# mmorise/World

Hardware: AMD Instinct MI355X
Metric: analysis frames/sec (Harvest+CheapTrick+D4C, 48 kHz, 5 ms hop) (higher is better)
Workload: dtype f64; 1 GPU; configs[1]: 1 x (48 kHz, 10 s) utterance(s) per step, Harvest+CheapTrick+D4C, fft_size=2048, frame_period=5 ms, inputs/outputs in HBM, 12 independent jobs in flight (one HIP stream + context each, a different utterance per job); utterances_per_gpu=1, jobs_in_flight=12, parallelism=single GPU, no collective

## Files before the change

### include/world_hip.h

```cpp
#ifndef WORLD_HIP_H_
#define WORLD_HIP_H_

#ifdef __cplusplus
extern "C" {
#endif

#if defined(__GNUC__)
#define WORLD_HIP_API __attribute__((visibility("default")))
#else
#define WORLD_HIP_API
#endif


typedef struct {
  double f0_floor;
  double f0_ceil;
  double channels_in_octave;
  double frame_period;
  int speed;
  double allowed_range;
} DioOption;

typedef struct {
  double f0_floor;
// ... 58 lines not shown
  fft_complex *c_in;
  double *in;
  fft_complex *c_out;
  double *out;
  double *input;
  int *ip;
  double *w;
} fft_plan;
typedef struct {
  int fft_size;
  double *waveform;
  fft_complex *spectrum;
  fft_plan forward_fft;
} ForwardRealFFT;
typedef struct {
  int fft_size;
  double *waveform;
  fft_complex *spectrum;
  fft_plan inverse_fft;
} InverseRealFFT;
typedef struct {
  int fft_size;
  double *log_spectrum;
  fft_complex *minimum_phase_spectrum;
  fft_complex *cepstrum;
  fft_plan inverse_fft;
  fft_plan forward_fft;
} MinimumPhaseAnalysis;
typedef struct {
  unsigned int g_randn_x;
  unsigned int g_randn_y;
  unsigned int g_randn_z;
  unsigned int g_randn_w;
} RandnState;
typedef struct {
  int fs;
  double frame_period;
  int buffer_size;
  int number_of_pointers;
  int fft_size;
  double *buffer;
  int current_pointer;
  int i;
  double *dc_remover;
  int *f0_length;
  int *f0_origin;
  double ***spectrogram;
  double ***aperiodicity;
  int current_pointer2;
  int head_pointer;
  int synthesized_sample;
  int handoff;
  double handoff_phase;
  double handoff_f0;
  int last_location;
  int cumulative_frame;
  int current_frame;
  double **interpolated_vuv;
  double **pulse_locations;
  int **pulse_locations_index;
  int *number_of_pulses;
  double *impulse_response;
  RandnState randn_state;
  MinimumPhaseAnalysis minimum_phase;
  InverseRealFFT inverse_real_fft;
  ForwardRealFFT forward_real_fft;
} WorldSynthesizer;
WORLD_HIP_API void InitializeSynthesizer(int fs, double frame_period, int fft_size, int buffer_size,
                                         int number_of_pointers, WorldSynthesizer *synth);
WORLD_HIP_API int AddParameters(double *f0, int f0_length, double **spectrogram, double **aperiodicity,
                                WorldSynthesizer *synth);
WORLD_HIP_API void RefreshSynthesizer(WorldSynthesizer *synth);
WORLD_HIP_API void DestroySynthesizer(WorldSynthesizer *synth);
WORLD_HIP_API int IsLocked(WorldSynthesizer *synth);
WORLD_HIP_API int Synthesis2(WorldSynthesizer *synth);

WORLD_HIP_API void wavwrite(const double *x, int x_length, int fs, int nbit, const char *filename);
WORLD_HIP_API int GetAudioLength(const char *filename);
WORLD_HIP_API void wavread(const char *filename, int *fs, int *nbit, double *x);
WORLD_HIP_API void WriteF0(const char *filename, int f0_length, double frame_period,
                           const double *temporal_positions, const double *f0, int text_flag);
WORLD_HIP_API int ReadF0(const char *filename, double *temporal_positions, double *f0);
WORLD_HIP_API double GetHeaderInformation(const char *filename, const char *parameter);
WORLD_HIP_API void WriteSpectralEnvelope(const char *filename, int fs, int f0_length, double frame_period,
                                         int fft_size, int number_of_dimensions, const double *const *spectrogram);
WORLD_HIP_API int ReadSpectralEnvelope(const char *filename, double **spectrogram);
WORLD_HIP_API void WriteAperiodicity(const char *filename, int fs, int f0_length, double frame_period,
                                     int fft_size, int number_of_dimensions, const double *const *aperiodicity);
WORLD_HIP_API int ReadAperiodicity(const char *filename, double **aperiodicity);


typedef void (*WorldHipErrorHandler)(const char *function, const char *message, void *user);
WORLD_HIP_API void world_hip_set_error_handler(WorldHipErrorHandler handler, void *user);
WORLD_HIP_API int world_hip_shutdown(void);
WORLD_HIP_API void world_hip_dropin_stats(unsigned long long *slots, unsigned long long *x_hits,
                                          unsigned long long *x_misses);

typedef struct WorldHipContext WorldHipContext;

WORLD_HIP_API WorldHipContext *world_hip_create(int device, void *stream);
WORLD_HIP_API void world_hip_destroy(WorldHipContext *ctx);
WORLD_HIP_API const char *world_hip_last_error(void);
#define WORLD_HIP_ABI_VERSION 6
#define WORLD_HIP_HINT_SHARED_DEVICE 1
WORLD_HIP_API int world_hip_set_hint(WorldHipContext *ctx, int hint);
WORLD_HIP_API int world_hip_abi_version(void);
WORLD_HIP_API int world_hip_sync(WorldHipContext *ctx);
WORLD_HIP_API unsigned long long world_hip_workspace_bytes(WorldHipContext *ctx);
WORLD_HIP_API unsigned long long world_hip_noise_table_bytes(WorldHipContext *ctx);
WORLD_HIP_API int world_hip_verify_tables(WorldHipContext *ctx);
WORLD_HIP_API double world_hip_noise_table_build_ms(WorldHipContext *ctx, int *builds);

WORLD_HIP_API void world_hip_profile_enable(int on);
WORLD_HIP_API int world_hip_profile_collect(char *buf, int cap);

WORLD_HIP_API int world_hip_harvest_batch(WorldHipContext *ctx, int n_utt, int fs, const double *d_x,
                                          int x_stride, const int *x_length, const HarvestOption *option,
                                          int f_stride, double *d_tpos, double *d_f0);
WORLD_HIP_API int world_hip_dio_batch(WorldHipContext *ctx, int n_utt, int fs, const double *d_x,
                                      int x_stride, const int *x_length, const DioOption *option,
                                      int f_stride, double *d_tpos, double *d_f0);
WORLD_HIP_API int world_hip_stonemask_batch(WorldHipContext *ctx, int n_utt, int fs, const double *d_x,
                                            int x_stride, const int *x_length, const int *n_frames,
                                            int f_stride, const double *d_tpos, const double *d_f0,
                                            double *d_refined_f0);
WORLD_HIP_API int world_hip_cheaptrick_batch(WorldHipContext *ctx, int n_utt, int fs, const double *d_x,
                                             int x_stride, const int *x_length, const int *n_frames,
                                             int f_stride, const double *d_tpos, const double *d_f0,
                                             const CheapTrickOption *option, double *d_spectrogram);
WORLD_HIP_API int world_hip_d4c_batch(WorldHipContext *ctx, int n_utt, int fs, const double *d_x,
                                      int x_stride, const int *x_length, const int *n_frames,
                                      int f_stride, const double *d_tpos, const double *d_f0,
                                      int fft_size, const D4COption *option, double *d_aperiodicity);

WORLD_HIP_API int world_hip_synthesis_batch(WorldHipContext *ctx, int n_utt, int fs, double frame_period,
                                            int fft_size, const int *n_frames, int f_stride, const double *d_f0,
                                            const double *d_spectrogram, const double *d_aperiodicity,
                                            const int *y_length, int y_stride, double *d_y);

WORLD_HIP_API int world_hip_synthesis_records(WorldHipContext *ctx, int n_utt, int fs, double frame_period, int fft_size,
                                              const int *n_frames, long long first_row, const double *d_block, int cols,
                                              int wire, int number_of_dimensions, const int *y_length, int y_stride,
                                              double *d_y);

WORLD_HIP_API int world_hip_probe_machine(WorldHipContext *ctx, double *values, int n_values);
WORLD_HIP_API int world_hip_probe_rfft(WorldHipContext *ctx, int lg_n, int max_lr, int threads, int static_plan,
                                       long long batch, const double *d_in, double *d_spectrum);
WORLD_HIP_API int world_hip_probe_irfft(WorldHipContext *ctx, int lg_n, int max_lr, int threads, int static_plan,
                                        long long batch, const double *d_spectrum, double *d_out);
WORLD_HIP_API int world_hip_probe_fft(WorldHipContext *ctx, int mode, int lg_n, int max_lr, int threads, int swizzle,
                                      long long batch, const void *d_in, void *d_out);
WORLD_HIP_API int world_hip_probe_select(WorldHipContext *ctx, int mode, int threads, int K, long long rows,
                                         const double *d_keys, double *d_out);
WORLD_HIP_API int world_hip_probe_harvest_contour(WorldHipContext *ctx, int n_utt, const int *nfb, const int *nc, int maxc,
                                                  int fb_stride, const double *d_cand, const double *d_score, double frame_period,
                                                  int f_stride, double *d_pruned_cand, double *d_pruned_score, double *d_step2,
                                                  double *d_step3, double *d_step4, int sec_cap, int *d_sec_n, int *d_sec,
                                                  double *d_basic_f0, double *d_tpos, double *d_f0);
WORLD_HIP_API int world_hip_probe_harvest_candidates(WorldHipContext *ctx, int n_utt, const int *nfb, double afs, double f0_floor,
                                                     double f0_ceil, int nch, const double *band_f0, int maxc, int fb_stride,
                                                     int nseg, int seg_cap, int ev_cap, int ev_group, int stages,
                                                     const double *d_seg_events, const int *d_seg_count, double *d_events,
                                                     int *d_ev_count, double *d_raw, double *d_cand, int *d_nc);

WORLD_HIP_API int world_hip_analyze_batch(WorldHipContext *ctx, int n_utt, int fs, const double *d_x, int x_stride,
                                          const int *x_length, const HarvestOption *harvest_option,
                                          const CheapTrickOption *cheaptrick_option, const D4COption *d4c_option,
                                          int f_stride, double *d_tpos, double *d_f0, double *d_spectrogram,
                                          double *d_aperiodicity);
WORLD_HIP_API int world_hip_record_columns(int fft_size, int wire);
WORLD_HIP_API int world_hip_analyze_packed(WorldHipContext *ctx, int n_utt, int fs, const double *d_x, int x_stride,
                                           const int *x_length, const HarvestOption *harvest_option,
                                           const CheapTrickOption *cheaptrick_option, const D4COption *d4c_option,
                                           long long first_row, double *d_block, int cols);
WORLD_HIP_API int world_hip_coded_columns(int fs, int number_of_dimensions);
WORLD_HIP_API int world_hip_analyze_coded(WorldHipContext *ctx, int n_utt, int fs, const double *d_x, int x_stride,
                                          const int *x_length, const HarvestOption *harvest_option,
                                          const CheapTrickOption *cheaptrick_option, const D4COption *d4c_option,
                                          int number_of_dimensions, long long first_row, double *d_block, int cols);
WORLD_HIP_API int world_hip_spectral_packed_range(WorldHipContext *ctx, int n_utt, int fs, const double *d_x, int x_stride,
                                                  const int *x_length, const int *n_frames, int f_stride,
                                                  const double *d_tpos, const double *d_f0,
                                                  const CheapTrickOption *cheaptrick_option, const D4COption *d4c_option,
                                                  int frame_lo, int frame_hi, int reuse_offsets, long long first_row,
                                                  double *d_block, int cols);
WORLD_HIP_API int world_hip_cheaptrick_batch_range(WorldHipContext *ctx, int n_utt, int fs, const double *d_x, int x_stride,
                                                   const int *x_length, const int *n_frames, int f_stride,
                                                   const double *d_tpos, const double *d_f0, const CheapTrickOption *option,
                                                   int frame_lo, int frame_hi, int reuse_offsets, double *d_spectrogram);
WORLD_HIP_API int world_hip_d4c_batch_range(WorldHipContext *ctx, int n_utt, int fs, const double *d_x, int x_stride,
                                            const int *x_length, const int *n_frames, int f_stride, const double *d_tpos,
                                            const double *d_f0, int fft_size, const D4COption *option, int frame_lo,
                                            int frame_hi, int reuse_offsets, double *d_aperiodicity);
WORLD_HIP_API int world_hip_pack_results(WorldHipContext *ctx, int n_utt, const int *n_frames, int f_stride,
                                         int bins, const double *d_tpos, const double *d_f0,
                                         const double *d_spectrogram, const double *d_aperiodicity,
                                         long long first_row, double *d_block);
WORLD_HIP_API int world_hip_unpack_results(WorldHipContext *ctx, int n_utt, const int *n_frames, int f_stride,
                                           int bins, const double *d_block, long long first_row, double *d_tpos,
                                           double *d_f0, double *d_spectrogram, double *d_aperiodicity);
WORLD_HIP_API int world_hip_allgather_blocks(int n_dev, WorldHipContext *const *ctxs, const double *const *d_src,
                                             const long long *rows, int cols, double *const *d_dst);

WORLD_HIP_API int world_hip_analyze_sharded(int n_dev, WorldHipContext *const *ctxs, int n_utt, int fs,
                                            const double *const *x, const int *x_length,
                                            const HarvestOption *harvest_option, const CheapTrickOption *cheaptrick_option,
                                            const D4COption *d4c_option, int sub_batch, double *const *d_blocks,
                                            long long rows_capacity, int cols, long long *where);

WORLD_HIP_API int world_hip_check_shape(int fs, int cheaptrick_fft_size, char *why, int why_capacity);

WORLD_HIP_API int world_hip_graph_begin(WorldHipContext *ctx);
WORLD_HIP_API int world_hip_graph_end(WorldHipContext *ctx, void **graph);
WORLD_HIP_API int world_hip_graph_launch(WorldHipContext *ctx, void *graph);
WORLD_HIP_API int world_hip_graph_destroy(void *graph);

WORLD_HIP_API int world_hip_set_synthesis_pulse_capacity(WorldHipContext *ctx, int pulses_per_utterance);
WORLD_HIP_API int world_hip_synthesis_pulses_dropped(WorldHipContext *ctx, int *needed);

WORLD_HIP_API int world_hip_pcm16_to_double(WorldHipContext *ctx, long long n, const short *d_pcm, double *d_x);

WORLD_HIP_API int world_hip_pcm_to_double(WorldHipContext *ctx, long long n, int nbit, const void *d_pcm, double *d_x);
WORLD_HIP_API int world_hip_double_to_pcm16(WorldHipContext *ctx, long long n, const double *d_x, short *d_pcm);
WORLD_HIP_API int world_hip_wav_layout(const char *filename, int *fs, int *nbit, int *x_length,
                                       long long *data_offset);
WORLD_HIP_API int world_hip_wav_write_pcm16(const char *filename, int fs, long long n, const short *pcm);

#define WORLD_HIP_RESAMPLE_BEST 0
#define WORLD_HIP_RESAMPLE_FAST 1
typedef struct { int zeros; double rolloff; double kaiser_beta; } WorldHipResampleOption;
WORLD_HIP_API void world_hip_resample_option(int quality, WorldHipResampleOption *opt);
WORLD_HIP_API int world_hip_resample_length(int n_in, int fs_in, int fs_out);
WORLD_HIP_API int world_hip_resample_shape(int fs_in, int fs_out, const WorldHipResampleOption *opt, int *L, int *M, int *W);
WORLD_HIP_API int world_hip_resample_taps(int fs_in, int fs_out, const WorldHipResampleOption *opt, double *table );
WORLD_HIP_API int world_hip_resample_batch(WorldHipContext *ctx, int n_utt, int fs_in, int fs_out,
                                           const WorldHipResampleOption *opt, const double *d_x, int x_stride,
                                           const int *x_length , double *d_y, int y_stride);

WORLD_HIP_API double world_hip_mcep_alpha(int fs);
WORLD_HIP_API int world_hip_mcep_tables(int fft_size, int order, double alpha, double *M ,
                                        double *D );
WORLD_HIP_API int world_hip_sp2mc(WorldHipContext *ctx, int rows, int fft_size, int order, double alpha, const double *d_sp,
                                  long long sp_row_stride, double *d_mc, long long mc_row_stride);
WORLD_HIP_API int world_hip_mc2sp(WorldHipContext *ctx, int rows, int fft_size, int order, double alpha, const double *d_mc,
                                  long long mc_row_stride, double *d_sp, long long sp_row_stride);

WORLD_HIP_API int world_hip_delta_batch(WorldHipContext *ctx, int n_utt, int dim, int n_win, int half_width,
                                        const double *win , const int *n_frames ,
                                        const unsigned char *d_mask, long long mask_utt_stride, const double *d_c,
                                        long long c_utt_stride, long long c_row_stride, double fill, double *d_out,
                                        long long out_utt_stride, long long out_row_stride);
WORLD_HIP_API int world_hip_mlpg_batch(WorldHipContext *ctx, int n_utt, int dim, int n_win, int half_width,
                                       const double *win , const int *n_frames ,
                                       const unsigned char *d_mask, long long mask_utt_stride, const double *d_mean,
                                       long long mean_utt_stride, long long mean_row_stride, const double *d_var,
                                       long long var_utt_stride, long long var_row_stride, int precision, double fill,
                                       double *d_out, long long out_utt_stride, long long out_row_stride);

WORLD_HIP_API long long world_hip_gmm_model_doubles(int M, int Dx, int Dy);
WORLD_HIP_API int world_hip_gmm_prepare(int M, int Dx, int Dy, const double *w, const double *mu, const double *cov,
                                        double *model );
WORLD_HIP_API int world_hip_gmm_model_parts(int M, int Dx, int Dy, const double *model , double *c, double *mux,
                                            double *muy, double *U, double *A, double *v);
WORLD_HIP_API int world_hip_gmm_convert(WorldHipContext *ctx, int M, int Dx, int Dy, const double *d_model, int rows,
                                        const double *d_x, long long x_row_stride, int mode, double *d_mean,
                                        long long mean_row_stride, double *d_var, long long var_row_stride, double *d_post,
                                        long long post_row_stride, double *d_loglik);
WORLD_HIP_API int world_hip_gmm_accumulate(WorldHipContext *ctx, int M, int P, int rows, const double *d_z,
                                           long long z_row_stride, const double *d_post, long long post_row_stride,
                                           const double *d_shift , double *d_N , double *d_S1 ,
                                           double *d_G );
WORLD_HIP_API int world_hip_gmm_update(int M, int P, const double *N, const double *S1, const double *G, const double *shift,
                                       double total_rows, double reg, double *w, double *mu, double *cov);
WORLD_HIP_API int world_hip_gmm_fit(WorldHipContext *ctx, int M, int P, int rows, const double *d_z, long long z_row_stride,
                                    int n_iter, double reg, double *w, double *mu, double *cov ,
                                    double *loglik );
WORLD_HIP_API int world_hip_gmm_init(WorldHipContext *ctx, int M, int P, int rows, const double *d_z, long long z_row_stride,
                                     double *w, double *mu, double *cov );

WORLD_HIP_API int world_hip_frame_power_batch(WorldHipContext *ctx, int n_utt, int fft_size, const int *n_frames ,
                                              const double *d_sp, long long sp_utt_stride, long long sp_row_stride,
                                              double *d_power, long long power_utt_stride, double *d_mean);
WORLD_HIP_API int world_hip_select_frames_batch(WorldHipContext *ctx, int n_utt, const int *n_frames ,
                                                const double *d_value, long long value_utt_stride, long long value_stride,
                                                double threshold, const double *d_scale, const unsigned char *d_mask,
                                                long long mask_utt_stride, int *d_index, long long index_utt_stride,
                                                int *d_count, unsigned char *d_keep, long long keep_utt_stride);
WORLD_HIP_API int world_hip_gather_rows_batch(WorldHipContext *ctx, int n_utt, int dim, const int *n_src ,
                                              const double *d_in, long long in_utt_stride, long long in_row_stride,
                                              const int *n_out , const int *d_index, long long index_utt_stride,
                                              double fill, double *d_out, long long out_utt_stride, long long out_row_stride);
WORLD_HIP_API int world_hip_joint_rows_batch(WorldHipContext *ctx, int n_pairs, int dim_a, int dim_b, const double *d_a,
                                             const long long *a_row , const int *n_a , long long a_row_stride,
                                             const double *d_b, const long long *b_row , const int *n_b ,
                                             long long b_row_stride, const int *path_len , const int *d_path,
                                             int p_stride, const int *d_sel_a, const int *n_sel_a ,
                                             long long sel_a_stride, const int *d_sel_b, const int *n_sel_b ,
                                             long long sel_b_stride, double fill, double *d_z, const long long *z_row ,
                                             long long z_row_stride);

WORLD_HIP_API int world_hip_code_spectral_envelope(WorldHipContext *ctx, int rows, int fs, int fft_size,
                                                   int number_of_dimensions, const double *d_spectrogram,
                                                   double *d_coded);
WORLD_HIP_API int world_hip_decode_spectral_envelope(WorldHipContext *ctx, int rows, int fs, int fft_size,
                                                     int number_of_dimensions, const double *d_coded,
                                                     double *d_spectrogram);
// ... 76 lines not shown
```

### world_amd/api.py

```python
import ctypes as C
import os
import weakref

import numpy as np

HERE = os.path.dirname(os.path.abspath(__file__))
LIB_PATH = os.environ.get("WORLD_HIP_LIB") or os.path.join(HERE, "libworld_hip.so")

_dp = C.POINTER(C.c_double)
_ip = C.POINTER(C.c_int)


class DioOption(C.Structure):
    _fields_ = [("f0_floor", C.c_double), ("f0_ceil", C.c_double), ("channels_in_octave", C.c_double),
                ("frame_period", C.c_double), ("speed", C.c_int), ("allowed_range", C.c_double)]


class HarvestOption(C.Structure):
    _fields_ = [("f0_floor", C.c_double), ("f0_ceil", C.c_double), ("frame_period", C.c_double)]


class CheapTrickOption(C.Structure):
    _fields_ = [("q1", C.c_double), ("f0_floor", C.c_double), ("fft_size", C.c_int)]

# ... 90 lines not shown
                ("cepstrum", C.c_void_p), ("inverse_fft", FftPlan), ("forward_fft", FftPlan)]


class WorldSynthesizer(C.Structure):
    _fields_ = [("fs", C.c_int), ("frame_period", C.c_double), ("buffer_size", C.c_int), ("number_of_pointers", C.c_int),
                ("fft_size", C.c_int), ("buffer", _dp), ("current_pointer", C.c_int), ("i", C.c_int),
                ("dc_remover", _dp), ("f0_length", _ip), ("f0_origin", _ip), ("spectrogram", C.c_void_p),
                ("aperiodicity", C.c_void_p), ("current_pointer2", C.c_int), ("head_pointer", C.c_int),
                ("synthesized_sample", C.c_int), ("handoff", C.c_int), ("handoff_phase", C.c_double),
                ("handoff_f0", C.c_double), ("last_location", C.c_int), ("cumulative_frame", C.c_int),
                ("current_frame", C.c_int), ("interpolated_vuv", C.c_void_p), ("pulse_locations", C.c_void_p),
                ("pulse_locations_index", C.POINTER(_ip)), ("number_of_pulses", _ip), ("impulse_response", _dp),
                ("randn_state", RandnState), ("minimum_phase", MinimumPhaseAnalysis),
                ("inverse_real_fft", InverseRealFFT), ("forward_real_fft", ForwardRealFFT)]


REALTIME_SCALARS = ("current_pointer", "i", "current_pointer2", "head_pointer", "synthesized_sample", "handoff",
                    "handoff_phase", "handoff_f0", "last_location", "cumulative_frame", "current_frame")
RT_ADD, RT_SYNTH, RT_LOCKED, RT_REFRESH = 0, 1, 2, 3


def bind_realtime(L):
    sp = C.POINTER(WorldSynthesizer)
    L.InitializeSynthesizer.argtypes = [C.c_int, C.c_double, C.c_int, C.c_int, C.c_int, sp]
    L.InitializeSynthesizer.restype = None
    L.AddParameters.argtypes = [_dp, C.c_int, C.POINTER(_dp), C.POINTER(_dp), sp]
    L.RefreshSynthesizer.argtypes = [sp]
    L.RefreshSynthesizer.restype = None
    L.DestroySynthesizer.argtypes = [sp]
    L.DestroySynthesizer.restype = None
    L.IsLocked.argtypes = [sp]
    L.Synthesis2.argtypes = [sp]
    return L


def run_realtime_plan(L, plan):
    fs, fp, fft, bs, P = (int(plan["fs"]), float(plan["frame_period"]), int(plan["fft_size"]), int(plan["buffer_size"]),
                          int(plan["number_of_pointers"]))
    f0, sp, ap = _f64(plan["f0"]), _f64(plan["sp"]), _f64(plan["ap"])
    chunks = [int(c) for c in plan["chunks"]]
    drain_every = int(plan.get("drain_every", 1))
    refresh_before = int(plan.get("refresh_before", -1))
    stop_on_lock = bool(plan.get("stop_on_lock", False))
    rows_sp, rows_ap = _rows(sp), _rows(ap)

    def at(rows, i):
        return C.cast(C.c_void_p(C.cast(rows, C.c_void_p).value + i * C.sizeof(_dp)), C.POINTER(_dp))

    s = WorldSynthesizer()
    L.InitializeSynthesizer(fs, fp, fft, bs, P, C.byref(s))
    calls, out, pulses, counts, rings = [], [], [], [], []

    def record(op, ret):
        r = s.randn_state
        calls.append([op, ret] + [getattr(s, k) for k in REALTIME_SCALARS] +
                     [r.g_randn_x, r.g_randn_y, r.g_randn_z, r.g_randn_w])

    def drain():
        while True:
            r = L.Synthesis2(C.byref(s))
            record(RT_SYNTH, r)
            if r == 0:
                break
            out.append(np.ctypeslib.as_array(s.buffer, shape=(bs,)).copy())
        locked = L.IsLocked(C.byref(s))
        record(RT_LOCKED, locked)
        return locked

    i = k = adds = 0
    refused = 0
    try:
        while k < len(chunks):
            if k == refresh_before and refused == 0:
                L.RefreshSynthesizer(C.byref(s))
                record(RT_REFRESH, 0)
                refresh_before = -1
            n = chunks[k]
            r = L.AddParameters(f0[i:].ctypes.data_as(_dp), n, at(rows_sp, i), at(rows_ap, i), C.byref(s))
            record(RT_ADD, r)
            if r == 1:
                slot = (s.head_pointer - 1) % P
                npu = s.number_of_pulses[slot]
                counts.append(npu)
                if npu:
                    pulses.extend(s.pulse_locations_index[slot][:npu])
                i += n; k += 1; adds += 1; refused = 0
                w = min(adds, P)
                rings.append([[s.f0_length[j] if j < w else 0 for j in range(P)],
                              [s.f0_origin[j] if j < w else 0 for j in range(P)],
                              [s.number_of_pulses[j] for j in range(P)]])
                if adds % drain_every != 0 and k < len(chunks):
                    continue
            else:
                refused += 1
                if refused > 1:
                    break
            if drain() and stop_on_lock:
                break
    finally:
        L.DestroySynthesizer(C.byref(s))
    return {"calls": np.array(calls, dtype=np.float64).reshape(-1, 2 + len(REALTIME_SCALARS) + 4),
            "out": np.concatenate(out) if out else np.zeros(0), "pulses": np.array(pulses, dtype=np.int64),
            "pulse_counts": np.array(counts, dtype=np.int64), "rings": np.array(rings, dtype=np.int64).reshape(-1, 3, P)}


def _hip_runtime_first():
    try:
        import torch
    except ImportError:
        pass


def load_library(path=LIB_PATH):
    if not os.path.exists(path):
        raise ImportError(f"{path} is missing: build it with `python -m world_amd.build` "
                          "(hipcc, gfx950). There is no non-GPU fallback.")
    _hip_runtime_first()
    lib = C.CDLL(path)
    abi = lib.world_hip_abi_version() if hasattr(lib, "world_hip_abi_version") else 5
    if abi not in (5, 6):
        raise ImportError(f"{path}: batched ABI version {abi}, this binding speaks 5-6")
    lib.abi_version = abi
    vp = C.c_void_p
    lib.world_hip_create.restype = vp
    lib.world_hip_create.argtypes = [C.c_int, vp]
    lib.world_hip_destroy.argtypes = [vp]
    lib.world_hip_last_error.restype = C.c_char_p
    lib.world_hip_sync.argtypes = [vp]
    lib.world_hip_workspace_bytes.restype = C.c_ulonglong
    lib.world_hip_workspace_bytes.argtypes = [vp]
    lib.world_hip_noise_table_bytes.restype = C.c_ulonglong
    lib.world_hip_noise_table_bytes.argtypes = [vp]
    lib.world_hip_verify_tables.argtypes = [vp]
    lib.world_hip_harvest_batch.argtypes = [vp, C.c_int, C.c_int, vp, C.c_int, _ip, C.POINTER(HarvestOption),
                                            C.c_int, vp, vp]
    lib.world_hip_dio_batch.argtypes = [vp, C.c_int, C.c_int, vp, C.c_int, _ip, C.POINTER(DioOption),
                                        C.c_int, vp, vp]
    lib.world_hip_stonemask_batch.argtypes = [vp, C.c_int, C.c_int, vp, C.c_int, _ip, _ip, C.c_int, vp, vp, vp]
    lib.world_hip_cheaptrick_batch.argtypes = [vp, C.c_int, C.c_int, vp, C.c_int, _ip, _ip, C.c_int, vp, vp,
                                               C.POINTER(CheapTrickOption), vp]
    lib.world_hip_d4c_batch.argtypes = [vp, C.c_int, C.c_int, vp, C.c_int, _ip, _ip, C.c_int, vp, vp, C.c_int,
                                        C.POINTER(D4COption), vp]
    lib.world_hip_synthesis_batch.argtypes = [vp, C.c_int, C.c_int, C.c_double, C.c_int, _ip, C.c_int, vp, vp, vp,
                                              _ip, C.c_int, vp]
    lib.world_hip_pcm16_to_double.argtypes = [vp, C.c_longlong, vp, vp]
    lib.world_hip_set_synthesis_pulse_capacity.argtypes = [vp, C.c_int]
    lib.world_hip_synthesis_pulses_dropped.argtypes = [vp, _ip]
    lib.world_hip_probe_rfft.argtypes = [vp, C.c_int, C.c_int, C.c_int, C.c_int, C.c_longlong, vp, vp]
    lib.world_hip_probe_irfft.argtypes = [vp, C.c_int, C.c_int, C.c_int, C.c_int, C.c_longlong, vp, vp]
    if hasattr(lib, "world_hip_probe_fft"):
        lib.world_hip_probe_fft.argtypes = [vp, C.c_int, C.c_int, C.c_int, C.c_int, C.c_int, C.c_longlong, vp, vp]
    if hasattr(lib, "world_hip_probe_select"):
        lib.world_hip_probe_select.argtypes = [vp, C.c_int, C.c_int, C.c_int, C.c_longlong, vp, vp]
    if hasattr(lib, "world_hip_probe_harvest_contour"):
        lib.world_hip_probe_harvest_contour.argtypes = [vp, C.c_int, _ip, _ip, C.c_int, C.c_int, vp, vp, C.c_double, C.c_int,
                                                        vp, vp, vp, vp, vp, C.c_int, vp, vp, vp, vp, vp]
    if hasattr(lib, "world_hip_probe_harvest_candidates"):
        lib.world_hip_probe_harvest_candidates.argtypes = [vp, C.c_int, _ip, C.c_double, C.c_double, C.c_double, C.c_int,
                                                           C.POINTER(C.c_double)] + [C.c_int] * 7 + [vp] * 7
    lib.world_hip_analyze_packed.argtypes = [vp, C.c_int, C.c_int, vp, C.c_int, _ip, C.POINTER(HarvestOption),
                                             C.POINTER(CheapTrickOption), C.POINTER(D4COption), C.c_longlong, vp, C.c_int]
    lib.world_hip_analyze_sharded.argtypes = [C.c_int, C.POINTER(vp), C.c_int, C.c_int, C.POINTER(vp), _ip,
                                              C.POINTER(HarvestOption), C.POINTER(CheapTrickOption), C.POINTER(D4COption),
                                              C.c_int, C.POINTER(vp), C.c_longlong, C.c_int, C.POINTER(C.c_longlong)]
    lib.world_hip_check_shape.argtypes = [C.c_int, C.c_int, C.c_char_p, C.c_int]
    if hasattr(lib, "world_hip_set_hint"):
        lib.world_hip_set_hint.argtypes = [vp, C.c_int]
    if hasattr(lib, "world_hip_probe_machine"):
        lib.world_hip_probe_machine.argtypes = [vp, C.POINTER(C.c_double), C.c_int]
    lib.world_hip_record_columns.argtypes = [C.c_int, C.c_int]
    if hasattr(lib, "world_hip_analyze_coded"):
        lib.world_hip_coded_columns.argtypes = [C.c_int, C.c_int]
        lib.world_hip_analyze_coded.argtypes = [vp, C.c_int, C.c_int, vp, C.c_int, _ip, C.POINTER(HarvestOption),
                                                C.POINTER(CheapTrickOption), C.POINTER(D4COption), C.c_int, C.c_longlong, vp, C.c_int]
    lib.world_hip_spectral_packed_range.argtypes = [vp, C.c_int, C.c_int, vp, C.c_int, _ip, _ip, C.c_int, vp, vp,
                                                    C.POINTER(CheapTrickOption), C.POINTER(D4COption), C.c_int, C.c_int,
                                                    C.c_int, C.c_longlong, vp, C.c_int]
    lib.world_hip_cheaptrick_batch_range.argtypes = [vp, C.c_int, C.c_int, vp, C.c_int, _ip, _ip, C.c_int, vp, vp,
                                                     C.POINTER(CheapTrickOption), C.c_int, C.c_int, C.c_int, vp]
    lib.world_hip_d4c_batch_range.argtypes = [vp, C.c_int, C.c_int, vp, C.c_int, _ip, _ip, C.c_int, vp, vp, C.c_int,
                                              C.POINTER(D4COption), C.c_int, C.c_int, C.c_int, vp]
    lib.world_hip_analyze_batch.argtypes = [vp, C.c_int, C.c_int, vp, C.c_int, _ip, C.POINTER(HarvestOption),
                                            C.POINTER(CheapTrickOption), C.POINTER(D4COption), C.c_int, vp, vp, vp, vp]
    lib.world_hip_graph_begin.argtypes = [vp]
    lib.world_hip_graph_end.argtypes = [vp, C.POINTER(vp)]
    lib.world_hip_graph_launch.argtypes = [vp, vp]
    lib.world_hip_graph_destroy.argtypes = [vp]
    lib.world_hip_pack_results.argtypes = [vp, C.c_int, _ip, C.c_int, C.c_int, vp, vp, vp, vp, C.c_longlong, vp]
    lib.world_hip_unpack_results.argtypes = [vp, C.c_int, _ip, C.c_int, C.c_int, vp, C.c_longlong, vp, vp, vp, vp]
    lib.world_hip_allgather_blocks.argtypes = [C.c_int, C.POINTER(vp), C.POINTER(vp), C.POINTER(C.c_longlong), C.c_int,
                                               C.POINTER(vp)]
    lib.world_hip_pcm_to_double.argtypes = [vp, C.c_longlong, C.c_int, vp, vp]
    lib.world_hip_double_to_pcm16.argtypes = [vp, C.c_longlong, vp, vp]
    lib.world_hip_wav_layout.argtypes = [C.c_char_p, _ip, _ip, _ip, C.POINTER(C.c_longlong)]
    lib.world_hip_wav_write_pcm16.argtypes = [C.c_char_p, C.c_int, C.c_longlong, vp]
    lib.world_hip_code_spectral_envelope.argtypes = [vp, C.c_int, C.c_int, C.c_int, C.c_int, vp, vp]
    lib.world_hip_decode_spectral_envelope.argtypes = [vp, C.c_int, C.c_int, C.c_int, C.c_int, vp, vp]
    lib.world_hip_code_aperiodicity.argtypes = [vp, C.c_int, C.c_int, C.c_int, vp, vp]
    lib.world_hip_decode_aperiodicity.argtypes = [vp, C.c_int, C.c_int, C.c_int, vp, vp]
    lib.GetNumberOfAperiodicities.argtypes = [C.c_int]
    lib.GetFFTSizeForCheapTrick.argtypes = [C.c_int, C.POINTER(CheapTrickOption)]
    if hasattr(lib, "world_hip_realtime_create"):
        lib.world_hip_realtime_create.argtypes = [vp, C.c_int, C.c_int, C.c_double, C.c_int, C.c_int, C.c_int,
                                                  C.POINTER(vp)]
        lib.world_hip_realtime_destroy.argtypes = [vp]
        lib.world_hip_realtime_destroy.restype = None
        lib.world_hip_realtime_add.argtypes = [vp, C.c_int, _dp, C.c_int, vp, vp, C.c_int]
        lib.world_hip_realtime_synthesize.argtypes = [vp, vp, _ip]
        lib.world_hip_realtime_is_locked.argtypes = [vp, C.c_int]
        lib.world_hip_realtime_refresh.argtypes = [vp, C.c_int]
        lib.world_hip_realtime_rng_jump.argtypes = [C.POINTER(C.c_uint32), C.c_ulonglong, C.POINTER(C.c_uint32)]
        lib.world_hip_realtime_rng_jump.restype = None
    if hasattr(lib, "world_hip_modify_batch"):
        mp = C.POINTER(WorldHipModification)
        lib.world_hip_f0_statistics.argtypes = [vp, C.c_int, _ip, C.c_int, vp, vp]
        lib.world_hip_modify_batch.argtypes = [vp, C.c_int, C.c_int, C.c_int, _ip, C.c_int, mp, vp, vp, vp, vp]
        lib.world_hip_resynthesis_length.argtypes = [C.c_int, C.c_int, C.c_double, C.c_double]
        lib.world_hip_resynthesize_batch.argtypes = [vp, C.c_int, C.c_int, vp, C.c_int, _ip, C.POINTER(HarvestOption),
                                                     C.POINTER(CheapTrickOption), C.POINTER(D4COption), mp, C.c_double,
                                                     _ip, C.c_int, vp]
    if hasattr(lib, "world_hip_modify_frames_batch"):
        mp, cp = C.POINTER(WorldHipModification), C.POINTER(WorldHipFrameCurves)
        lib.world_hip_modify_frames_batch.argtypes = [vp, C.c_int, C.c_int, C.c_int, _ip, C.c_int, _ip, C.c_int, mp, cp,
                                                      vp, vp, vp, vp, vp, vp]
        lib.world_hip_resynthesize_frames_batch.argtypes = [vp, C.c_int, C.c_int, vp, C.c_int, _ip, C.POINTER(HarvestOption),
                                                            C.POINTER(CheapTrickOption), C.POINTER(D4COption), mp, cp, _ip,
                                                            C.c_int, _ip, C.c_int, vp]
    if hasattr(lib, "world_hip_synthesis_records"):
        lib.world_hip_synthesis_records.argtypes = [vp, C.c_int, C.c_int, C.c_double, C.c_int, _ip, C.c_longlong, vp,
                                                    C.c_int, C.c_int, C.c_int, _ip, C.c_int, vp]
        lib.world_hip_realtime_add_coded.argtypes = [vp, C.c_int, _dp, C.c_int, vp, C.c_int, vp, C.c_int]
    if hasattr(lib, "world_hip_align_batch"):
        lp = C.POINTER(C.c_longlong)
        lib.world_hip_align_batch.argtypes = [vp, C.c_int, C.c_int, vp, lp, _ip, C.c_int, vp, lp, _ip, C.c_int, C.c_int,
                                              vp, vp, vp, C.c_int, vp, vp]
        lib.world_hip_align_workspace_cells.argtypes = []
    if hasattr(lib, "world_hip_morph_batch"):
        lib.world_hip_morph_length.argtypes = [C.c_int, C.c_int, C.c_double]
        lib.world_hip_morph_batch.argtypes = [vp, C.c_int, C.c_int, C.c_int, _ip, C.c_int, vp, vp, vp, _ip, C.c_int, vp, vp, vp,
                                              C.c_int, vp, vp, C.POINTER(WorldHipMorph), C.POINTER(WorldHipMorphCurves),
                                              C.c_int, vp, vp, vp, vp, vp]
    if hasattr(lib, "world_hip_resample_batch"):
        op = C.POINTER(WorldHipResampleOption)
        lib.world_hip_resample_option.argtypes = [C.c_int, op]
        lib.world_hip_resample_option.restype = None
        lib.world_hip_resample_length.argtypes = [C.c_int, C.c_int, C.c_int]
        lib.world_hip_resample_shape.argtypes = [C.c_int, C.c_int, op, _ip, _ip, _ip]
        lib.world_hip_resample_taps.argtypes = [C.c_int, C.c_int, op, vp]
        lib.world_hip_resample_batch.argtypes = [vp, C.c_int, C.c_int, C.c_int, op, vp, C.c_int, _ip, vp, C.c_int]
    if hasattr(lib, "world_hip_sp2mc"):
        lib.world_hip_mcep_alpha.argtypes = [C.c_int]
        lib.world_hip_mcep_alpha.restype = C.c_double
        lib.world_hip_mcep_tables.argtypes = [C.c_int, C.c_int, C.c_double, vp, vp]
        for fn in (lib.world_hip_sp2mc, lib.world_hip_mc2sp):
            fn.argtypes = [vp, C.c_int, C.c_int, C.c_int, C.c_double, vp, C.c_longlong, vp, C.c_longlong]
    if hasattr(lib, "world_hip_mlpg_batch"):
        ll = C.c_longlong
        lib.world_hip_delta_batch.argtypes = [vp, C.c_int, C.c_int, C.c_int, C.c_int, vp, _ip, vp, ll, vp, ll, ll, C.c_double,
                                              vp, ll, ll]
        lib.world_hip_mlpg_batch.argtypes = [vp, C.c_int, C.c_int, C.c_int, C.c_int, vp, _ip, vp, ll, vp, ll, ll, vp, ll, ll,
                                             C.c_int, C.c_double, vp, ll, ll]
    if hasattr(lib, "world_hip_gmm_convert"):
        ll, i, d = C.c_longlong, C.c_int, C.c_double
        lib.world_hip_gmm_model_doubles.argtypes = [i, i, i]
        lib.world_hip_gmm_model_doubles.restype = ll
        lib.world_hip_gmm_prepare.argtypes = [i, i, i, vp, vp, vp, vp]
        lib.world_hip_gmm_model_parts.argtypes = [i, i, i, vp, vp, vp, vp, vp, vp, vp]
        lib.world_hip_gmm_convert.argtypes = [vp, i, i, i, vp, i, vp, ll, i, vp, ll, vp, ll, vp, ll, vp]
        lib.world_hip_gmm_accumulate.argtypes = [vp, i, i, i, vp, ll, vp, ll, vp, vp, vp, vp]
        lib.world_hip_gmm_update.argtypes = [i, i, vp, vp, vp, vp, d, d, vp, vp, vp]
        lib.world_hip_gmm_fit.argtypes = [vp, i, i, i, vp, ll, i, d, vp, vp, vp, vp]
        lib.world_hip_gmm_init.argtypes = [vp, i, i, i, vp, ll, vp, vp, vp]
    if hasattr(lib, "world_hip_joint_rows_batch"):
        ll, i, d, lp = C.c_longlong, C.c_int, C.c_double, C.POINTER(C.c_longlong)
        lib.world_hip_frame_power_batch.argtypes = [vp, i, i, _ip, vp, ll, ll, vp, ll, vp]
        lib.world_hip_select_frames_batch.argtypes = [vp, i, _ip, vp, ll, ll, d, vp, vp, ll, vp, ll, vp, vp, ll]
        lib.world_hip_gather_rows_batch.argtypes = [vp, i, i, _ip, vp, ll, ll, _ip, vp, ll, d, vp, ll, ll]
        lib.world_hip_joint_rows_batch.argtypes = [vp, i, i, i, vp, lp, _ip, ll, vp, lp, _ip, ll, _ip, vp, i, vp, _ip, ll, vp, _ip, ll,
                                                   d, vp, lp, ll]
    lib.world_hip_profile_enable.argtypes = [C.c_int]
    lib.world_hip_profile_collect.argtypes = [C.c_char_p, C.c_int]
    return lib


def frame_count(fs, x_length, frame_period):
    return int(1000.0 * x_length / fs / frame_period) + 1


def resample_length(n_in, fs_in, fs_out):
    import math
    n_in, fs_in, fs_out = int(n_in), int(fs_in), int(fs_out)
    if n_in < 1 or fs_in < 1 or fs_out < 1:
        raise ValueError(f"resample_length: {n_in} samples, {fs_in} -> {fs_out} Hz")
    g = math.gcd(fs_in, fs_out)
    n = -((-n_in * (fs_out // g)) // (fs_in // g))
    if n > 2 ** 31 - 1:
        raise ValueError(f"resample_length: {n_in} samples at {fs_in} Hz are more than INT_MAX at {fs_out} Hz")
    return n


def resample_option(quality="best"):
    if isinstance(quality, WorldHipResampleOption):
        return quality
    if isinstance(quality, str):
        if quality not in RESAMPLE_QUALITIES:
            raise ValueError(f"resample: quality {quality!r} is neither 'best' nor 'fast' nor a (zeros, rolloff, beta) triple")
# ... 1624 lines not shown
```

### world_amd/csrc/api.hip

```cpp
#include "../../include/world_hip.h"

#include <algorithm>
#include <climits>
#include <cmath>
#include <cstdint>
#include <cstring>
#include <cstdarg>
#include <deque>
#include <mutex>
#include <thread>
#include <unordered_map>
#include <stdexcept>
#include <string>
#include <vector>

#include "common.h"
#include "bandfilter.h"
#include "codec.h"
#include "decimate.h"
#include "dio.h"
#include "exchange.h"
#include "fft_probe.h"
#include "d4c_select_probe.h"
#include "gmm_host.h"
// ... 271 lines not shown
}
template <class T> static T *upload(WorldHipContext *c, const std::vector<T> &v) { return upload(c, v.data(), v.size()); }

struct Span { const void *p; size_t bytes; const char *name; };
static void refuse_overlap(const char *call, std::initializer_list<Span> outs, std::initializer_list<Span> ins) {
  auto meet = [](const Span &a, const Span &b) {
    const char *a_lo = static_cast<const char *>(a.p), *b_lo = static_cast<const char *>(b.p);
    return a.p && b.p && a_lo < b_lo + b.bytes && b_lo < a_lo + a.bytes;
  };
  for (const Span *o = outs.begin(); o != outs.end(); ++o) {
    for (const Span &i : ins)
      if (meet(*o, i)) fail("%s: %s overlaps %s; no output may alias an input", call, o->name, i.name);
    for (const Span *o2 = o + 1; o2 != outs.end(); ++o2)
      if (meet(*o, *o2)) fail("%s: %s overlaps %s", call, o->name, o2->name);
  }
}

static int ilog2_exact(int n) {
  int l = 0;
  while ((1 << l) < n) ++l;
  if ((1 << l) != n) fail("fft size %d is not a power of two", n);
  return l;
}
constexpr int kGridY = 65535;

static int frame_count(int fs, int x_length, double frame_period) {
  return static_cast<int>(1000.0 * x_length / fs / frame_period) + 1;
}

static void check_batch(int n_utt, int fs, const void *d_x, int x_stride, const int *x_length) {
  if (n_utt <= 0) fail("n_utt must be positive");
  if (fs <= 0) fail("fs must be positive");
  if (!d_x || !x_length) fail("null input");
  for (int u = 0; u < n_utt; ++u)
    if (x_length[u] <= 0 || x_length[u] > x_stride) fail("x_length[%d]=%d outside (0, x_stride=%d]", u, x_length[u], x_stride);
}
static int max_frame_count(const int *n_frames, int n_utt, int f_stride) {
  int max_frames = 0;
  for (int u = 0; u < n_utt; ++u) {
    if (n_frames[u] < 0 || n_frames[u] > f_stride) fail("n_frames[%d] outside [0, f_stride]", u);
    max_frames = std::max(max_frames, n_frames[u]);
  }
  return max_frames;
}
static std::vector<int> record_rows(const int *n_frames, int n_utt, long long first_row) {
  std::vector<int> rows(n_utt);
  long long row = first_row;
  for (int u = 0; u < n_utt; ++u) {
    if (row + n_frames[u] > 0x7FFFFFFFll) fail("block exceeds 2^31 records");
    rows[u] = static_cast<int>(row);
    row += n_frames[u];
  }
  return rows;
}
static BatchView batch_view(WorldHipContext *c, int n_utt, int fs, const double *d_x, int x_stride, const int *x_length,
                            const int *n_frames, int f_stride) {
  BatchView b;
  b.n_utt = n_utt; b.fs = fs; b.x_stride = x_stride; b.f_stride = f_stride; b.x = d_x;
  b.x_len = upload(c, std::vector<int>(x_length, x_length + n_utt));
  b.n_frames = upload(c, std::vector<int>(n_frames, n_frames + n_utt));
  return b;
}

struct RowLayout {
  const int *rows = nullptr;
  size_t stride = 0;
  size_t col_bytes = 0;
  int f32 = 0;
  double *rec = nullptr;
  int code_dims = 0;
  const int *code_knot = nullptr;
  const double *code_frac = nullptr, *code_w_re = nullptr, *code_w_im = nullptr;
  int frame_lo = 0, frame_hi = 0x7FFFFFFF;
  bool skip_prepare = false;
};
static int record_cols(int fft_size, int wire) {
  const int nb = fft_size / 2 + 1;
  return wire == 1 ? 2 + nb : 2 + 2 * nb;
}

static int d4c_internal_fft(int fs) { return static_cast<int>(pow(2.0, 1.0 + static_cast<int>(log(4.0 * fs / kFloorF0D4C + 1) / kLog2))); }
static int d4c_park_slots(int n_utt, int f_stride) {
  return static_cast<int>(std::min<size_t>((size_t)n_utt * f_stride, (size_t)std::max(n_utt, 2048)));
}

static void arena_reset(WorldHipContext *c) {
  c->arena.reset();
  c->prep_ct.valid = c->prep_d4c.valid = false;
}
template <class Carve> static void begin_stage(WorldHipContext *c, Carve carve) {
  ensure_arena(c, measure(carve));
  arena_reset(c);
  devrt::dpoison(c->arena.base + c->arena.floor, c->arena.cap - c->arena.floor, c->stream);
  carve(c->arena);
  open_uploads(c);
}
template <class Carve, class Body> static void hold_at_floor(WorldHipContext *c, const char *what, Carve carve, Body body) {
  struct Release {
    WorldHipContext *c;
    ~Release() { c->arena.floor = 0; c->prep_ct.valid = c->prep_d4c.valid = false; }
  } release{c};
  size_t want = 0;
  for (int attempt = 0;; ++attempt) {
    c->arena.floor = 0;
    ensure_arena(c, std::max(measure(carve), want));
    arena_reset(c);
    devrt::dpoison(c->arena.base, c->arena.cap, c->stream);
    carve(c->arena);
    c->arena.floor = c->arena.used;
    try {
      body();
      return;
    } catch (const ArenaRegrow &r) {
      if (devrt::is_capturing(c->stream)) fail("a call shape that was never run before cannot be captured: run it once first");
      if (attempt >= 4) fail("%s: the workspace did not settle", what);
      want = std::max(want, r.bytes);
    }
  }
}

static uint64_t lengths_hash(const int *x_length, const int *n_frames, int n_utt) {
  const uint64_t a = SmallArrays::hash(x_length, sizeof(int) * n_utt), b = SmallArrays::hash(n_frames, sizeof(int) * n_utt);
  return a * 0x9E3779B97F4A7C15ull ^ b;
}
static void claim_prepared(WorldHipContext *c, WorldHipContext::PrepToken &mine, WorldHipContext::PrepToken &other,
                           WorldHipContext::PrepToken want, bool reuse, const char *stage) {
  want.arena_base = c->arena.base; want.generation = c->generation;
  if (reuse) {
    if (!mine.valid)
      fail("%s: reuse_offsets, but this context holds no prepared offsets (another stage, another shape or a regrown "
           "workspace since the call that prepared them)", stage);
    if (!mine.same_inputs(want))
      fail("%s: reuse_offsets, but the prepared offsets belong to other inputs (shape, buffers or options differ from the "
           "call that prepared them)", stage);
    return;
  }
  if (other.valid && want.lo < other.hi && other.lo < want.hi) other.valid = false;
  mine = want;
  mine.valid = true;
}
static void carve_cheaptrick(Arena &a, CtParams &p) {
  p.offsets = a.take<unsigned>((size_t)p.b.n_utt * p.b.f_stride);
  p.frec = a.take<CtFrameRec>((size_t)p.b.n_utt * p.b.f_stride);
}
static void carve_d4c(Arena &a, D4cParams &p) {
  CtParams below;
  below.b = p.b;
  carve_cheaptrick(a, below);
  const size_t fr = (size_t)p.b.n_utt * p.b.f_stride;
  p.ap0 = a.take<double>(fr);
  p.offsets1 = a.take<unsigned>(fr);
  p.draws2 = a.take<unsigned>(fr);
  p.draws1 = a.take<unsigned>(p.b.n_utt);
  p.frec = a.take<D4cFrameRec>(fr);
  p.coarse = a.take<double>(fr * 16);
  const size_t slot = d4c_park_slot_doubles(p.lg_d4c);
  p.park_ws = slot ? a.take<double>(slot * p.park_slots) : nullptr;
}
static void spectral_workspace(WorldHipContext *c, CtParams *ct, D4cParams *d4c, const int *x_length, const int *n_frames) {
  ensure_arena(c, d4c ? measure([&](Arena &a) { carve_d4c(a, *d4c); }) : measure([&](Arena &a) { carve_cheaptrick(a, *ct); }));
  const BatchView &b = ct ? ct->b : d4c->b;
  WorldHipContext::PrepToken t;
  t.n_utt = b.n_utt; t.fs = b.fs; t.f_stride = b.f_stride; t.x_stride = b.x_stride; t.x = b.x;
  t.lengths_hash = lengths_hash(x_length, n_frames, b.n_utt);
  if (ct) {
    c->arena.reset();
    carve_cheaptrick(c->arena, *ct);
    t.fft = 1 << ct->lg_fft; t.f0 = ct->f0; t.tpos = ct->tpos; t.opt = ct->f0_floor;
    t.lo = 0; t.hi = c->arena.used;
    claim_prepared(c, c->prep_ct, c->prep_d4c, t, ct->skip_prepare != 0, "CheapTrick");
    if (!ct->skip_prepare) devrt::dpoison(c->arena.base + c->arena.floor, c->arena.used - c->arena.floor, c->stream);
  }
  if (d4c) {
    c->arena.reset();
    carve_d4c(c->arena, *d4c);
    t.fft = d4c->fft_out; t.f0 = d4c->f0; t.tpos = d4c->tpos; t.opt = d4c->threshold;
    t.lo = reinterpret_cast<char *>(d4c->ap0) - c->arena.base; t.hi = c->arena.used;
    claim_prepared(c, c->prep_d4c, c->prep_ct, t, d4c->skip_prepare != 0, "D4C");
    char *lo = reinterpret_cast<char *>(d4c->skip_prepare ? d4c->coarse : d4c->ap0);
    devrt::dpoison(lo, c->arena.base + c->arena.used - lo, c->stream);
  }
}

static std::string shape_limit(int what, int fs, int fft_size);
static void refuse_shape_limit(int what, int fs, int fft_size) {
  const std::string lim = shape_limit(what, fs, fft_size);
  if (!lim.empty()) fail("%s", lim.c_str());
}
static bool inkernel_consts() { return getenv("WORLD_HIP_INKERNEL_CONSTS") != nullptr; }
static CtParams setup_cheaptrick(WorldHipContext *c, int n_utt, int fs, const double *d_x, int x_stride,
                                 const int *x_length, const int *n_frames, int f_stride, const double *d_tpos,
                                 const double *d_f0, const CheapTrickOption *opt, double *d_sp, const RowLayout &lay,
                                 int *max_frames_out) {
  check_batch(n_utt, fs, d_x, x_stride, x_length);
  const int lg = ilog2_exact(opt->fft_size);
  const std::string lim = shape_limit(2, fs, opt->fft_size);
  if (!lim.empty()) fail("%s", lim.c_str());
  const int max_frames = *max_frames_out = max_frame_count(n_frames, n_utt, f_stride);
  CtParams p;
  p.b = batch_view(c, n_utt, fs, d_x, x_stride, x_length, n_frames, f_stride);
  p.tpos = d_tpos; p.f0 = d_f0; p.spectrogram = d_sp;
  p.out_row = lay.rows ? upload(c, std::vector<int>(lay.rows, lay.rows + n_utt)) : nullptr;
  p.out_stride = lay.stride ? lay.stride : (size_t)(opt->fft_size / 2 + 1);
  p.out_col_bytes = lay.col_bytes; p.out_f32 = lay.f32;
  p.code_ndim = lay.code_dims; p.code_knot = lay.code_knot; p.code_frac = lay.code_frac;
  p.code_w_re = lay.code_w_re; p.code_w_im = lay.code_w_im;
  if (p.code_ndim > 0 && (lay.f32 || !lay.code_knot || p.code_ndim > opt->fft_size / 4 + 1)) fail("CheapTrick: bad coded-row layout");
  p.f0_floor = 3.0 * fs / (opt->fft_size - 3.0);
  p.noise = ensure_noise(c, (size_t)max_frames * ct_max_draws_per_frame(opt->fft_size));
  p.tab = c->tab;
  p.q1 = opt->q1;
  p.lg_fft = lg;
  p.frec = nullptr;
  p.frame_consts = inkernel_consts() ? 0 : 1;
  p.frame_threads = ct_frame_threads(lg);
  p.lift0 = (1.0 - 2.0 * opt->q1) + 2.0 * opt->q1;
  if (lay.frame_lo < 0 || lay.frame_hi < lay.frame_lo) fail("bad frame range [%d, %d)", lay.frame_lo, lay.frame_hi);
  p.frame_lo = lay.frame_lo; p.frame_hi = lay.frame_hi; p.skip_prepare = lay.skip_prepare ? 1 : 0;
  return p;
}
static void run_cheaptrick(WorldHipContext *c, int n_utt, int fs, const double *d_x, int x_stride,
                           const int *x_length, const int *n_frames, int f_stride, const double *d_tpos,
                           const double *d_f0, const CheapTrickOption *opt, double *d_sp,
                           const RowLayout &lay = RowLayout()) {
  open_uploads(c);
  int max_frames = 0;
  CtParams p = setup_cheaptrick(c, n_utt, fs, d_x, x_stride, x_length, n_frames, f_stride, d_tpos, d_f0, opt, d_sp, lay,
                                &max_frames);
  spectral_workspace(c, &p, nullptr, x_length, n_frames);
  launch_cheaptrick(p, max_frames, c->stream);
}

static D4cParams setup_d4c(WorldHipContext *c, int n_utt, int fs, const double *d_x, int x_stride, const int *x_length,
                           const int *n_frames, int f_stride, const double *d_tpos, const double *d_f0, int fft_size,
                           const D4COption *opt, double *d_ap, const RowLayout &lay, int *max_frames_out) {
  check_batch(n_utt, fs, d_x, x_stride, x_length);
  ilog2_exact(fft_size);
  const int max_frames = *max_frames_out = max_frame_count(n_frames, n_utt, f_stride);
  const int fft_d4c = d4c_internal_fft(fs);
  const int fft_love = static_cast<int>(pow(2.0, 1.0 + static_cast<int>(log(3.0 * fs / 40.0 + 1) / kLog2)));
  if (fft_d4c > 16384 || fft_love > 16384)
    fail("D4C: fs=%d needs an internal FFT of %d > 16384 points (LDS budget); fs <= 192 kHz supported", fs, std::max(fft_d4c, fft_love));
  if (fs < 15800) fail("D4C: fs=%d is below the 15.8 kHz the reference's LoveTrain band edges require", fs);
  const int nap = static_cast<int>(std::min(15000.0, fs / 2.0 - 3000.0) / 3000.0);
  const int wl = static_cast<int>(3000.0 * fft_d4c / fs) * 2 + 1;
  if (nap < 1 || nap > 6) fail("D4C: unsupported number of aperiodicity bands %d", nap);
  if (c->nuttall_len != wl) {
    std::vector<double> w(wl);
    for (int i = 0; i < wl; ++i) {
      double t = i / (wl - 1.0);
      w[i] = 0.355768 - 0.487396 * cos(2.0 * kPi * t) + 0.144232 * cos(4.0 * kPi * t) - 0.012604 * cos(6.0 * kPi * t);
    }
    devrt::sync(c->stream);
    put_table(c, c->d_nuttall, w);
    devrt::sync(c->stream);
    c->nuttall_len = wl;
  }
  if (c->ap_grid_fs != fs || c->ap_grid_fft != fft_size) {
    const int nb_out = fft_size / 2 + 1, nk = nap + 2;
    std::vector<double> frac(nb_out);
    std::vector<int> knot(nb_out);
    for (int i = 0; i < nb_out; ++i) {
      const double xi = static_cast<double>(i) * fs / fft_size;
      int cnt = 0;
      for (int k = 0; k < nk; ++k) {
        const double kn = k <= nap ? k * 3000.0 : fs / 2.0;
        if (kn <= xi) cnt++;
      }
      const int k = cnt < 1 ? 1 : (cnt > nk - 1 ? nk - 1 : cnt);
      const double x0 = (k - 1) <= nap ? (k - 1) * 3000.0 : fs / 2.0;
      const double x1 = k <= nap ? k * 3000.0 : fs / 2.0;
      knot[i] = k;
      frac[i] = (xi - x0) / (x1 - x0);
    }
    devrt::sync(c->stream);
    put_table(c, c->d_ap_frac, frac);
    put_table(c, c->d_ap_knot, knot);
    devrt::sync(c->stream);
    c->ap_grid_fs = fs; c->ap_grid_fft = fft_size;
  }
  D4cParams p;
  p.b = batch_view(c, n_utt, fs, d_x, x_stride, x_length, n_frames, f_stride);
  p.tpos = d_tpos; p.f0 = d_f0; p.aperiodicity = d_ap;
  p.out_row = lay.rows ? upload(c, std::vector<int>(lay.rows, lay.rows + n_utt)) : nullptr;
  p.out_stride = lay.stride ? lay.stride : (size_t)(fft_size / 2 + 1);
  p.out_col_bytes = lay.col_bytes; p.out_f32 = lay.f32;
  p.code_nap = lay.code_dims;
  if (p.code_nap > 0 && lay.f32) fail("D4C: bad coded-row layout");
  p.rec = lay.rec;
  p.park_slots = d4c_park_slots(n_utt, f_stride);
  p.noise = ensure_noise(c, (size_t)max_frames * d4c_max_draws_per_frame(fs));
  p.nuttall = c->d_nuttall;
  p.ap_frac = c->d_ap_frac; p.ap_knot = c->d_ap_knot;
  p.tab = c->tab;
  p.threshold = opt->threshold;
  p.fft_out = fft_size;
  p.lg_love = ilog2_exact(fft_love);
  p.lg_d4c = ilog2_exact(fft_d4c);
  p.nap = nap;
  p.wl = wl;
  if (wl / 2 + 1 > 512) fail("D4C: band window of %d samples at fs=%d exceeds the 1023 the frame kernel is built for", wl, fs);
  for (int b = 0; b < 8; ++b) p.band_center[b] = static_cast<int>(3000.0 * (b + 1) * fft_d4c / fs);
  p.frec = nullptr;
  p.frame_consts = inkernel_consts() ? 0 : 1;
  p.love_threads = d4c_love_threads(p.lg_love);
  p.frame_threads = d4c_frame_threads(p.lg_d4c);
  p.love_b[0] = static_cast<int>(ceil(100.0 * fft_love / fs));
  p.love_b[1] = static_cast<int>(ceil(4000.0 * fft_love / fs));
  p.love_b[2] = static_cast<int>(ceil(7900.0 * fft_love / fs));
  p.band_bnd = mround(fft_d4c * 8.0 / wl);
  if (lay.frame_lo < 0 || lay.frame_hi < lay.frame_lo) fail("bad frame range [%d, %d)", lay.frame_lo, lay.frame_hi);
  p.frame_lo = lay.frame_lo; p.frame_hi = lay.frame_hi;
  p.skip_prepare = lay.skip_prepare ? kD4cSkipScan | kD4cSkipLoveTrain : 0;
  return p;
}
static void run_d4c(WorldHipContext *c, int n_utt, int fs, const double *d_x, int x_stride, const int *x_length,
                    const int *n_frames, int f_stride, const double *d_tpos, const double *d_f0, int fft_size,
                    const D4COption *opt, double *d_ap, const RowLayout &lay = RowLayout()) {
  open_uploads(c);
  int max_frames = 0;
  D4cParams p = setup_d4c(c, n_utt, fs, d_x, x_stride, x_length, n_frames, f_stride, d_tpos, d_f0, fft_size, opt, d_ap,
                          lay, &max_frames);
  spectral_workspace(c, nullptr, &p, x_length, n_frames);
  launch_d4c(p, max_frames, c->stream);
}

static void prepare_bands(WorldHipContext *c, int fs, double f0_floor, double f0_ceil, int ratio) {
  HarvestBands &hb = c->bands;
  if (hb.fs == fs && hb.f0_floor == f0_floor && hb.f0_ceil == f0_ceil && hb.nch > 0) return;
  const double lo = f0_floor * 0.9, hi = f0_ceil * 1.1, cpo = 40;
  const int nch = 1 + static_cast<int>(log(hi / lo) / kLog2 * cpo);
  const double afs = static_cast<double>(fs) / ratio;
  std::vector<double> fb(nch), taps;
  std::vector<int> half(nch), off(nch);
  int max_half = 0;
  for (int i = 0; i < nch; ++i) {
    fb[i] = lo * pow(2.0, (i + 1) / cpo);
    const int L = mround(afs / fb[i] * 2.0);
    half[i] = L;
    off[i] = (int)taps.size();
    max_half = std::max(max_half, L);
    const int len = 2 * L + 1;
    for (int k = -L; k <= L; ++k) {
      double t = (k + L) / (len - 1.0);
      double w = 0.355768 - 0.487396 * cos(2.0 * kPi * t) + 0.144232 * cos(4.0 * kPi * t) - 0.012604 * cos(6.0 * kPi * t);
      taps.push_back(w * cos(2 * kPi * fb[i] * k / afs));
    }
  }
  devrt::sync(c->stream);
  put_table(c, hb.d_band_f0, fb);
  put_table(c, hb.d_taps, taps);
  put_table(c, hb.d_half, half);
  put_table(c, hb.d_off, off);
  devrt::sync(c->stream);
  hb.fs = fs; hb.f0_floor = f0_floor; hb.f0_ceil = f0_ceil; hb.nch = nch; hb.max_half = max_half;
  hb.band_f0 = fb;
  hb.fft_seg = getenv("WORLD_HIP_HARVEST_FIR") ? 0 : hv_fft_segment(max_half);
  if (hb.fft_seg > 0) {
    put_table(c, hb.d_spec, (size_t)nch * kBandFftBins);
    launch_band_spectra(hb.d_taps, hb.d_off, hb.d_half, nch, hb.d_spec, c->tab, c->stream);
    devrt::sync(c->stream);
  } else {
    drop_table(c, hb.d_spec);
  }
  const int hw_max = static_cast<int>(1.5 * afs / f0_floor + 1.0) + 2;
  const size_t head = (size_t)(hw_max + 1) * 6;
  std::vector<double> wt(head + (size_t)(hw_max + 1) * WAVE * 2);
  const long double pi_l = 3.14159265358979323846264338327950288L;
  for (int hw = 0; hw <= hw_max; ++hw) {
    const double wlen_t = (2.0 * hw + 1.0) / afs;
    const double d = (1.0 / afs) * (2.0 / wlen_t);
    wt[6 * hw + 0] = sin(kPi * d); wt[6 * hw + 1] = cos(kPi * d);
    wt[6 * hw + 2] = sin(kPi * (WAVE * d)); wt[6 * hw + 3] = cos(kPi * (WAVE * d));
    wt[6 * hw + 4] = 2.0 / ((2.0 * hw + 1.0) * (1.0 / afs));
    wt[6 * hw + 5] = kPi * d;
    const long double dl = 2.0L / (2.0L * hw + 1.0L);
    for (int lane = 0; lane < WAVE; ++lane) {
      const long double a = pi_l * (lane - hw - 1) * dl;
      wt[head + ((size_t)hw * WAVE + lane) * 2 + 0] = (double)sinl(a);
      wt[head + ((size_t)hw * WAVE + lane) * 2 + 1] = (double)cosl(a);
    }
  }
  hb.win_full_entries = 0;
  if (fmod(afs, 1000.0) == 0.0) {
    hb.win_full_entries = (size_t)(hw_max + 1) * (hw_max + 1);
    const size_t base = wt.size();
    wt.resize(base + 2 * hb.win_full_entries);
    std::vector<long double> w;
    for (int hw = 0; hw <= hw_max; ++hw) {
      const int blen = 2 * hw + 1;
      w.assign(blen, 0.0L);
      const long double dl = 2.0L / (2.0L * hw + 1.0L);
      for (int i = 0; i < blen; ++i) {
        const long double a = pi_l * (i - hw - 1) * dl;
        w[i] = 0.42L + 0.5L * cosl(a) + 0.08L * cosl(2.0L * a);
      }
      double *o = wt.data() + base + 2 * (size_t)hw * hw;
      for (int i = 0; i < blen; ++i) {
        long double dw;
        if (blen == 1) dw = 0.0L;
        else if (i == 0) dw = -w[1] / 2.0L;
        else if (i == blen - 1) dw = w[blen - 2] / 2.0L;
        else dw = -(w[i + 1] - w[i - 1]) / 2.0L;
        o[2 * i] = (double)w[i]; o[2 * i + 1] = (double)dw;
      }
    }
  }
  put_table(c, hb.d_win_tab, wt);
  devrt::sync(c->stream);
  hb.win_tab_len = hw_max + 1;
}

static void plan_harvest_tail(const WorldHipContext *c, HarvestParams &p, int n_utt, int max_fb) {
  p.fb_stride = (max_fb + 7) & ~7;
  p.sec_cap = hv_section_rows(max_fb);
  p.lone_job = n_utt == 1 && !(c->hint & WORLD_HIP_HINT_SHARED_DEVICE);
  p.ext_cap = max_fb + 304 * hv_sliced_sections(max_fb) + 8;
}
static void carve_harvest_tail(Arena &a, HarvestParams &p, size_t B) {
  const size_t cand_elems = B * p.fb_stride * p.maxc;
  p.cand_a = a.take<double>(cand_elems); p.score_a = a.take<double>(cand_elems);
  p.cand_b = a.take<double>(cand_elems); p.score_b = a.take<double>(cand_elems);
  p.nc = a.take<int>(B);
  p.c0 = a.take<double>(B * p.fb_stride);
  p.c2 = a.take<double>(B * p.fb_stride); p.c3 = a.take<double>(B * p.fb_stride);
  p.basic_f0 = a.take<double>(B * p.fb_stride);
  p.sec = a.take<int>(B * 6 * p.sec_cap);
  p.sec_n = a.take<int>(B * 2);
  p.sec_sum = a.take<double>(B * p.sec_cap);
  p.ext = a.take<double>(B * p.ext_cap);
}

static void run_harvest(WorldHipContext *c, int n_utt, int fs, const double *d_x, int x_stride,
                        const int *x_length, const HarvestOption *opt, int f_stride, double *d_tpos,
                        double *d_f0) {
  check_batch(n_utt, fs, d_x, x_stride, x_length);
  if (!(opt->f0_floor > 0) || !(opt->f0_ceil > opt->f0_floor) || !(opt->frame_period > 0)) fail("bad HarvestOption");
  HarvestParams p;
  p.ratio = std::max(std::min(mround(fs / 8000.0), 12), 1);
  p.afs = static_cast<double>(fs) / p.ratio;
  prepare_bands(c, fs, opt->f0_floor, opt->f0_ceil, p.ratio);
  const HarvestBands &hb = c->bands;
  p.f0_floor = opt->f0_floor; p.f0_ceil = opt->f0_ceil; p.frame_period = opt->frame_period;
  p.nch = hb.nch;
  p.maxc = mround(hb.nch / 10.0) * 7;
  if (p.maxc > 256) fail("Harvest: %d candidate slots per frame exceed the 256 the tracking kernel handles", p.maxc);
  p.lag = static_cast<int>(ceil(140.0 / p.ratio) * p.ratio);
  std::vector<int> xl(x_length, x_length + n_utt), yl(n_utt), nfb(n_utt), nfr(n_utt), rfft(n_utt);
  int max_x = 0, max_y = 0, max_fb = 0, max_fr = 0;
  for (int u = 0; u < n_utt; ++u) {
    yl[u] = static_cast<int>(ceil(static_cast<double>(xl[u]) / p.ratio));
    const int span = yl[u] + 5 + 2 * static_cast<int>(2.0 * p.afs / hb.band_f0[0]);
    rfft[u] = static_cast<int>(pow(2.0, static_cast<int>(log(static_cast<double>(span)) / kLog2) + 1.0));
    nfb[u] = frame_count(fs, xl[u], 1);
    nfr[u] = frame_count(fs, xl[u], opt->frame_period);
    if (nfr[u] > f_stride) fail("f_stride %d too small for %d frames", f_stride, nfr[u]);
    max_x = std::max(max_x, xl[u]); max_y = std::max(max_y, yl[u]);
    max_fb = std::max(max_fb, nfb[u]); max_fr = std::max(max_fr, nfr[u]);
  }
  p.y_stride = (max_y + 7) & ~7;
  plan_harvest_tail(c, p, n_utt, max_fb);
  p.m_stride = (max_x + 2 * p.lag + 2 * kDecPad + 7) & ~7;
  p.ev_cap = max_y / 2 + 2;
// ... 1804 lines not shown
    run_analyze_coded(c, n_utt, fs, d_x, x_stride, x_length, harvest_option, cheaptrick_option, d4c_option,
                      number_of_dimensions, first_row, d_block, cols);
  });
}

int world_hip_spectral_packed_range(WorldHipContext *c, int n_utt, int fs, const double *d_x, int x_stride, const int *x_length,
                                     const int *n_frames, int f_stride, const double *d_tpos, const double *d_f0,
                                     const CheapTrickOption *cheaptrick_option, const D4COption *d4c_option, int frame_lo,
                                     int frame_hi, int reuse_offsets, long long first_row, double *d_block, int cols) {
  return guarded(c, [&] {
    run_spectral_packed_range(c, n_utt, fs, d_x, x_stride, x_length, n_frames, f_stride, d_tpos, d_f0, cheaptrick_option,
                              d4c_option, frame_lo, frame_hi, first_row, d_block, cols, reuse_offsets != 0);
  });
}

int world_hip_cheaptrick_batch_range(WorldHipContext *c, int n_utt, int fs, const double *d_x, int x_stride,
                                     const int *x_length, const int *n_frames, int f_stride, const double *d_tpos,
                                     const double *d_f0, const CheapTrickOption *option, int frame_lo, int frame_hi,
                                     int reuse_offsets, double *d_sp) {
  return guarded(c, [&] {
    RowLayout lay;
    lay.frame_lo = frame_lo; lay.frame_hi = frame_hi; lay.skip_prepare = reuse_offsets != 0;
    run_cheaptrick(c, n_utt, fs, d_x, x_stride, x_length, n_frames, f_stride, d_tpos, d_f0, option, d_sp, lay);
  });
}
int world_hip_d4c_batch_range(WorldHipContext *c, int n_utt, int fs, const double *d_x, int x_stride, const int *x_length,
                              const int *n_frames, int f_stride, const double *d_tpos, const double *d_f0, int fft_size,
                              const D4COption *option, int frame_lo, int frame_hi, int reuse_offsets, double *d_ap) {
  return guarded(c, [&] {
    RowLayout lay;
    lay.frame_lo = frame_lo; lay.frame_hi = frame_hi; lay.skip_prepare = reuse_offsets != 0;
    run_d4c(c, n_utt, fs, d_x, x_stride, x_length, n_frames, f_stride, d_tpos, d_f0, fft_size, option, d_ap, lay);
  });
}

struct GraphHandle {
  void *exec;
  WorldHipContext *ctx;
  unsigned long long generation;
};
int world_hip_graph_begin(WorldHipContext *c) {
  return guarded(c, [&] { devrt::graph_begin(c->stream); });
}
int world_hip_graph_end(WorldHipContext *c, void **graph) {
  return guarded(c, [&] {
    if (!graph) fail("null graph handle");
    *graph = nullptr;
    void *exec = devrt::graph_end(c->stream);
    *graph = new GraphHandle{exec, c, c->generation};
  });
}
int world_hip_graph_launch(WorldHipContext *c, void *graph) {
  return guarded(c, [&] {
    if (!graph) fail("null graph");
    const GraphHandle *g = static_cast<const GraphHandle *>(graph);
    if (g->ctx != c) fail("graph_launch: the graph was captured on another context");
    if (g->generation != c->generation)
      fail("graph_launch: stale graph -- the context reallocated memory the graph points into since it was captured "
           "(a larger batch, a new option set or shape ran eagerly); capture it again");
    devrt::graph_launch(g->exec, c->stream);
  });
}
int world_hip_graph_destroy(void *graph) {
  if (!graph) return 0;
  GraphHandle *g = static_cast<GraphHandle *>(graph);
  try { devrt::graph_destroy(g->exec); delete g; return 0; } catch (const std::exception &e) { delete g; g_last_error = e.what(); return 1; }
}

int world_hip_check_shape(int fs, int cheaptrick_fft_size, char *why, int cap) {
  const std::string r = shape_limit(15, fs, cheaptrick_fft_size);
  if (why && cap > 0) { snprintf(why, (size_t)cap, "%s", r.c_str()); }
  return r.empty() ? 0 : 1;
}

int world_hip_synthesis_batch(WorldHipContext *c, int n_utt, int fs, double frame_period, int fft_size,
                              const int *n_frames, int f_stride, const double *d_f0, const double *d_spectrogram,
                              const double *d_aperiodicity, const int *y_length, int y_stride, double *d_y) {
  return guarded(c, [&] {
    run_synthesis(c, n_utt, fs, frame_period, fft_size, n_frames, f_stride, d_f0, d_spectrogram, d_aperiodicity,
                  y_length, y_stride, d_y);
  });
}

int world_hip_synthesis_records(WorldHipContext *c, int n_utt, int fs, double frame_period, int fft_size,
                                const int *n_frames, long long first_row, const double *d_block, int cols, int wire,
                                int number_of_dimensions, const int *y_length, int y_stride, double *d_y) {
  return guarded(c, [&] {
    run_synthesis_records(c, n_utt, fs, frame_period, fft_size, n_frames, first_row, d_block, cols, wire,
                          number_of_dimensions, y_length, y_stride, d_y);
  });
}

int world_hip_probe_machine(WorldHipContext *c, double *values, int n_values) {
  return guarded(c, [&] {
    if (!values || n_values < world_hip::kMachineProbeValues) fail("probe_machine: room for %d values needed", world_hip::kMachineProbeValues);
    devrt::sync(c->stream);
    world_hip::run_machine_probe(values, c->stream);
  });
}

static void run_fft_probe(WorldHipContext *c, bool inverse, int lg_n, int max_lr, int threads, int static_plan,
                          long long batch, const void *d_in, void *d_out) {
  if (lg_n < 6 || lg_n > kTwLog2) fail("probe: 2^%d points unsupported (64 .. %d)", lg_n, kTwN);
  if (max_lr != 3 && max_lr != 4) fail("probe: max_lr must be 3 (radix-8 plan) or 4 (radix-16 plan)");
  if (threads == 0) threads = std::max(64, (1 << lg_n) >> (max_lr + 1));
  if (threads < 64 || threads > 1024 || threads % 64) fail("probe: bad workgroup size %d", threads);
  if (batch < 0 || batch > 0x7FFFFFFFll) fail("probe: bad batch");
  if (batch == 0) return;
  if (!d_in || !d_out) fail("null buffer");
  if (static_plan && !fft_probe_has_static(lg_n, max_lr)) fail("probe: no compile-time plan for 2^%d points, max_lr %d", lg_n, max_lr);
  launch_fft_probe(inverse, lg_n, max_lr, threads, static_plan != 0, (long)batch, d_in, d_out, c->tab, c->stream);
}
int world_hip_probe_rfft(WorldHipContext *c, int lg_n, int max_lr, int threads, int static_plan, long long batch,
                         const double *d_in, double *d_spectrum) {
  return guarded(c, [&] { run_fft_probe(c, false, lg_n, max_lr, threads, static_plan, batch, d_in, d_spectrum); });
}
int world_hip_probe_irfft(WorldHipContext *c, int lg_n, int max_lr, int threads, int static_plan, long long batch,
                          const double *d_spectrum, double *d_out) {
  return guarded(c, [&] { run_fft_probe(c, true, lg_n, max_lr, threads, static_plan, batch, d_spectrum, d_out); });
}

int world_hip_probe_fft(WorldHipContext *c, int mode, int lg_n, int max_lr, int threads, int swizzle, long long batch,
                        const void *d_in, void *d_out) {
  return guarded(c, [&] {
    if (swizzle != 0 && swizzle != 1) fail("probe_fft: swizzle map %d unsupported (0: the shipped map, 1: d4c.hip's)", swizzle);
    if (batch < 0 || batch > 0x7FFFFFFFll) fail("probe_fft: bad batch");
    if (batch == 0) return;
    if (!d_in || !d_out) fail("null buffer");
#ifdef WORLD_EMU
    if (swizzle == 1 && !launch_fft_routes_swz1) fail("probe_fft: this host emulation was built without fft_probe_swz1.hip");
#endif
    const bool ok = swizzle == 0 ? launch_fft_routes_swz0(mode, lg_n, max_lr, threads, (long)batch, d_in, d_out, c->tab, c->stream)
                                 : launch_fft_routes_swz1(mode, lg_n, max_lr, threads, (long)batch, d_in, d_out, c->tab, c->stream);
    if (!ok)
      fail("probe_fft: mode %d at 2^%d points, max_lr %d, %d threads, swizzle %d is not a composition the stage kernels run.  Supported "
           "(threads = 64 .. 1024 in steps of 64 unless fixed; include/world_hip.h): modes 1, 2 at 2^6 .. 2^14, max_lr 3 or 4; 3 at "
           "2^6 .. 2^14, max_lr 3; 4, 5 at 2^6 .. 2^13, max_lr 4; 6 at 2^6 .. 2^13, max_lr 3; 7, 8, 9 at 2^10 .. 2^12, max_lr 3; 10 .. 13 "
           "at 2^12, max_lr 3, 256 threads; 14 .. 17 at 2^11 .. 2^14, max_lr 3, N / 16 threads; 18, 19 at lg_n 3 (rows of 8).  Swizzle 0 has modes "
           "1 .. 12, 18 and 19; swizzle 1 modes 1 (max_lr 3), 7 (2^11) and 13 .. 19.  Modes 7 .. 17 do not exist in the one-lane host emulation", mode, lg_n, max_lr, threads, swizzle);
  });
}

int world_hip_probe_select(WorldHipContext *c, int mode, int threads, int K, long long rows, const double *d_keys, double *d_out) {
  return guarded(c, [&] {
    if (mode != 0 && mode != 1) fail("probe_select: mode %d unsupported (0: block_excluding_largest, 1: block_smallest_sum)", mode);
    if (threads != 128 && threads != 256 && threads != 512 && threads != 1024)
      fail("probe_select: threads = %d is not one of d4c_frame's workgroup sizes (128, 256, 512, 1024)", threads);
    if (K < 1 || K > 10 * threads) fail("probe_select: K = %d outside 1 .. %d (the keys of a row)", K, 10 * threads);
    if (rows < 0 || rows > 0x7FFFFFFFll) fail("probe_select: bad rows");
    if (!d_keys || !d_out) fail("probe_select: null buffer (%s)", !d_keys ? "keys" : "out");
    if (rows == 0) return;
    if (!launch_d4c_select_probe(mode, threads, K, (long)rows, d_keys, d_out, c->stream)) fail("probe_select: threads = %d has no kernel", threads);
  });
}

int world_hip_probe_harvest_contour(WorldHipContext *c, int n_utt, const int *nfb, const int *nc, int maxc, int fb_stride,
                                    const double *d_cand, const double *d_score, double frame_period, int f_stride,
                                    double *d_pruned_cand, double *d_pruned_score, double *d_step2, double *d_step3,
                                    double *d_step4, int sec_cap, int *d_sec_n, int *d_sec, double *d_basic_f0,
                                    double *d_tpos, double *d_f0) {
  return guarded(c, [&] {
    const char *const me = "probe_harvest_contour";
    if (n_utt <= 0 || n_utt > kGridY) fail("%s: n_utt = %d outside 1 .. %d", me, n_utt, kGridY);
    if (!nfb || !nc) fail("%s: null buffer (%s)", me, !nfb ? "nfb" : "nc");
    if (maxc < 7 || maxc > 256 || maxc % 7) fail("%s: maxc = %d is not a multiple of 7 in 7 .. 252 (256 slots is what the tracking kernel handles)", me, maxc);
    if (!(frame_period > 0)) fail("%s: frame_period must be positive", me);
    const struct { const void *p; const char *name; } bufs[] = {
        {d_cand, "cand"}, {d_score, "score"}, {d_pruned_cand, "pruned_cand"}, {d_pruned_score, "pruned_score"}, {d_step2, "step2"},
        {d_step3, "step3"}, {d_step4, "step4"}, {d_sec_n, "sec_n"}, {d_sec, "sec"}, {d_basic_f0, "basic_f0"}, {d_tpos, "tpos"}, {d_f0, "f0"}};
    for (const auto &b : bufs)
      if (!b.p) fail("%s: null buffer (%s)", me, b.name);
    HarvestParams p{};
    p.maxc = maxc; p.frame_period = frame_period;
    std::vector<int> fb(nfb, nfb + n_utt), cn(nc, nc + n_utt), nfr(n_utt);
    int max_fb = 0, max_fr = 0;
    for (int u = 0; u < n_utt; ++u) {
      if (fb[u] < 1) fail("%s: nfb[%d] = %d: an utterance has at least one frame", me, u, fb[u]);
      if (cn[u] < 0 || cn[u] * 7 > maxc) fail("%s: nc[%d] = %d: 7 nc slots do not fit maxc = %d", me, u, cn[u], maxc);
      nfr[u] = static_cast<int>((fb[u] - 1) / frame_period) + 1;
      if (nfr[u] > f_stride) fail("%s: f_stride %d too small for %d frames", me, f_stride, nfr[u]);
      max_fb = std::max(max_fb, fb[u]); max_fr = std::max(max_fr, nfr[u]);
    }
    plan_harvest_tail(c, p, n_utt, max_fb);
    if (fb_stride != p.fb_stride) fail("%s: fb_stride = %d, the batch's is %d (max nfb rounded up to 8)", me, fb_stride, p.fb_stride);
    if (sec_cap != p.sec_cap) fail("%s: sec_cap = %d, the batch's is %d (max nfb / 2 + 4)", me, sec_cap, p.sec_cap);
    const size_t B = n_utt, row = p.fb_stride, cand_bytes = sizeof(double) * B * row * maxc;
    refuse_overlap(me,
                   {{d_pruned_cand, cand_bytes, "pruned_cand"}, {d_pruned_score, cand_bytes, "pruned_score"},
                    {d_step2, sizeof(double) * B * row, "step2"}, {d_step3, sizeof(double) * B * row, "step3"},
                    {d_step4, sizeof(double) * B * row, "step4"}, {d_basic_f0, sizeof(double) * B * row, "basic_f0"},
                    {d_sec_n, sizeof(int) * B * 2, "sec_n"}, {d_sec, sizeof(int) * B * 6 * p.sec_cap, "sec"},
                    {d_tpos, sizeof(double) * B * f_stride, "tpos"}, {d_f0, sizeof(double) * B * f_stride, "f0"}},
                   {{d_cand, cand_bytes, "cand"}, {d_score, cand_bytes, "score"}});
    begin_stage(c, [&](Arena &a) { carve_harvest_tail(a, p, B); });
    p.b.n_utt = n_utt; p.b.f_stride = f_stride;
    p.b.n_frames = upload(c, nfr);
    p.nfb = upload(c, fb);
    devrt::d2d(p.nc, upload(c, cn), sizeof(int) * B, c->stream);
    for (size_t u = 0; u < B; ++u) {
      const size_t at = u * row * maxc, n = sizeof(double) * fb[u] * maxc;
      devrt::d2d(p.cand_b + at, d_cand + at, n, c->stream);
      devrt::d2d(p.score_b + at, d_score + at, n, c->stream);
    }
    p.tpos = d_tpos; p.f0 = d_f0;
    launch_harvest_tail(p, max_fb, max_fr, c->stream);
    for (size_t u = 0; u < B; ++u) {
      const size_t at = u * row * maxc, n = sizeof(double) * fb[u] * maxc, f = u * row, nf = sizeof(double) * fb[u];
      if (cn[u]) {
        devrt::d2d(d_pruned_cand + at, p.cand_a + at, n, c->stream);
        devrt::d2d(d_pruned_score + at, p.score_a + at, n, c->stream);
      }
      devrt::d2d(d_step2 + f, p.c2 + f, nf, c->stream);
      devrt::d2d(d_step3 + f, p.c3 + f, nf, c->stream);
      devrt::d2d(d_step4 + f, p.c0 + f, nf, c->stream);
      devrt::d2d(d_basic_f0 + f, p.basic_f0 + f, nf, c->stream);
    }
    devrt::d2d(d_sec_n, p.sec_n, sizeof(int) * B * 2, c->stream);
    devrt::d2d(d_sec, p.sec, sizeof(int) * B * 6 * p.sec_cap, c->stream);
  });
}

int world_hip_probe_harvest_candidates(WorldHipContext *c, int n_utt, const int *nfb, double afs, double f0_floor, double f0_ceil,
                                       int nch, const double *band_f0, int maxc, int fb_stride, int nseg, int seg_cap, int ev_cap,
                                       int ev_group, int stages, const double *d_seg_events, const int *d_seg_count,
                                       double *d_events, int *d_ev_count, double *d_raw, double *d_cand, int *d_nc) {
  return guarded(c, [&] {
    const char *const me = "probe_harvest_candidates";
    if (n_utt <= 0 || n_utt > kGridY) fail("%s: n_utt = %d outside 1 .. %d", me, n_utt, kGridY);
    if (stages <= 0 || (stages & ~7)) fail("%s: stages = %d: 1 compaction, 2 raw candidates, 4 detection", me, stages);
    if (nch < 12 || nch > 365) fail("%s: nch = %d outside 12 .. 365", me, nch);
    if (!nfb || !band_f0) fail("%s: null buffer (%s)", me, !nfb ? "nfb" : "band_f0");
    for (int j = 0; j < nch; ++j)
      if (!(band_f0[j] > 0)) fail("%s: band_f0[%d] is not positive", me, j);
    if (maxc != mround(nch / 10.0) * 7) fail("%s: maxc = %d, Harvest's is %d (round(nch / 10) * 7)", me, maxc, mround(nch / 10.0) * 7);
    if (!(afs > 0) || !(f0_floor > 0) || !(f0_ceil > f0_floor)) fail("%s: afs, f0_floor, f0_ceil must be positive and ascending", me);
    if (nseg < 1) fail("%s: nseg = %d: at least one segment list", me, nseg);
    if (seg_cap < 1) fail("%s: seg_cap = %d: a segment list holds at least one event", me, seg_cap);
    if (ev_cap < 1) fail("%s: ev_cap = %d: an event list holds at least one event", me, ev_cap);
    if (ev_group < 1) fail("%s: ev_group = %d: a group has at least one utterance", me, ev_group);
    const bool direct_lists = nseg == 1;
    if (direct_lists && seg_cap != ev_cap) fail("%s: seg_cap = %d, but with nseg = 1 the segment lists are the final lists of ev_cap = %d", me, seg_cap, ev_cap);
    if ((stages & 3) == 2 && !direct_lists) fail("%s: stages = %d: %d segment lists need the compaction (1) in front of the raw candidates (2)", me, stages, nseg);
    const bool reports_lists = (stages & 1) && !direct_lists;
    const struct { const void *p; bool needed; const char *name; } bufs[] = {
        {d_seg_events, (stages & 3) != 0, "seg_events"}, {d_seg_count, (stages & 3) != 0, "seg_count"}, {d_events, reports_lists, "events"},
        {d_ev_count, reports_lists, "ev_count"}, {d_raw, (stages & 6) != 0, "raw"}, {d_cand, (stages & 4) != 0, "cand"}, {d_nc, (stages & 4) != 0, "nc"}};
    for (const auto &b : bufs)
      if (b.needed && !b.p) fail("%s: null buffer (%s)", me, b.name);
    HarvestParams p{};
    p.afs = afs; p.f0_floor = f0_floor; p.f0_ceil = f0_ceil; p.nch = nch; p.maxc = maxc;
    p.nseg = nseg; p.seg_cap = seg_cap; p.ev_cap = ev_cap;
    p.fft_seg = direct_lists ? 1 : 0;
    std::vector<int> fb(nfb, nfb + n_utt);
    int max_fb = 0;
    for (int u = 0; u < n_utt; ++u) {
      if (fb[u] < 1) fail("%s: nfb[%d] = %d: an utterance has at least one frame", me, u, fb[u]);
      max_fb = std::max(max_fb, fb[u]);
    }
    plan_harvest_tail(c, p, n_utt, max_fb);
    if (fb_stride != p.fb_stride) fail("%s: fb_stride = %d, the batch's is %d (max nfb rounded up to 8)", me, fb_stride, p.fb_stride);
    const size_t B = n_utt, L = static_cast<size_t>(nch) * 4, row = p.fb_stride;
    p.ev_group = std::min(n_utt, ev_group);
    const size_t E = p.ev_group;
    refuse_overlap(me,
                   {{reports_lists ? d_events : nullptr, sizeof(double) * B * L * ev_cap, "events"},
                    {reports_lists ? d_ev_count : nullptr, sizeof(int) * B * L, "ev_count"},
                    {(stages & 2) ? d_raw : nullptr, sizeof(double) * B * nch * row, "raw"},
                    {(stages & 4) ? d_cand : nullptr, sizeof(double) * B * row * maxc, "cand"}, {(stages & 4) ? d_nc : nullptr, sizeof(int) * B, "nc"}},
                   {{(stages & 3) ? d_seg_events : nullptr, sizeof(double) * B * L * nseg * seg_cap, "seg_events"},
                    {(stages & 3) ? d_seg_count : nullptr, sizeof(int) * B * L * nseg, "seg_count"},
                    {(stages & 6) == 4 ? d_raw : nullptr, sizeof(double) * B * nch * row, "raw"}});
    if (stages & 3) {
      std::vector<int> cnt(B * L * nseg);
      devrt::d2h(cnt.data(), d_seg_count, sizeof(int) * cnt.size(), c->stream);
      devrt::sync(c->stream);
      for (size_t i = 0; i < cnt.size(); ++i)
        if (cnt[i] < 0 || cnt[i] > seg_cap) fail("%s: seg_count[%zu] = %d outside 0 .. seg_cap = %d", me, i, cnt[i], seg_cap);
    }
    begin_stage(c, [&](Arena &a) {
      p.events = a.take<double>(E * L * ev_cap);
      p.ev_count = a.take<int>(E * L);
      if (direct_lists) {
        p.seg_events = p.events; p.seg_count = p.ev_count;
      } else {
        p.seg_events = a.take<double>(E * L * nseg * seg_cap);
        p.seg_count = a.take<int>(E * L * nseg);
      }
    });
    p.b.n_utt = n_utt;
    p.nfb = upload(c, fb);
    p.band_f0 = upload(c, band_f0, static_cast<size_t>(nch));
    p.raw = d_raw; p.cand_a = d_cand; p.nc = d_nc;
    std::vector<int> got;
    if (stages & 3)
      for (int u0 = 0; u0 < n_utt; u0 += p.ev_group) {
        HarvestParams g = p;
        g.ev_u0 = u0;
        const int G = std::min(p.ev_group, n_utt - u0);
        devrt::d2d(p.seg_events, d_seg_events + u0 * L * nseg * seg_cap, sizeof(double) * G * L * nseg * seg_cap, c->stream);
        devrt::d2d(p.seg_count, d_seg_count + u0 * L * nseg, sizeof(int) * G * L * nseg, c->stream);
        launch_harvest_raw(g, G, max_fb, stages & 3, c->stream);
        if (reports_lists) {
          got.resize(G * L);
          devrt::d2h(got.data(), p.ev_count, sizeof(int) * got.size(), c->stream);
          devrt::sync(c->stream);
          for (size_t l = 0; l < got.size(); ++l)
// ... 502 lines not shown
```

### world_amd/csrc/d4c.hip

```cpp
#ifdef D4C_FP_CONTRACT
#pragma clang fp contract(fast)
#endif
#ifndef WH_SWZ
#define WH_SWZ 1
#endif
#include <type_traits>
#include "stage_params.h"
#include "prepare.h"
#include "trace.h"
#include "d4c_select_probe.h"
WH_TRACE_DEFINE(d4c)
WH_BARTRACE_DEFINE(d4c)

namespace world_hip {

constexpr int kHanning = 1, kBlackman = 2;

__global__ void d4c_prepare1(D4cParams p) {
  DYN_LDS(lds);
  if (blockIdx.y == 0) d4c_offsets1_utt(p, blockIdx.x, reinterpret_cast<double *>(lds));
  else d4c_records_utt(p, blockIdx.x, blockIdx.y - 1);
}
__global__ void spectral_prepare(CtParams cp, D4cParams dp) {
  DYN_LDS(lds);
// ... 146 lines not shown
  int j;
  if (a + c3 >= K1) { j = 3; *bucket = c3; }
  else if ((a += c3) + c2 >= K1) { j = 2; *bucket = c2; }
  else if ((a += c2) + c1 >= K1) { j = 1; *bucket = c1; }
  else { j = 0; *bucket = c0; }
  *bin = 4 * l1 + j;
}
__device__ __forceinline__ void sel_zero_bins(int *hist, int tid, int nt) {
  for (int i = tid; i < 336; i += nt) reinterpret_cast<int4 *>(hist)[i] = make_int4(0, 0, 0, 0);
}

template <int NT, int kKeys>
__device__ __forceinline__ bool block_excluding_largest(const unsigned long long (&key)[kKeys], int K, int *hist, double *scratch,
                                                        double *partial, double *total, bool trace_me = false, int threads = NT,
                                                        int *route = nullptr) {
  (void)trace_me;
  constexpr int kFull = kKeys - 2;
  static_assert(NT % WAVE == 0 && NT / WAVE <= 16, "whole wavefronts");
  const int hx = (int)(key[kFull] >> 32);
  const int tid = wg_thread<NT>();
  int hk[kFull];
#pragma unroll
  for (int q = 0; q < kFull; ++q) hk[q] = (int)(key[q] >> 32);
  sel_zero_bins(hist, tid, NT);
  int fl, tp;
  {
    int hm = hx;
#pragma unroll
    for (int q = 0; q < kFull; ++q) hm = hk[q] > hm ? hk[q] : hm;
    sel_floor_top<NT>(hm, reinterpret_cast<int *>(scratch + 48), &fl, &tp);
  }
  WH_STAMP(0, 3);
  bool fast = threads >= K && tp > fl;
  bool t_low_two = false; (void)t_low_two;
  int t_low = 0;
  if (fast) {
    const unsigned range = (unsigned)(tp - fl);
    const int bits = 32 - __builtin_clz(range), s0 = bits > 10 ? bits - 10 : 0;
    auto count0 = [&](int h) __attribute__((always_inline)) {
      const unsigned b = (unsigned)(h - fl) >> s0;
      if (b < 1024u) { atomicAdd(&hist[b], 1); atomicAdd(&hist[1024 + (b >> 4)], 1); }
    };
#pragma unroll
    for (int q = 0; q < kFull; ++q) count0(hk[q]);
    if (tid == 0 && kFull < kKeys) count0(hx);
    __syncthreads();
    int bin0, above0, bucket;
    sel_locate_two_level(hist, K, &bin0, &above0, &bucket);
    t_low = fl + (bin0 << s0);
    WH_STAMP(0, 4);
    if (bucket != 1) {
      if (s0 == 0) {
        fast = false;
      } else {
        const int K1 = K - above0, s1 = s0 > 8 ? s0 - 8 : 0;
        int *h1 = hist + 1088;
        auto count1 = [&](int h) __attribute__((always_inline)) {
          const unsigned d = (unsigned)(h - t_low);
          if (d < (1u << s0)) atomicAdd(&h1[d >> s1], 1);
        };
#pragma unroll
        for (int q = 0; q < kFull; ++q) count1(hk[q]);
        if (tid == 0 && kFull < kKeys) count1(hx);
        __syncthreads();
        int bin1;
        sel_locate_256(h1, K1, &bin1, &bucket);
        t_low += bin1 << s1;
        t_low_two = true;
        if (bucket != 1) fast = false;
        WH_STAMP(0, 5);
      }
    }
  }
#ifdef WH_TRACE
  if (tid == 0) atomicAdd(reinterpret_cast<unsigned long long *>(&wh_trace[!fast ? 102 : (t_low_two ? 101 : 100)]), 1ull);
#endif
  if (route) *route = !fast ? 2 : (t_low_two ? 1 : 0);
  if (!fast) {
    __syncthreads();
    block_smallest_sum<NT>(key, kKeys, NT * kKeys, NT * kKeys - K, hist, scratch, partial, total, trace_me);
    return true;
  }
  double s_lt = 0.0, s_all = 0.0;
#pragma unroll
  for (int q = 0; q < kFull; ++q) {
    const double x = __longlong_as_double((long long)key[q]);
    s_all += x;
    s_lt += hk[q] < t_low ? x : 0.0;
  }
  if (tid == 0 && kFull < kKeys) {
    const double x = __longlong_as_double((long long)key[kFull]);
    s_all += x;
    s_lt += hx < t_low ? x : 0.0;
  }
  WH_STAMP(0, 8);
  *partial = wave_sum(s_lt);
  *total = wave_sum(s_all);
  return false;
}

template <int NMAX, int T> struct D4cShape {
  static constexpr int kItems = (NMAX / 4 + 1 + T - 1) / T;
  static constexpr int kBins = 2 * kItems;
  static constexpr int kLo = NMAX / 2 / T;
};

struct D4cWin {
  const double *x;
  const uint32_t *noise;
  int x_len, hw, wlen, origin, kind;
  double scale;
};
__device__ __forceinline__ D4cWin d4c_win(const double *x, int x_len, int hw, int origin, double scale, int kind,
                                          const uint32_t *noise) {
  D4cWin w;
  w.x = x; w.x_len = x_len; w.noise = noise; w.kind = kind;
  w.hw = hw;
  w.wlen = 2 * w.hw + 1;
  w.origin = origin;
  w.scale = scale;
  return w;
}
struct D4cWinRot { double c, s, dc, ds; };
__device__ __forceinline__ D4cWinRot d4c_win_rot(const D4cWin &w, int i0, double step_s, double step_c) {
  D4cWinRot r;
  sincospi(w.scale * (i0 - w.hw), &r.s, &r.c);
  r.ds = step_s; r.dc = step_c;
  return r;
}
__device__ __forceinline__ double d4c_win_next(const D4cWin &w, D4cWinRot &r) {
  const double c1 = r.c;
  const double v = w.kind == kHanning ? 0.5 * c1 + 0.5 : 0.42 + 0.5 * c1 + 0.08 * (2.0 * c1 * c1 - 1.0);
  r.c = c1 * r.dc - r.s * r.ds;
  r.s = r.s * r.dc + c1 * r.ds;
  return v;
}
struct D4cSample { double v, w; };
__device__ __forceinline__ D4cSample d4c_sample(const D4cWin &w, int i, D4cWinRot &rot) {
  D4cSample s;
  s.w = d4c_win_next(w, rot);
  s.v = w.x[imin(w.x_len - 1, imax(0, w.origin + i - w.hw))] * s.w + randn_value(w.noise[i]) * kSafeGuardD4C;
  return s;
}
template <int NT = 0>
__device__ __forceinline__ double d4c_window_to_lds(const D4cWin &w, const D4cWinRot &rot0, cplx *Z, double *scratch) {
  double s1 = 0.0, s2 = 0.0;
  D4cWinRot rot = rot0;
  block_map<4, D4cSample, NT>(w.wlen, [&](int i) { return d4c_sample(w, i, rot); },
                              [&](int i, D4cSample s) { rfft_in(Z, i) = s.v; s1 += s.v; s2 += s.w; });
  block_sum2<NT>(s1, s2, scratch);
  return s1 / s2;
}

template <int LGN, bool REC>
__device__ __forceinline__ void d4c_love_frame(const D4cParams &p, char *lds) {
  const int u = blockIdx.y, f = blockIdx.x;
  if (f >= p.b.n_frames[u]) return;
  const size_t fi = (size_t)u * p.b.f_stride + f;
  const double f0 = d4c_sane_f0(p.f0[fi], p.b.fs);
  if (f0 == 0.0) { if (threadIdx.x == 0) { p.ap0[fi] = 0.0; p.draws2[fi] = 0u; } return; }
  const int lgn = LGN > 0 ? LGN : p.lg_love, M = 1 << lgn, fs = p.b.fs;
  cplx *Z = reinterpret_cast<cplx *>(lds);
  double *Zr = reinterpret_cast<double *>(lds);
  double *scratch = Zr + M;
  const TwLds tw = stage_twiddles(scratch + 64, lgn - 1, p.tab.tw);
  D4cFrameRec own;
  const D4cFrameRec *rec = &own;
  if constexpr (REC) rec = p.frec + fi;
  else d4c_love_consts(own, f0, p.tpos[fi], fs, blockDim.x);
  auto fld = [](auto *field) __attribute__((always_inline)) {
    if constexpr (REC) return uniform_const_load(field); else return *field;
  };
  const D4cWin w = d4c_win(p.b.x + (size_t)u * p.b.x_stride, p.b.x_len[u], fld(&rec->love_hw), fld(&rec->love_origin), fld(&rec->love_scale),
                           kBlackman, p.noise + p.offsets1[fi]);
  const D4cWinRot rot0 = d4c_win_rot(w, threadIdx.x, fld(&rec->love_step_s), fld(&rec->love_step_c));
  const int b0 = REC ? p.love_b[0] : static_cast<int>(ceil(100.0 * M / fs));
  const int b1 = REC ? p.love_b[1] : static_cast<int>(ceil(4000.0 * M / fs));
  const int b2 = REC ? p.love_b[2] : static_cast<int>(ceil(7900.0 * M / fs));
  double lo = 0.0, hi = 0.0;
  auto band_power = [&](int k, double re, double im) __attribute__((always_inline)) {
    if (k > b0 && k <= b2) {
      const double pw = re * re + im * im;
      hi += pw;
      if (k <= b1) lo += pw;
    }
  };
  if constexpr (LGN > 0 && (1 << LGN) == 16 * 256) {
    constexpr int T = 256, kPer = (1 << LGN) / T, kItems = ((1 << LGN) / 4 + 1 + T - 1) / T;
    const int tid = wg_thread<T>();
    double v[kPer], ww[kPer];
    double s1 = 0.0, s2 = 0.0;
    {
      D4cWinRot rot = rot0;
#pragma unroll
      for (int j = 0; j < kPer; ++j) {
        const int i = tid + j * T;
        v[j] = 0.0; ww[j] = 0.0;
        if (i < w.wlen) { const D4cSample sm = d4c_sample(w, i, rot); v[j] = sm.v; ww[j] = sm.w; s1 += sm.v; s2 += sm.w; }
      }
    }
    block_sum2<T>(s1, s2, scratch);
    const double coef = s1 / s2;
#pragma unroll
    for (int j = 0; j < kPer; ++j) rfft_in(Z, tid + j * T) = v[j] - ww[j] * coef;
    constexpr FftPlan plan = make_plan_max(LGN - 1, 3);
    block_cfft_dif_static<LGN - 1, 3, T>(Z, tw);
    const cplx wb = twiddle(tw, tid, LGN, -1);
    const int h = 1 << (LGN - 1);
    rfft_merge_items_w<kItems, T, true>(Z, LGN, plan, [&](int m, int) { return mul_w16_fwd(wb, m); },
                                  [&](int, int k, double ar, double ai, bool paired, double br, double bi) {
      band_power(k, ar, ai);
      if (paired) band_power(h - k, br, bi);
    });
  } else {
    const double coef = d4c_window_to_lds(w, rot0, Z, scratch);
    {
      D4cWinRot rot = rot0;
      for (int i = threadIdx.x; i < M; i += blockDim.x)
        rfft_in(Z, i) = i < w.wlen ? rfft_in(Z, i) - d4c_win_next(w, rot) * coef : 0.0;
    }
    block_rfft<3, LGN>(Z, lgn, tw, band_power);
  }
  block_sum2<LGN == 11 ? 128 : LGN == 12 ? 256 : 0>(lo, hi, scratch);
  if (threadIdx.x == 0) {
    const double ap0 = lo / hi;
    p.ap0[fi] = ap0;
    const double bf0 = kFloorF0D4C > f0 ? kFloorF0D4C : f0;
    const int body_hw = REC ? fld(&rec->hw) : d4c_win_half(4.0, fs, bf0);
    p.draws2[fi] = ap0 <= p.threshold ? 0u : 3u * (unsigned)(2 * body_hw + 1);
  }
}
template <int LGN, bool REC = true>
__global__ void __launch_bounds__(256) d4c_lovetrain(D4cParams p) {
  DYN_LDS(lds);
  d4c_love_frame<LGN, REC>(p, lds);
}

#ifndef D4C_MIN_WAVES
#define D4C_MIN_WAVES 3
#endif
#if defined(D4C_FENCES)
#define D4C_SCHED_FENCE() __builtin_amdgcn_sched_barrier(0)
#else
#define D4C_SCHED_FENCE() do { } while (0)
#endif
#define D4C_KEY_PAD 0ull
#ifndef D4C_TW_LEVEL
#define D4C_TW_LEVEL 2
#endif
#if !defined(WORLD_SIMT)
#define D4C_FRESH_TID() do { asm volatile("" : "+v"(tid)); __builtin_assume(tid >= 0 && tid < T); } while (0)
#else
#define D4C_FRESH_TID() do { } while (0)
#endif
__host__ __device__ constexpr size_t d4c_frame_direct_tw_offset(int lg) {
  const size_t N = (size_t)1 << lg;
  const size_t park = lg > 13 ? 0 : N / 2 + 2;
  return sizeof(double) * (N + 64 + ((size_t)1 << (lg - D4C_TW_LEVEL - 2)) + 2 + park + 16 * (N / 1024 > 1 ? N / 1024 : 1));
}
template <int NMAX, int T, bool REC = true>
__global__ void __launch_bounds__(T, D4C_MIN_WAVES) d4c_frame(D4cParams p) {
  constexpr int kItems = D4cShape<NMAX, T>::kItems, kBins = D4cShape<NMAX, T>::kBins, kLo = D4cShape<NMAX, T>::kLo;
  constexpr bool kRot = T * 16 == NMAX;
  DYN_LDS(lds);
  const int u = blockIdx.y, f = p.frame_lo + blockIdx.x;
  const size_t fi = (size_t)u * p.b.f_stride + f;
  int tid = wg_thread<T>();
  constexpr int nt = T;
  const int nf_u = p.b.n_frames[u];
  const double f0_in = p.f0[fi], ap0_in = p.ap0[fi];
  const int x_len = p.b.x_len[u];
  const unsigned draws1_u = p.draws1[u];
  constexpr int kCntAhead = 8;
  unsigned cnt_v[kCntAhead];
  {
    const unsigned *cnt = p.draws2 + (size_t)u * p.b.f_stride;
#pragma unroll
    for (int k = 0; k < kCntAhead; ++k) cnt_v[k] = cnt[imin(tid + k * nt, f)];
  }
  if (f >= nf_u || f >= p.frame_hi) return;
  constexpr int kPwAt = T > 8 * WAVE ? 48 : 40;
  const double f0 = d4c_sane_f0(f0_in, p.b.fs);
  if (f0 == 0 || ap0_in <= p.threshold) return;
  const bool trace_me = f == WH_TRACE_FRAME && u == WH_TRACE_UTT; (void)trace_me;
  wh_bartrace_arm(trace_me);
  WH_STAMP(32, 0);
  constexpr int lgn = const_log2(NMAX);
  const int N = 1 << lgn, H = N / 2, q = H / 2, fs = p.b.fs;
  cplx *Z = reinterpret_cast<cplx *>(lds);
  double *Zr = reinterpret_cast<double *>(lds);
  double *scratch = Zr + N;
  const TwLds tw = stage_direct_twiddles<T>(stage_twiddles<T>(scratch + 64, lgn - D4C_TW_LEVEL, p.tab.tw),
                                            reinterpret_cast<cplx *>(lds + d4c_frame_direct_tw_offset(lgn)),
                                            lgn - 1 - 3, 1 << (lgn - 1 - 6), lgn - 1 - 6, 1 << (lgn - 1 - 9));
  constexpr FftPlan plan = make_plan_max(lgn - 1, 3);
  auto cfft = [&]() __attribute__((always_inline)) { block_cfft_dif_static<lgn - 1, 3, T>(Z, tw); };
  const cplx wb = twiddle(tw, tid, lgn, -1);
  auto for_nat = [&](auto body) __attribute__((always_inline)) {
#pragma unroll
    for (int m = 0; m < kItems; ++m) {
      const int it = tid + m * nt;
      if (it <= q) { body(2 * m, it); if (it < q) body(2 * m + 1, H - it); }
      D4C_SCHED_FENCE();
    }
  };
  auto for_pair = [&](auto body) __attribute__((always_inline)) {
#pragma unroll
    for (int m = 0; m < kItems; ++m) {
      const int it = tid + m * nt;
      if (it <= q) { body(2 * m, 2 * it); if (it < q) body(2 * m + 1, 2 * it + 1); }
      D4C_SCHED_FENCE();
    }
  };

  const double *x = p.b.x + (size_t)u * p.b.x_stride;
  D4cFrameRec own;
  const D4cFrameRec *rec = &own;
  if constexpr (REC) rec = p.frec + fi;
  else d4c_body_consts(own, f0, p.tpos[fi], fs, N, nt);
  auto fld = [](auto *field) __attribute__((always_inline)) {
    if constexpr (REC) return uniform_const_load(field); else return *field;
  };
  unsigned stream_at;
  {
    const unsigned *cnt = p.draws2 + (size_t)u * p.b.f_stride;
    unsigned su = 0;
#pragma unroll
    for (int k = 0; k < kCntAhead; ++k) su += tid + k * nt < f ? cnt_v[k] : 0u;
    for (int g = tid + kCntAhead * nt; g < f; g += nt) su += cnt[g];
    int s_ = wave_sum_int((int)su);
    int *part = reinterpret_cast<int *>(Zr);
    if (lane_id() == 0) part[wave_in_block()] = s_;
    __syncthreads();
    int tot_ = 0;
    for (int wv = 0; wv < wg_waves<T>(); ++wv) tot_ += part[wv];
    tot_ = __builtin_amdgcn_readfirstlane(tot_);
    stream_at = draws1_u + (unsigned)tot_;
  }
  const uint32_t *noise = p.noise + stream_at;
  const int wdraws = 2 * fld(&rec->hw) + 1;
  const bool park_global = lgn > 13;
  double *const after_tw = scratch + 64 + twiddle_lds_doubles(lgn - D4C_TW_LEVEL);
  double *park = park_global ? p.park_ws + ((size_t)blockIdx.y * gridDim.x + blockIdx.x) * (size_t)(H + 2) : after_tw;
  const double inv_n = 1.0 / N;

  auto dc_correct = [&](double (&S)[kBins], auto for_own) __attribute__((always_inline)) {
    const int upper = fld(&rec->upper), nrep = upper - 1;
    __syncthreads();
    for_own([&](int slot, int k) { if (k <= upper) Zr[k] = S[slot]; });
    __syncthreads();
    const int b0 = fld(&rec->b0);
    const double fr0 = fld(&rec->fr0);
    for_own([&](int slot, int k) {
      if (k < nrep) {
        const int b = b0 - k;
        const double y0 = Zr[b], y1 = Zr[b + 1 <= upper ? b + 1 : upper];
        S[slot] = keep(S[slot] + (y0 + (y1 - y0) * fr0));
      }
    });
    __syncthreads();
  };
  auto smooth = [&](const double (&in)[kBins], auto for_in, const D4cSmoothConsts *sc, double (&out)[kBins], auto for_out, const bool pre = true) __attribute__((always_inline)) {
    const int bnd = fld(&sc->bnd);
    const int seg_len = H + 2 * bnd + 1;
    if (pre) __syncthreads();
    for_in([&](int slot, int k) {
      const double v = in[slot] * fs * inv_n;
      Zr[k + bnd] = v;
      if (k >= 1 && k <= bnd) Zr[bnd - k] = v;
      if (k < H && k >= H - bnd) Zr[2 * H + bnd - k] = v;
    });
    block_scan_incl_double<T>(Zr, seg_len, scratch);
    const double inv_width = fld(&sc->inv_width);
    const int i_lo = fld(&sc->i_lo), i_hi = fld(&sc->i_hi);
    const double f_lo = fld(&sc->f_lo), f_hi = fld(&sc->f_hi);
    const double *z_lo = Zr + i_lo, *z_hi = Zr + i_hi;
    for_out([&](int slot, int k) {
      const double l0 = z_lo[k], l1 = z_lo[k + 1], h0 = z_hi[k], h1 = z_hi[k + 1];
      const double lo = l0 + (l1 - l0) * f_lo, hi = h0 + (h1 - h0) * f_hi;
      out[slot] = keep((hi - lo) * inv_width);
    });
    (void)seg_len;
  };

  const D4cWinRot rot0 = d4c_win_rot(d4c_win(x, x_len, fld(&rec->hw), fld(&rec->origin[2]), fld(&rec->scale), kHanning, noise), tid,
                                     fld(&rec->step_s), fld(&rec->step_c));

  auto for_hi = [&](const D4cWin &w, double coef, auto body) __attribute__((always_inline)) {
    if (w.wlen > H) {
      D4cWinRot rot = rot0;
#pragma unroll 1
      for (int i = tid; i < H; i += nt) d4c_win_next(w, rot);
      for (int i = H + tid; i < w.wlen; i += nt) {
        const D4cSample s = d4c_sample(w, i, rot);
        body(i, s.v - s.w * coef);
      }
    }
  };
  auto hi_samples = [&](const D4cWin &w, double coef, auto body) __attribute__((always_inline)) {
    if (w.wlen > H) {
      D4cWinRot rot = rot0;
#pragma unroll 1
      for (int i = tid; i < H; i += nt) d4c_win_next(w, rot);
#pragma unroll
      for (int k = 0; k < kLo; ++k) {
        const int i = H + tid + k * nt;
        if (i < w.wlen) {
          const D4cSample sm = d4c_sample(w, i, rot);
          body(k, i, sm.v - sm.w * coef);
        }
      }
    }
  };
  auto balanced = [&](const D4cWin &w, double (&ulo)[kLo]) __attribute__((always_inline)) {
    double wlo[kLo];
    double s1 = 0.0, s2 = 0.0;
    D4cWinRot rot = rot0;
    double xv[kLo];
    uint32_t nz[kLo];
#pragma unroll
    for (int j = 0; j < kLo; ++j) {
      const int i = imin(tid + j * nt, w.wlen - 1);
      xv[j] = w.x[imin(w.x_len - 1, imax(0, w.origin + i - w.hw))];
      nz[j] = w.noise[i];
    }
#pragma unroll
    for (int j = 0; j < kLo; ++j) { xv[j] = keep(xv[j]); nz[j] = keep_word(nz[j]); }
#pragma unroll
    for (int j = 0; j < kLo; ++j) {
      const int i = tid + j * nt;
      ulo[j] = 0.0; wlo[j] = 0.0;
      if (i < w.wlen && i < H) {
        const double ww = d4c_win_next(w, rot);
        const double v = xv[j] * ww + randn_value(nz[j]) * kSafeGuardD4C;
        ulo[j] = v; wlo[j] = ww; s1 += v; s2 += ww;
      }
    }
    for (int i = H + tid; i < w.wlen; i += nt) { const D4cSample s = d4c_sample(w, i, rot); s1 += s.v; s2 += s.w; }
    block_sum2<T, false>(s1, s2, scratch);
    const double coef = s1 / s2;
#pragma unroll
    for (int j = 0; j < kLo; ++j) ulo[j] = ulo[j] - wlo[j] * coef;
    return coef;
  };

  static_assert(kLo == 8 && T * 8 * 2 == NMAX, "one radix-8 butterfly per thread");
  auto cfft_from_registers = [&](cplx (&a)[8], const cplx &w1) __attribute__((always_inline)) {
    constexpr int sh = lgn - 1 - 3;
    dft_reg<true, 3>(a);
    mul_powers<3>(a, w1);
    const int s0 = swz(tid);
#pragma unroll
    for (int k = 0; k < 8; ++k) Z[s0 ^ swz(k << sh)] = a[k];
    DifStages<lgn - 1, 3, lgn - 1 - 3, T>::run(Z, tw);
    __syncthreads();
  };

#pragma unroll 1
  for (int c = 0; c < 2; ++c) {
    const D4cWin w = d4c_win(x, x_len, fld(&rec->hw), fld(&rec->origin[c]), fld(&rec->scale), kBlackman, noise + (size_t)c * wdraws);
    D4C_FRESH_TID();
    double ulo[kLo];
    const double coef = balanced(w, ulo);
    WH_STAMP(32, 1 + 4 * c);
    double pw = 0.0;
    {
      cplx a[8];
#pragma unroll
      for (int j = 0; j < 8; ++j) {
        a[j].re = ulo[j]; a[j].im = ulo[j] * (tid + j * nt + 1.0);
        pw += ulo[j] * ulo[j];
      }
      hi_samples(w, coef, [&](int k, int i, double uh) { a[k].re += uh; a[k].im += uh * (i + 1.0); pw += uh * uh; });
      pw = wave_sum(pw);
      if (lane_id() == 0) scratch[kPwAt + wave_in_block()] = pw;
      cfft_from_registers(a, twiddle(tw, tid, lgn - 1, -1));
    }
    pw = 0.0;
    for (int wv = 0; wv < wg_waves<T>(); ++wv) pw += scratch[kPwAt + wv];
    const double half_inv_pw = 0.5 / pw;
#pragma unroll
    for (int m = 0; m < kItems; ++m) {
      const int it = tid + m * nt;
      if (it <= q) {
        const cplx P = Z[fft_slot(plan, it)], Q = Z[fft_slot(plan, (H - it) & (H - 1))];
        const double v = (P.im * Q.re + Q.im * P.re) * half_inv_pw;
        park[2 * it] = c == 0 ? v : park[2 * it] + v;
      }
    }
    WH_STAMP(32, 2 + 4 * c);
    __syncthreads();
    D4C_FRESH_TID();
    {
      cplx a[8];
#pragma unroll
      for (int j = 0; j < 8; ++j) { a[j].re = ulo[j]; a[j].im = ulo[j] * (tid + j * nt + 1.0); }
      hi_samples(w, coef, [&](int k, int i, double uh) { a[k].re -= uh; a[k].im -= uh * (i + 1.0); });
#pragma unroll
      for (int j = 0; j < 8; ++j) a[j] = cmul(a[j], kRot ? mul_w16_fwd(wb, j) : twiddle(tw, tid + j * nt, lgn, -1));
      WH_STAMP(32, 3 + 4 * c);
      cfft_from_registers(a, twiddle(tw, tid, lgn - 1, -1));
    }
#pragma unroll
    for (int m = 0; m < kItems; ++m) {
      const int it = tid + m * nt;
      if (it < q) {
        const cplx P = Z[fft_slot(plan, it)], Q = Z[fft_slot(plan, H - 1 - it)];
        const double v = (P.im * Q.re + Q.im * P.re) * half_inv_pw;
        park[2 * it + 1] = c == 0 ? v : park[2 * it + 1] + v;
      }
    }
    WH_STAMP(32, 4 + 4 * c);
    __syncthreads();
  }
  WH_STAMP(32, 9);
  D4C_FRESH_TID();
  lds_dead(Zr, N);

  double B[kBins];
  {
    const D4cWin w = d4c_win(x, x_len, fld(&rec->hw), fld(&rec->origin[2]), fld(&rec->scale), kHanning, noise + (size_t)2 * wdraws);
    double ulo[kLo];
    const double coef = balanced(w, ulo);
#pragma unroll
    for (int j = 0; j < kLo; ++j) {
      const int n = tid + j * nt;
      if (n < H) rfft_in(Z, n) = ulo[j];
    }
    for (int i = H + tid; i < N; i += nt) rfft_in(Z, i) = 0.0;
    for_hi(w, coef, [&](int i, double uh) { rfft_in(Z, i) = uh; });
    WH_STAMP(32, 10);
    cfft();
    double Bn[kBins];
    rfft_merge_items_rot<kItems, T>(Z, lgn, plan, tw, wb, [&](int m, int, double ar, double ai, bool, double br, double bi) {
      Bn[2 * m] = keep(ar * ar + ai * ai); Bn[2 * m + 1] = keep(br * br + bi * bi);
    });
    WH_STAMP(32, 11);
    D4C_FRESH_TID();
    if (fld(&rec->upper) < WAVE) {
      const int upper = fld(&rec->upper), nrep = upper - 1;
      const int b0 = fld(&rec->b0);
      const double fr0 = fld(&rec->fr0);
      if (wave_in_block() == 0) {
        const int b = b0 - lane_id();
        const double y0 = __shfl(Bn[0], b & (WAVE - 1), WAVE), y1 = __shfl(Bn[0], (b + 1 <= upper ? b + 1 : upper) & (WAVE - 1), WAVE);
        if (lane_id() < nrep) Bn[0] = keep(Bn[0] + (y0 + (y1 - y0) * fr0));
      }
    } else
    dc_correct(Bn, for_nat);
    smooth(Bn, for_nat, &rec->sm[0], B, for_pair, false);
  }
  WH_STAMP(32, 12);
  lds_dead(Zr, N);

  double A[kBins];
  {
    const int upper = fld(&rec->upper), nrep = upper - 1;
    const int b0 = fld(&rec->b0);
    const double fr0 = fld(&rec->fr0);
    for_pair([&](int slot, int k) {
      double v = park[k];
      if (k < nrep) {
        const int b = b0 - k;
        const double y0 = park[b], y1 = park[b + 1 <= upper ? b + 1 : upper];
        v = v + (y0 + (y1 - y0) * fr0);
      }
      A[slot] = keep(v);
    });
  }
  WH_STAMP(32, 13);
  D4C_FRESH_TID();
#pragma unroll
  for (int e = 0; e < kBins; ++e) A[e] = fast_div(A[e], B[e]);
  D4C_FRESH_TID();
  smooth(A, for_pair, &rec->sm[1], A, for_pair);
  WH_STAMP(32, 14);
  D4C_FRESH_TID();
  smooth(A, for_pair, &rec->sm[0], B, for_pair);
  for_pair([&](int slot, int k) { park[k] = A[slot] - B[slot]; });
  WH_STAMP(32, 15);

  const int bnd = REC ? p.band_bnd : mround(N * 8.0 / p.wl);
  const int hwl = p.wl / 2, wl = 2 * hwl + 1;
  const int nz = hwl + 1;
  int mine = 0;
  for_nat([&](int, int) { ++mine; });
  int *hist = reinterpret_cast<int *>(Zr);
  constexpr int kWaves = (T + WAVE - 1) / WAVE;
  double *band_sums = park_global ? after_tw : park + (H + 2);
  const double nut0 = 2 * tid < wl ? p.nuttall[2 * tid] : 0.0, nut1 = 2 * tid + 1 < wl ? p.nuttall[2 * tid + 1] : 0.0;
  constexpr int kNzR = (512 + T - 1) / T;
  const cplx w_first = twiddle(tw, tid, plan.lg, -1);
  const bool second = kNzR == 2 && tid + T < nz;
  double nut2 = 0.0, nut3 = 0.0;
  if (second) { nut2 = p.nuttall[2 * (tid + T)]; nut3 = 2 * (tid + T) + 1 < wl ? p.nuttall[2 * (tid + T) + 1] : 0.0; }
  const bool any_second = kNzR == 2 && __builtin_amdgcn_ballot_w64(second) != 0ull;
  for (int band = 0; band < p.nap; ++band) {
    const int lo_k = p.band_center[band] - hwl;
    D4C_FRESH_TID();
    __syncthreads();
    auto slice = [&](int n) {
      cplx v;
      const double *g = park + lo_k + 2 * n;
      if (n == tid) {
        v.re = g[0] * nut0;
        v.im = 2 * n + 1 < wl ? g[1] * nut1 : 0.0;
      } else {
        v.re = g[0] * p.nuttall[2 * n];
        v.im = 2 * n + 1 < wl ? g[1] * p.nuttall[2 * n + 1] : 0.0;
      }
      return v;
    };
    {
      constexpr int R = 8;
      const int sh = plan.lg - 3, qq = 1 << sh;
      const int s0 = swz(tid);
      cplx z0; z0.re = 0.0; z0.im = 0.0;
      if constexpr (kNzR <= 2) {
        const cplx a0 = (kNzR == 2 || tid < nz) ? slice(tid) : z0;
        cplx a[R];
        if (any_second) {
          cplx a1 = z0;
          if (second) {
            const double *g = park + lo_k + 2 * (tid + T);
            a1.re = g[0] * nut2;
            a1.im = 2 * (tid + T) + 1 < wl ? g[1] * nut3 : 0.0;
          }
          dft8_head2<true>(a0, a1, a);
          if (!second) {
#pragma unroll
            for (int r = 0; r < R; ++r) a[r] = a0;
          }
          mul_powers<3>(a, w_first);
#pragma unroll
          for (int k = 0; k < R; ++k) Z[s0 ^ swz(k << sh)] = a[k];
        } else {
#pragma unroll
          for (int r = 0; r < R; ++r) a[r] = a0;
          mul_powers<3>(a, w_first);
#pragma unroll
          for (int k = 0; k < R; ++k) Z[s0 ^ swz(k << sh)] = a[k];
        }
      } else {
        cplx a[R];
        const bool single = tid + qq >= nz;
#pragma unroll
        for (int r = 0; r < R; ++r) a[r] = (r < kNzR && tid + r * qq < nz) ? slice(tid + r * qq) : z0;
        if (single) {
#pragma unroll
          for (int r = 1; r < R; ++r) a[r] = a[0];
        } else {
          dft_reg<true, 3>(a);
        }
        mul_powers<3>(a, w_first);
#pragma unroll
        for (int k = 0; k < R; ++k) Z[s0 ^ swz(k << sh)] = a[k];
      }
      DifStages<lgn - 1, 3, lgn - 1 - 3, T>::run(Z, tw);
      __syncthreads();
    }
    if (band == 0) WH_STAMP(32, 16);
    unsigned long long key[kBins];
#pragma unroll
    for (int e = 0; e < kBins; ++e) key[e] = D4C_KEY_PAD;
    rfft_merge_items_rot<kItems, T, true>(Z, lgn, plan, tw, wb, [&](int m, int, double ar, double ai, bool paired, double br, double bi) {
      key[2 * m] = (unsigned long long)__double_as_longlong(ar * ar + ai * ai);
      if (paired) key[2 * m + 1] = (unsigned long long)__double_as_longlong(br * br + bi * bi);
    });
    if (band == 0) WH_STAMP(32, 17);
    lds_dead(Zr, N);
    double part, tot;
    (void)mine;
    const bool whole = block_excluding_largest<T>(key, bnd + 1, hist, scratch, &part, &tot, trace_me, N / 16);
    if (lane_id() == 0) {
      const int wv = wave_in_block();
      band_sums[(2 * band) * kWaves + wv] = whole && wv > 0 ? 0.0 : part;
      band_sums[(2 * band + 1) * kWaves + wv] = whole && wv > 0 ? 0.0 : tot;
    }
    if (band == 0) WH_STAMP(32, 18);
  }
  __syncthreads();
  for (int b = tid; b < 2 * p.nap; b += nt) {
    const int band = b < p.nap ? b : b - p.nap, which = b < p.nap ? 0 : 1;
    const double *w = band_sums + (2 * band + which) * kWaves;
    double t = 0.0;
#pragma unroll
    for (int k = 0; k < kWaves; ++k) t += w[k];
    p.coarse[fi * 16 + (which ? 9 : 1) + band] = t;
  }
  WH_STAMP(32, 19);
}

__global__ void d4c_finish(D4cParams p) {
  const int u = blockIdx.y, f = p.frame_lo + blockIdx.x;
  if (f >= p.b.n_frames[u] || f >= p.frame_hi) return;
  const size_t fi = (size_t)u * p.b.f_stride + f;
  const int tid = threadIdx.x, nt = blockDim.x, fs = p.b.fs;
  const int nb_out = p.fft_out / 2 + 1;
  const size_t orow = p.out_row ? (size_t)p.out_row[u] + f : fi;
  char *row_at = reinterpret_cast<char *>(p.aperiodicity + orow * p.out_stride) + p.out_col_bytes;
  double *row = reinterpret_cast<double *>(row_at);
  float *row32 = reinterpret_cast<float *>(row_at);
  const double f0 = d4c_sane_f0(p.f0[fi], p.b.fs);
  if (p.rec && tid == 0) { double *r = p.rec + orow * p.out_stride; r[0] = p.tpos[fi]; r[1] = p.f0[fi]; }
  auto code_bands = [&](auto ap_value) __attribute__((always_inline)) {
    for (int band = tid; band < p.code_nap; band += nt) {
      const double pos = (3000.0 * (band + 1.0) - 0) / (static_cast<double>(fs) / p.fft_out);
      const int b = static_cast<int>(pos);
      const double fr = pos - b;
      const double y0 = 20 * log10(ap_value(b));
      const double dy = b < nb_out - 1 ? 20 * log10(ap_value(b + 1)) - y0 : 0.0;
      row[band] = y0 + dy * fr;
    }
  };
  if (f0 == 0 || p.ap0[fi] <= p.threshold) {
    if (p.code_nap > 0) { code_bands([&](int) { return 1.0 - kTiny; }); return; }
    if (p.out_f32) { for (int i = tid; i < nb_out; i += nt) row32[i] = static_cast<float>(1.0 - kTiny); }
    else { for (int i = tid; i < nb_out; i += nt) row[i] = 1.0 - kTiny; }
    return;
  }
  DYN_LDS(lds);
  double *coarse_db = reinterpret_cast<double *>(lds);
  for (int b = tid; b < p.nap; b += nt) {
    const double cf0 = kFloorF0D4C > f0 ? kFloorF0D4C : f0;
    double c = 10 * log10(p.coarse[fi * 16 + 1 + b] / p.coarse[fi * 16 + 9 + b]);
    c = c + (cf0 - 100) / 50.0;
    coarse_db[1 + b] = c < 0.0 ? c : 0.0;
  }
  __syncthreads();
  const double *coarse_in = coarse_db;
  const int nk = p.nap + 2;
  (void)nk;
  auto ap_value = [&](int i) __attribute__((always_inline)) {
    const int k = p.ap_knot[i];
    const double s = p.ap_frac[i];
    auto cval = [&](int j) { return j == 0 ? -60.0 : (j == p.nap + 1 ? -kTiny : coarse_in[j]); };
    double y = cval(k - 1) + s * (cval(k) - cval(k - 1));
    return exp10(y / 20.0);
  };
  if (p.code_nap > 0) { code_bands(ap_value); return; }
  for (int i = tid; i < nb_out; i += nt) {
    const double v = ap_value(i);
    if (p.out_f32) row32[i] = static_cast<float>(v); else row[i] = v;
  }
}

template <int NT>
__global__ void __launch_bounds__(NT) d4c_select_probe(const double *keys, double *out, int K, int mode) {
  constexpr int kKeys = 10, N = 16 * NT, kWaves = NT / WAVE;
  static_assert(D4cShape<N, NT>::kBins == kKeys, "d4c_frame's keys per thread");
  DYN_LDS(lds);
  double *Zr = reinterpret_cast<double *>(lds);
  double *scratch = Zr + N;
  double *band_sums = scratch + 64;
  int *hist = reinterpret_cast<int *>(Zr);
  const int tid = wg_thread<NT>();
  const double *mine = keys + ((size_t)blockIdx.x * NT + tid) * kKeys;
  unsigned long long key[kKeys];
#pragma unroll
  for (int e = 0; e < kKeys; ++e) key[e] = (unsigned long long)__double_as_longlong(mine[e]);
  lds_dead(Zr, N);
  double part, tot;
  int route = 2;
  bool whole = true;
  if (mode == 0) whole = block_excluding_largest<NT>(key, K, hist, scratch, &part, &tot, false, NT, &route);
  else block_smallest_sum<NT>(key, kKeys, NT * kKeys, NT * kKeys - K, hist, scratch, &part, &tot, false);
  if (K == NT * kKeys) part = 0.0;
  if (lane_id() == 0) {
    const int wv = wave_in_block();
    band_sums[wv] = whole && wv > 0 ? 0.0 : part;
    band_sums[kWaves + wv] = whole && wv > 0 ? 0.0 : tot;
  }
  __syncthreads();
  if (tid < 2) {
    const double *w = band_sums + tid * kWaves;
    double t = 0.0;
#pragma unroll
    for (int k = 0; k < kWaves; ++k) t += w[k];
    out[(size_t)blockIdx.x * 3 + tid] = t;
  }
  if (tid == 2) out[(size_t)blockIdx.x * 3 + 2] = (double)route;
}
static size_t d4c_select_probe_lds_bytes(int threads) { return sizeof(double) * ((size_t)16 * threads + 64 + 2 * (threads / WAVE)); }
bool launch_d4c_select_probe(int mode, int threads, int K, long rows, const double *d_keys, double *d_out, hipStream_t stream) {
  const dim3 grid((unsigned)rows);
  const size_t lds = d4c_select_probe_lds_bytes(threads);
  if (threads == 128) WH_BLOCKS(d4c_select_probe<128>, grid, 128, lds, stream, d_keys, d_out, K, mode);
  else if (threads == 256) WH_BLOCKS(d4c_select_probe<256>, grid, 256, lds, stream, d_keys, d_out, K, mode);
  else if (threads == 512) WH_BLOCKS(d4c_select_probe<512>, grid, 512, lds, stream, d_keys, d_out, K, mode);
  else if (threads == 1024) WH_BLOCKS(d4c_select_probe<1024>, grid, 1024, lds, stream, d_keys, d_out, K, mode);
  else return false;
  return true;
}

size_t d4c_love_lds_bytes(int lg) { return sizeof(double) * (size_t)((1 << lg) + 64 + (1 << lg) / 8 + 2); }
size_t d4c_frame_lds_bytes(int lg) {
  return d4c_frame_direct_tw_offset(lg) + 2 * sizeof(double) * (((size_t)1 << (lg - 7)) + ((size_t)1 << (lg - 10)));
}
size_t d4c_park_slot_doubles(int lg) { return lg > 13 ? ((size_t)1 << (lg - 1)) + 2 : 0; }
int d4c_frame_threads(int lg) { return (1 << lg) / 16; }
int d4c_love_threads(int lg) { return lg <= 11 ? 128 : 256; }
size_t d4c_max_draws_per_frame(int fs) {
  return (size_t)(2 * mround(3.0 * fs / 40.0 / 2.0) + 1) + 3 * (size_t)(2 * mround(4.0 * fs / kFloorF0D4C / 2.0) + 1);
}

void launch_spectral_prepare(const CtParams &cp, const D4cParams &dp, int max_frames, hipStream_t stream) {
  WH_BLOCKS(spectral_prepare, dim3(cp.b.n_utt, 2, 1 + rec_chunks(max_frames)), 256, 64 * sizeof(double), stream, cp, dp);
}

void launch_d4c(const D4cParams &p, int max_frames, hipStream_t stream) {
  if (!(p.skip_prepare & kD4cSkipScan)) WH_BLOCKS(d4c_prepare1, dim3(p.b.n_utt, 1 + rec_chunks(max_frames)), 1024, 64 * sizeof(double), stream, p);
  if (!(p.skip_prepare & kD4cSkipLoveTrain) && max_frames > 0) {
    const dim3 love_grid(max_frames, p.b.n_utt);
    const size_t love_lds = d4c_love_lds_bytes(p.lg_love);
    const int love_nt = d4c_love_threads(p.lg_love);
    auto love = [&](auto rec) {
      constexpr bool R = decltype(rec)::value;
      if (p.lg_love == 11) devrt::launch_blocks("d4c_lovetrain", d4c_lovetrain<11, R>, love_grid, love_nt, love_lds, stream, p);
      else if (p.lg_love == 12) devrt::launch_blocks("d4c_lovetrain", d4c_lovetrain<12, R>, love_grid, love_nt, love_lds, stream, p);
      else devrt::launch_blocks("d4c_lovetrain", d4c_lovetrain<0, R>, love_grid, love_nt, love_lds, stream, p);
    };
    if (p.frame_consts) love(std::true_type()); else love(std::false_type());
  }
  const int range_frames = imin(max_frames, p.frame_hi) - p.frame_lo;
  if (range_frames <= 0) return;
  const size_t lds = d4c_frame_lds_bytes(p.lg_d4c);
  const int per_launch = p.lg_d4c > 13 ? imax(1, p.park_slots / p.b.n_utt) : range_frames;
  for (int lo = 0; lo < range_frames; lo += per_launch) {
    D4cParams q = p;
    q.frame_lo = p.frame_lo + lo;
    q.frame_hi = imin(q.frame_lo + per_launch, p.frame_lo + range_frames);
    const dim3 grid(q.frame_hi - q.frame_lo, p.b.n_utt);
    auto frame = [&](auto rec) {
      constexpr bool R = decltype(rec)::value;
      if (p.lg_d4c == 11) devrt::launch_blocks("d4c_frame", d4c_frame<2048, 128, R>, grid, 128, lds, stream, q);
      else if (p.lg_d4c == 12) devrt::launch_blocks("d4c_frame", d4c_frame<4096, 256, R>, grid, 256, lds, stream, q);
      else if (p.lg_d4c == 13) devrt::launch_blocks("d4c_frame", d4c_frame<8192, 512, R>, grid, 512, lds, stream, q);
      else devrt::launch_blocks("d4c_frame", d4c_frame<16384, 1024, R>, grid, 1024, lds, stream, q);
    };
    if (p.frame_consts) frame(std::true_type()); else frame(std::false_type());
  }
  WH_BLOCKS(d4c_finish, dim3(range_frames, p.b.n_utt), 256, 8 * sizeof(double), stream, p);
}

}
```

### world_amd/csrc/devrt.h

```cpp
#pragma once

#include <cmath>
#include <cstddef>
#include <cstdint>
#include <cstdio>
#include <cstdlib>
#include <cstring>
#include <stdexcept>

#ifdef WORLD_EMU
struct dim3 {
  unsigned x, y, z;
  dim3(unsigned x_ = 1, unsigned y_ = 1, unsigned z_ = 1) : x(x_), y(y_), z(z_) {}
};
struct double2 { double x, y; };
struct uint4 { uint32_t x, y, z, w; };
static inline double2 make_double2(double a, double b) { double2 r; r.x = a; r.y = b; return r; }
static inline uint4 make_uint4(uint32_t a, uint32_t b, uint32_t c, uint32_t d) { uint4 r = {a, b, c, d}; return r; }
extern thread_local dim3 threadIdx, blockIdx, blockDim, gridDim;
extern thread_local char *emu_lds_base;
#define __global__
#define __device__
#define __host__
#define __forceinline__ inline
// ... 461 lines not shown
  const auto l = __builtin_amdgcn_permlane32_swap(lo, lo, false, false);
  const auto h = __builtin_amdgcn_permlane32_swap(hi, hi, false, false);
  return __hiloint2double(h[0], l[0]) + __hiloint2double(h[1], l[1]);
}
#endif
__device__ __forceinline__ double wave_pick(double v, int src_lane) {
#ifndef WORLD_EMU
  return readlane_f64(v, __builtin_amdgcn_readfirstlane(src_lane));
#else
  (void)src_lane;
  return v;
#endif
}
__device__ __forceinline__ double wave_bcast(double v, int src_lane) {
#ifndef WORLD_EMU
  return __shfl(v, src_lane, 64);
#else
  (void)src_lane;
  return v;
#endif
}
__device__ __forceinline__ int wave_bcast_int(int v, int src_lane) {
#ifndef WORLD_EMU
  return __shfl(v, src_lane, 64);
#else
  (void)src_lane;
  return v;
#endif
}

template <int NT = 0, bool PRE = true> __device__ __forceinline__ double block_sum(double v, double *scratch) {
#ifndef WORLD_EMU
  v = wave_sum(v);
  int nw = wg_waves<NT>();
  if (nw == 1) return v;
  if (PRE) __syncthreads();
  if (lane_id() == 0) scratch[wave_in_block()] = v;
  __syncthreads();
  double t = 0.0;
  for (int w = 0; w < nw; ++w) t += scratch[w];
  return t;
#else
  (void)scratch;
  return v;
#endif
}
template <int NT = 0, bool PRE = true> __device__ __forceinline__ void block_sum2(double &a, double &b, double *scratch) {
#ifndef WORLD_EMU
  a = wave_sum(a); b = wave_sum(b);
  int nw = wg_waves<NT>();
  if (nw == 1) return;
  if (PRE) __syncthreads();
  if (lane_id() == 0) { scratch[wave_in_block()] = a; scratch[32 + wave_in_block()] = b; }
  __syncthreads();
  double ta = 0.0, tb = 0.0;
  for (int w = 0; w < nw; ++w) { ta += scratch[w]; tb += scratch[32 + w]; }
  a = ta; b = tb;
#else
  (void)scratch;
#endif
}
template <int NT = 0, bool PRE = true> __device__ __forceinline__ void block_sum3(double &a, double &b, double &c, double *scratch) {
#ifndef WORLD_EMU
  a = wave_sum(a); b = wave_sum(b); c = wave_sum(c);
  int nw = wg_waves<NT>();
  if (nw == 1) return;
  if (PRE) __syncthreads();
  if (lane_id() == 0) { scratch[wave_in_block()] = a; scratch[16 + wave_in_block()] = b; scratch[32 + wave_in_block()] = c; }
  __syncthreads();
  double ta = 0.0, tb = 0.0, tc = 0.0;
  for (int w = 0; w < nw; ++w) { ta += scratch[w]; tb += scratch[16 + w]; tc += scratch[32 + w]; }
  a = ta; b = tb; c = tc;
#else
  (void)scratch;
#endif
}
template <int NT = 0> __device__ __forceinline__ void block_sum4(double &a, double &b, double &c, double &d, double *scratch) {
#ifndef WORLD_EMU
  a = wave_sum(a); b = wave_sum(b); c = wave_sum(c); d = wave_sum(d);
  int nw = wg_waves<NT>();
  if (nw == 1) return;
  __syncthreads();
  if (lane_id() == 0) {
    double *s = scratch + 4 * wave_in_block();
    s[0] = a; s[1] = b; s[2] = c; s[3] = d;
  }
  __syncthreads();
  double ta = 0.0, tb = 0.0, tc = 0.0, td = 0.0;
  for (int w = 0; w < nw; ++w) { ta += scratch[4 * w]; tb += scratch[4 * w + 1]; tc += scratch[4 * w + 2]; td += scratch[4 * w + 3]; }
  a = ta; b = tb; c = tc; d = td;
#else
  (void)scratch;
#endif
}
template <int K, class T, int NT = 0, class Produce, class Consume>
__device__ __forceinline__ void block_map(int n, Produce produce, Consume consume) {
  const int tid = wg_thread<NT>(), nt = wg_size<NT>();
  for (int base = tid; base < n; base += K * nt) {
    T v[K];
#pragma unroll
    for (int q = 0; q < K; ++q) { const int i = base + q * nt; if (i < n) v[q] = produce(i); }
#pragma unroll
    for (int q = 0; q < K; ++q) { const int i = base + q * nt; if (i < n) consume(i, v[q]); }
  }
}

__device__ __forceinline__ int block_excl_scan_int(int v, int *total, double *scratch) {
#ifndef WORLD_EMU
  int wt, off = wave_excl_scan_int(v, &wt);
  int nw = waves_per_block();
  if (nw == 1) { *total = wt; return off; }
  int *is = reinterpret_cast<int *>(scratch);
  __syncthreads();
  if (lane_id() == 0) is[wave_in_block()] = wt;
  __syncthreads();
  int base = 0, tot = 0;
  for (int w = 0; w < nw; ++w) { int c = is[w]; if (w < wave_in_block()) base += c; tot += c; }
  *total = tot;
  return base + off;
#else
  (void)scratch;
  *total = v;
  return 0;
#endif
}

template <bool PRE = true>
__device__ __forceinline__ unsigned long long block_excl_scan_u64(unsigned long long v, unsigned long long *total,
                                                                  double *scratch) {
#ifndef WORLD_EMU
  const int lane = lane_id();
  const unsigned lo = (unsigned)wave_incl_scan_int((int)(unsigned)v), hi = (unsigned)wave_incl_scan_int((int)(unsigned)(v >> 32));
  const unsigned long long inc = ((unsigned long long)hi << 32) | lo;
  const unsigned long long wt = ((unsigned long long)(unsigned)__builtin_amdgcn_readlane((int)hi, 63) << 32) |
                                (unsigned)__builtin_amdgcn_readlane((int)lo, 63);
  const int nw = waves_per_block();
  if (nw == 1) { *total = wt; return inc - v; }
  unsigned long long *us = reinterpret_cast<unsigned long long *>(scratch);
  if (PRE) __syncthreads();
  if (lane == 0) us[wave_in_block()] = wt;
  __syncthreads();
  unsigned long long base = 0, tot = 0;
  for (int w = 0; w < nw; ++w) { unsigned long long c = us[w]; if (w < wave_in_block()) base += c; tot += c; }
  *total = tot;
  return base + (inc - v);
#else
  (void)scratch;
  *total = v;
  return 0;
#endif
}

template <int NT = 0>
__device__ __forceinline__ void block_scan_incl_double(double *a, int n, double *scratch) {
  int nt = wg_size<NT>(), tid = wg_thread<NT>();
  int chunk = (n + nt - 1) / nt;
  int lo = tid * chunk, hi = lo + chunk < n ? lo + chunk : n;
  __syncthreads();
#ifndef WORLD_EMU
  constexpr int kRegChunk = 12;
  if (chunk <= kRegChunk) {
    double v[kRegChunk];
#pragma unroll
    for (int q = 0; q < kRegChunk; ++q) v[q] = lo + q < hi ? a[lo + q] : 0.0;
#pragma unroll
    for (int q = 1; q < kRegChunk; ++q) v[q] += v[q - 1];
    const double s = v[kRegChunk - 1];
    const int lane = lane_id(), w = wave_in_block();
    const double inc = wave_incl_scan_f64(s);
    if (lane == 63) scratch[w] = inc;
    __syncthreads();
    double base = 0.0;
    for (int k = 0; k < w; ++k) base += scratch[k];
    const double off = base + (inc - s);
#pragma unroll
    for (int q = 0; q < kRegChunk; ++q) if (lo + q < hi) a[lo + q] = v[q] + off;
    __syncthreads();
    return;
  }
#endif
  double s = 0.0;
  for (int i = lo; i < hi; ++i) { s += a[i]; a[i] = s; }
#ifndef WORLD_EMU
  int lane = lane_id();
  const double inc = wave_incl_scan_f64(s);
  int nw = waves_per_block(), w = wave_in_block();
  if (lane == 63) scratch[w] = inc;
  __syncthreads();
  double base = 0.0;
  for (int k = 0; k < w; ++k) base += scratch[k];
  double off = base + (inc - s);
  (void)nw;
  for (int i = lo; i < hi; ++i) a[i] += off;
#else
  (void)scratch;
#endif
  __syncthreads();
}
```

### world_amd/csrc/fft.h

```cpp
#pragma once
#include "devrt.h"
#include "tables.h"

#ifndef WH_SWZ
#define WH_SWZ 0
#endif
#define WH_FFT_NS2(n) fft_swz##n
#define WH_FFT_NS(n) WH_FFT_NS2(n)
namespace world_hip {
inline namespace WH_FFT_NS(WH_SWZ) {

struct cplx { double re, im; };

__device__ __forceinline__ cplx cmul(cplx a, cplx b) {
  cplx r; r.re = fma(a.re, b.re, -(a.im * b.im)); r.im = fma(a.re, b.im, a.im * b.re); return r;
}
__device__ __forceinline__ cplx cadd(cplx a, cplx b) { cplx r; r.re = a.re + b.re; r.im = a.im + b.im; return r; }
__device__ __forceinline__ cplx csub(cplx a, cplx b) { cplx r; r.re = a.re - b.re; r.im = a.im - b.im; return r; }
__device__ __forceinline__ cplx cconj(cplx a) { a.im = -a.im; return a; }
struct TwLds {
  const double *q; int lg;
  double fine_c, fine_s;
  double fine2_c, fine2_s;
  const cplx *dir_a = nullptr, *dir_b = nullptr;
// ... 365 lines not shown
template <int LG, int MAXLR, int LEV, int NT = 0> struct DifStages {
  static __device__ __forceinline__ void run(cplx *z, const TwLds &tw) {
    constexpr int LR = LEV >= MAXLR ? MAXLR : LEV;
    constexpr bool local = FftWaveLocal<LG, MAXLR, NT>::dif_local(LEV);
    if constexpr (local) wave_sync(); else __syncthreads();
    if constexpr (FftWaveLocal<LG, MAXLR, NT>::one_per_thread && LR < MAXLR) dif_stage<LR, NT, MAXLR - LR>(z, LG, LEV, tw);
    else dif_stage<LR, NT>(z, LG, LEV, tw);
    if constexpr (LEV - LR > 0) DifStages<LG, MAXLR, LEV - LR, NT>::run(z, tw);
  }
};
template <int LG, int MAXLR, int NT = 0>
__device__ __forceinline__ void block_cfft_dif_static(cplx *z, const TwLds &tw) {
  DifStages<LG, MAXLR, LG, NT>::run(z, tw);
  __syncthreads();
}
template <int LG, int MAXLR, class Src>
__device__ __forceinline__ void block_cfft_dif_from_static(cplx *z, const TwLds &tw, Src src) {
  constexpr int LR = LG >= MAXLR ? MAXLR : LG;
  __syncthreads();
  dif_first_stage<LR>(z, LG, tw, src);
  if constexpr (LG - LR > 0) DifStages<LG, MAXLR, LG - LR>::run(z, tw);
  __syncthreads();
}
template <int LG, int MAXLR, int DONE, int NT = 0> struct DitStages {
  template <class Epi> static __device__ __forceinline__ void run(cplx *z, const TwLds &tw, Epi epi) {
    constexpr int LR = (DONE == 0 && LG % MAXLR != 0) ? LG % MAXLR : MAXLR;
    constexpr bool local = FftWaveLocal<LG, MAXLR, NT>::dit_local(DONE, LR);
    constexpr bool last = DONE + LR >= LG;
    if constexpr (local) wave_sync(); else __syncthreads();
    if constexpr (last) {
      if constexpr (FftWaveLocal<LG, MAXLR, NT>::one_per_thread && LR < MAXLR) dit_stage<LR, NT, MAXLR - LR, Epi>(z, LG, DONE, tw, epi);
      else dit_stage<LR, NT, -1, Epi>(z, LG, DONE, tw, epi);
    } else {
      if constexpr (FftWaveLocal<LG, MAXLR, NT>::one_per_thread && LR < MAXLR) dit_stage<LR, NT, MAXLR - LR>(z, LG, DONE, tw);
      else dit_stage<LR, NT>(z, LG, DONE, tw);
      DitStages<LG, MAXLR, DONE + LR, NT>::run(z, tw, epi);
    }
  }
};
template <int LG, int MAXLR, int NT = 0, class Epi = FftNoEpilogue>
__device__ __forceinline__ void block_cfft_dit_static(cplx *z, const TwLds &tw, Epi epi = Epi()) {
  DitStages<LG, MAXLR, 0, NT>::run(z, tw, epi);
  __syncthreads();
}

template <int MAXLR = 4>
__device__ __forceinline__ void block_cfft_dit(cplx *z, const FftPlan &p, const TwLds &tw) {
  int done = 0;
  for (int s = p.ns - 1; s >= 0; --s) {
    __syncthreads();
    switch (p.rl(s)) {
      case 4: if (MAXLR >= 4) dit_stage<4>(z, p.lg, done, tw); break;
      case 3: if (MAXLR >= 3) dit_stage<3>(z, p.lg, done, tw); break;
      case 2: dit_stage<2>(z, p.lg, done, tw); break;
      default: dit_stage<1>(z, p.lg, done, tw); break;
    }
    done += p.rl(s);
  }
  __syncthreads();
}

__device__ __forceinline__ double &rfft_in(cplx *z, int n) {
  cplx &c = z[swz(n >> 1)];
  return (n & 1) ? c.im : c.re;
}
template <class Emit>
__device__ __forceinline__ void rfft_merge(cplx *z, int lgn, const FftPlan &plan, const TwLds &tw, Emit emit);

template <int MAXLR = 4, int LGN = 0, class Emit>
__device__ __forceinline__ void block_rfft(cplx *z, int lgn, const TwLds &tw, Emit emit) {
  if constexpr (LGN > 0) {
    constexpr FftPlan plan = make_plan_max(LGN - 1, MAXLR);
    block_cfft_dif_static<LGN - 1, MAXLR>(z, tw);
    rfft_merge(z, LGN, plan, tw, emit);
  } else {
    const FftPlan plan = make_plan_max(lgn - 1, MAXLR);
    block_cfft_dif<MAXLR>(z, plan, tw);
    rfft_merge(z, lgn, plan, tw, emit);
  }
}
template <int MAXLR = 4, int LGN = 0, class Src, class Emit>
__device__ __forceinline__ void block_rfft_from(cplx *z, int lgn, const TwLds &tw, Src src, Emit emit) {
  if constexpr (LGN > 0) {
    constexpr FftPlan plan = make_plan_max(LGN - 1, MAXLR);
    block_cfft_dif_from_static<LGN - 1, MAXLR>(z, tw, src);
    rfft_merge(z, LGN, plan, tw, emit);
  } else {
    const FftPlan plan = make_plan_max(lgn - 1, MAXLR);
    block_cfft_dif_from<MAXLR>(z, plan, tw, src);
    rfft_merge(z, lgn, plan, tw, emit);
  }
}
template <class Emit>
__device__ __forceinline__ void rfft_merge(cplx *z, int lgn, const FftPlan &plan, const TwLds &tw, Emit emit) {
  const int lgh = lgn - 1, h = 1 << lgh, q = h >> 1;
  const int top_bit = plan.rl(plan.ns - 1) - 1;
  struct Pair { int k; double ar, ai, br, bi; };
  auto item = [&](int it) {
      Pair r;
      if (it < q) {
        const int pos = ((it >> top_bit) << (top_bit + 1)) | (it & ((1 << top_bit) - 1));
        const int slot = swz(pos);
        const int k = fft_bin_of_slot(plan, slot);
        const cplx za = z[slot];
        r.k = k;
        if (k == 0) {
          r.ar = za.re + za.im; r.ai = 0.0; r.br = za.re - za.im; r.bi = 0.0;
        } else {
          const cplx zb = z[fft_slot(plan, h - k)];
          cplx e, o;
          e.re = 0.5 * (za.re + zb.re); e.im = 0.5 * (za.im - zb.im);
          o.re = 0.5 * (za.im + zb.im); o.im = -0.5 * (za.re - zb.re);
          const cplx ow = cmul(o, twiddle(tw, k, lgn, -1));
          r.ar = e.re + ow.re; r.ai = e.im + ow.im; r.br = e.re - ow.re; r.bi = ow.im - e.im;
        }
      } else {
        const cplx za = z[fft_slot(plan, q)];
        r.k = q; r.ar = za.re; r.ai = -za.im; r.br = 0.0; r.bi = 0.0;
      }
      return r;
    };
  auto out = [&](int, Pair r) {
      emit(r.k, r.ar, r.ai);
      if (r.k != q) emit(h - r.k, r.br, r.bi);
    };
  const bool odd_one = (int)threadIdx.x == (int)blockDim.x - 1;
  Pair last;
  if (odd_one) last = item(q);
  block_map<2, Pair>(q, item, out);
  if (odd_one) out(q, last);
  __syncthreads();
}

__device__ __forceinline__ cplx mul_w16_fwd(cplx a, int m) {
  switch (m & 15) {
    case 0: return a;
    case 1: return mul_w16<true, 1>(a);
    case 2: return mul_w16<true, 2>(a);
    case 3: return mul_w16<true, 3>(a);
    case 4: return mul_w16<true, 4>(a);
    case 5: return mul_w16<true, 5>(a);
    case 6: return mul_w16<true, 6>(a);
    case 7: return mul_w16<true, 7>(a);
    case 8: return mul_w16<true, 8>(a);
    case 9: return mul_w16<true, 9>(a);
    case 10: return mul_w16<true, 10>(a);
    case 11: return mul_w16<true, 11>(a);
    case 12: return mul_w16<true, 12>(a);
    case 13: return mul_w16<true, 13>(a);
    case 14: return mul_w16<true, 14>(a);
    default: return mul_w16<true, 15>(a);
  }
}
template <int KITEMS, int NT, bool TWICE = false, class Wk, class Emit>
__device__ __forceinline__ void rfft_merge_items_w(cplx *z, int lgn, const FftPlan &plan, Wk wk, Emit emit) {
  const int lgh = lgn - 1, h = 1 << lgh, q = h >> 1;
  const int tid = wg_thread<NT>(), nt = wg_size<NT>();
#pragma unroll
  for (int m = 0; m < KITEMS; ++m) {
    const int k = tid + m * nt;
    if (k == 0) {
      const cplx za = z[fft_slot(plan, 0)];
      const double a = za.re + za.im, b = za.re - za.im;
      if (TWICE) emit(m, 0, a + a, 0.0, true, b + b, 0.0);
      else emit(m, 0, a, 0.0, true, b, 0.0);
    } else if (k < q) {
      const cplx za = z[fft_slot(plan, k)], zb = z[fft_slot(plan, h - k)];
      cplx e, o;
      if (TWICE) {
        e.re = za.re + zb.re; e.im = za.im - zb.im;
        o.re = za.im + zb.im; o.im = zb.re - za.re;
      } else {
        e.re = 0.5 * (za.re + zb.re); e.im = 0.5 * (za.im - zb.im);
        o.re = 0.5 * (za.im + zb.im); o.im = -0.5 * (za.re - zb.re);
      }
      const cplx ow = cmul(o, wk(m, k));
      emit(m, k, e.re + ow.re, e.im + ow.im, true, e.re - ow.re, ow.im - e.im);
    } else if (k == q) {
      const cplx za = z[fft_slot(plan, q)];
      if (TWICE) emit(m, q, za.re + za.re, -(za.im + za.im), false, 0.0, 0.0);
      else emit(m, q, za.re, -za.im, false, 0.0, 0.0);
    }
#ifndef WORLD_EMU
    if (m & 1) __builtin_amdgcn_sched_barrier(0);
#endif
  }
  __syncthreads();
}
template <int KITEMS, int NT = 0, class Emit>
__device__ __forceinline__ void rfft_merge_items(cplx *z, int lgn, const FftPlan &plan, const TwLds &tw, Emit emit) {
  rfft_merge_items_w<KITEMS, NT>(z, lgn, plan, [&](int, int k) { return twiddle(tw, k, lgn, -1); }, emit);
}
template <int KITEMS, int NT, bool TWICE = false, class Emit>
__device__ __forceinline__ void rfft_merge_items_rot(cplx *z, int lgn, const FftPlan &plan, const TwLds &tw, cplx wbase, Emit emit) {
  rfft_merge_items_w<KITEMS, NT, TWICE>(z, lgn, plan, [&](int m, int k) {
    if (NT * 16 == (1 << lgn)) return mul_w16_fwd(wbase, m);
    return twiddle(tw, k, lgn, -1);
  }, emit);
}

template <class Spec>
__device__ __forceinline__ void irfft_pretwiddle(cplx *z, int lgn, const FftPlan &plan, const TwLds &tw, Spec spec) {
  const int lgh = lgn - 1, h = 1 << lgh;
  __syncthreads();
  const int q = h >> 1, top_bit = plan.rl(plan.ns - 1) - 1;
  struct Pair { int slot, mslot; cplx r, rm; };
  auto item = [&](int it) {
      Pair o;
      o.mslot = -1;
      if (it < q) {
        const int pos = ((it >> top_bit) << (top_bit + 1)) | (it & ((1 << top_bit) - 1));
        o.slot = swz(pos);
        const int k = fft_bin_of_slot(plan, o.slot);
        cplx x = spec(k), y = spec(h - k);
        if (k == 0) {
          o.r.re = x.re + y.re; o.r.im = x.re - y.re;
        } else {
          y.im = -y.im;
          const cplx s = cadd(x, y), d = csub(x, y);
          const cplx t = cmul(d, twiddle(tw, k, lgn, +1));
          o.r.re = s.re - t.im; o.r.im = s.im + t.re;
          o.rm.re = s.re + t.im; o.rm.im = t.re - s.im;
          o.mslot = fft_slot(plan, h - k);
        }
      } else {
        const cplx x = spec(q);
        o.slot = fft_slot(plan, q);
        o.r.re = 2.0 * x.re; o.r.im = -2.0 * x.im;
      }
      return o;
    };
  auto out = [&](int, Pair o) {
      z[o.slot] = o.r;
      if (o.mslot >= 0) z[o.mslot] = o.rm;
    };
  const bool odd_one = (int)threadIdx.x == (int)blockDim.x - 1;
  Pair last;
  if (odd_one) last = item(q);
  block_map<2, Pair>(q, item, out);
  if (odd_one) out(q, last);
}
template <int KITEMS, int NT = 0, class Spec>
__device__ __forceinline__ void irfft_pretwiddle_items(cplx *z, int lgn, const FftPlan &plan, const TwLds &tw, Spec spec) {
  const int lgh = lgn - 1, h = 1 << lgh, q = h >> 1;
  const int tid = wg_thread<NT>(), nt = wg_size<NT>();
  __syncthreads();
#pragma unroll
  for (int m = 0; m < KITEMS; ++m) {
    const int k = tid + m * nt;
    if (k == 0) {
      const cplx x = spec(0), y = spec(h);
      cplx r; r.re = x.re + y.re; r.im = x.re - y.re;
      z[fft_slot(plan, 0)] = r;
    } else if (k < q) {
      cplx x = spec(k), y = spec(h - k);
      y.im = -y.im;
      const cplx s = cadd(x, y), d = csub(x, y);
      const cplx t = cmul(d, twiddle(tw, k, lgn, +1));
      cplx r, rm;
      r.re = s.re - t.im; r.im = s.im + t.re;
      rm.re = s.re + t.im; rm.im = t.re - s.im;
      z[fft_slot(plan, k)] = r;
      z[fft_slot(plan, h - k)] = rm;
    } else if (k == q) {
      const cplx x = spec(q);
      cplx r; r.re = 2.0 * x.re; r.im = -2.0 * x.im;
      z[fft_slot(plan, q)] = r;
    }
  }
}
template <int KITEMS, int NT, class Pair>
__device__ __forceinline__ void irfft_pretwiddle_items_w(cplx *z, int lgn, const FftPlan &plan, Pair pair) {
  const int lgh = lgn - 1, h = 1 << lgh, q = h >> 1;
  const int tid = wg_thread<NT>(), nt = wg_size<NT>();
  __syncthreads();
#pragma unroll
  for (int m = 0; m < KITEMS; ++m) {
    const int k = tid + m * nt;
    cplx x, y, w;
    if (k <= q) pair(m, k, x, y, w);
    if (k == 0) {
      cplx r; r.re = x.re + y.re; r.im = x.re - y.re;
      z[fft_slot(plan, 0)] = r;
    } else if (k < q) {
      y.im = -y.im;
      const cplx s = cadd(x, y), d = csub(x, y);
      const cplx t = cmul(d, w);
      cplx r, rm;
      r.re = s.re - t.im; r.im = s.im + t.re;
      rm.re = s.re + t.im; rm.im = t.re - s.im;
      z[fft_slot(plan, k)] = r;
      z[fft_slot(plan, h - k)] = rm;
    } else if (k == q) {
      cplx r; r.re = 2.0 * x.re; r.im = -2.0 * x.im;
      z[fft_slot(plan, q)] = r;
    }
  }
}
template <int MAXLR = 4, int LGN = 0, class Spec>
__device__ __forceinline__ void block_irfft(cplx *z, int lgn, const TwLds &tw, Spec spec) {
  if constexpr (LGN > 0) {
    constexpr FftPlan plan = make_plan_max(LGN - 1, MAXLR);
    irfft_pretwiddle(z, LGN, plan, tw, spec);
    block_cfft_dit_static<LGN - 1, MAXLR>(z, tw);
  } else {
    const FftPlan plan = make_plan_max(lgn - 1, MAXLR);
    irfft_pretwiddle(z, lgn, plan, tw, spec);
    block_cfft_dit<MAXLR>(z, plan, tw);
  }
}

}
}
```

### world_amd/csrc/prepare.h

```cpp
#pragma once
#include "stage_params.h"

namespace world_hip {

__device__ __forceinline__ double ct_effective_f0(double f0, double floor_f0, int fs) {
  const double nyq = 0.5 * fs;
  return !(f0 > floor_f0) ? kDefaultF0 : (f0 > nyq ? nyq : f0);
}
__device__ __forceinline__ double d4c_sane_f0(double f0, int fs) {
  const double nyq = 0.5 * fs;
  return f0 != f0 ? 0.0 : (f0 > nyq ? nyq : f0);
}


struct CtSmooth { double width; int bnd, seg_len; };
__device__ __forceinline__ CtSmooth ct_smooth_shape(double cf0, int N, int fs) {
  CtSmooth s;
  s.width = cf0 * 2.0 / 3.0;
  s.bnd = static_cast<int>(s.width * N / fs) + 1;
  s.seg_len = N / 2 + 2 * s.bnd + 1;
  return s;
}
__device__ __forceinline__ int ct_win_half(int fs, double cf0) { return mround(1.5 * fs / cf0); }
__device__ __forceinline__ CtFrameRec ct_frame_consts(double cf0, double pos, int fs, int N, int nt) {
  CtFrameRec r;
  r.cf0 = cf0;
  r.hw = ct_win_half(fs, cf0);
  r.origin = mround(pos * fs + 0.001);
  r.win_scale = 1.0 / 1.5 / fs * cf0;
  sincospi(r.win_scale * nt, &r.step_s, &r.step_c);
  r.upper = 2 + static_cast<int>(cf0 * N / fs);
  const CtSmooth sm = ct_smooth_shape(cf0, N, fs);
  r.width = sm.width;
  r.bnd = sm.bnd;
  r.origin_axis = -(sm.bnd - 0.5) * fs / N;
  r.f0_over_fs = cf0 / fs;
  return r;
}

__device__ __forceinline__ int d4c_win_half(double ratio, int fs, double f0) { return mround(ratio * fs / f0 / 2.0); }
__device__ __forceinline__ int d4c_win_origin(double pos, int fs) { return mround(pos * fs + 0.001); }
__device__ __forceinline__ double d4c_win_scale(double ratio, int fs, double f0) { return 2.0 / ratio / fs * f0; }
__device__ __forceinline__ D4cSmoothConsts d4c_smooth_consts(double width, int N, int fs) {
  D4cSmoothConsts s;
  s.bnd = static_cast<int>(width * N / fs) + 1;
  const double origin_axis = -(s.bnd - 0.5) * fs / N;
  const double inv_step = static_cast<double>(N) / fs;
  s.inv_width = 1.0 / width;
  const double c_lo = (0.0 - width / 2.0 - origin_axis) * inv_step, c_hi = (width / 2.0 - origin_axis) * inv_step;
  s.i_lo = static_cast<int>(c_lo); s.i_hi = static_cast<int>(c_hi);
  s.f_lo = c_lo - s.i_lo; s.f_hi = c_hi - s.i_hi;
  s.pad_ = 0;
  return s;
}
__device__ __forceinline__ void d4c_love_consts(D4cFrameRec &r, double f0, double pos, int fs, int nt) {
  const double cf0 = f0 > 40.0 ? f0 : 40.0;
  r.love_hw = d4c_win_half(3.0, fs, cf0);
  r.love_origin = d4c_win_origin(pos, fs);
  r.love_scale = d4c_win_scale(3.0, fs, cf0);
  sincospi(r.love_scale * nt, &r.love_step_s, &r.love_step_c);
}
__device__ __forceinline__ void d4c_body_consts(D4cFrameRec &r, double f0, double pos, int fs, int N, int nt) {
  const double cf0 = kFloorF0D4C > f0 ? kFloorF0D4C : f0;
  r.hw = d4c_win_half(4.0, fs, cf0);
  r.scale = d4c_win_scale(4.0, fs, cf0);
  sincospi(r.scale * nt, &r.step_s, &r.step_c);
  r.origin[0] = d4c_win_origin(pos - 0.25 / cf0, fs);
  r.origin[1] = d4c_win_origin(pos + 0.25 / cf0, fs);
  r.origin[2] = d4c_win_origin(pos, fs);
  r.upper = 2 + static_cast<int>(cf0 * N / fs);
  const double pos0 = (0.0 - cf0) * (-static_cast<double>(N) / fs);
  r.b0 = static_cast<int>(pos0);
  r.fr0 = pos0 - r.b0;
  r.sm[0] = d4c_smooth_consts(cf0, N, fs);
  r.sm[1] = d4c_smooth_consts(cf0 / 2.0, N, fs);
}

constexpr int kRecSpan = 256;
__device__ __forceinline__ void ct_records_utt(const CtParams &p, int u, int chunk) {
  const int nf = p.b.n_frames[u], hi = imin(nf, (chunk + 1) * kRecSpan);
  for (int f = chunk * kRecSpan + threadIdx.x; f < hi; f += blockDim.x) {
    const size_t fi = (size_t)u * p.b.f_stride + f;
    p.frec[fi] = ct_frame_consts(ct_effective_f0(p.f0[fi], p.f0_floor, p.b.fs), p.tpos[fi], p.b.fs, 1 << p.lg_fft, p.frame_threads);
  }
}
__device__ __forceinline__ void d4c_records_utt(const D4cParams &p, int u, int chunk) {
  const int nf = p.b.n_frames[u], hi = imin(nf, (chunk + 1) * kRecSpan);
  for (int f = chunk * kRecSpan + threadIdx.x; f < hi; f += blockDim.x) {
    const size_t fi = (size_t)u * p.b.f_stride + f;
    const double f0f = d4c_sane_f0(p.f0[fi], p.b.fs);
    if (f0f == 0.0) continue;
    const double pos = p.tpos[fi];
    D4cFrameRec r;
    d4c_love_consts(r, f0f, pos, p.b.fs, p.love_threads);
    d4c_body_consts(r, f0f, pos, p.b.fs, 1 << p.lg_d4c, p.frame_threads);
    p.frec[fi] = r;
  }
}
__host__ __device__ __forceinline__ int rec_chunks(int max_frames) { return (max_frames + kRecSpan - 1) / kRecSpan; }

__device__ __forceinline__ void ct_offsets_utt(const CtParams &p, int u, double *scratch) {
  const int nf = p.b.n_frames[u];
  const int N = 1 << p.lg_fft, nb = N / 2 + 1;
  const double *f0 = p.f0 + (size_t)u * p.b.f_stride;
  unsigned *off_out = p.offsets + (size_t)u * p.b.f_stride;
  unsigned running = 0;
  for (int base = 0; base < nf; base += blockDim.x) {
    int f = base + threadIdx.x;
    int cnt = 0;
    if (f < nf) {
      double cf0 = ct_effective_f0(f0[f], p.f0_floor, p.b.fs);
      cnt = 2 * ct_win_half(p.b.fs, cf0) + 1 + nb;
    }
    int total, off = block_excl_scan_int(cnt, &total, scratch);
    if (f < nf) off_out[f] = running + (unsigned)off;
    running += (unsigned)total;
  }
}

__device__ __forceinline__ void d4c_offsets1_utt(const D4cParams &p, int u, double *scratch) {
  const int nf = p.b.n_frames[u];
  const double *f0 = p.f0 + (size_t)u * p.b.f_stride;
  unsigned *off_out = p.offsets1 + (size_t)u * p.b.f_stride;
  unsigned running = 0;
  for (int base = 0; base < nf; base += blockDim.x) {
    int f = base + threadIdx.x, cnt = 0;
    const double f0f = f < nf ? d4c_sane_f0(f0[f], p.b.fs) : 0.0;
    if (f < nf && f0f != 0.0) {
      double cf0 = f0f > 40.0 ? f0f : 40.0;
      cnt = 2 * d4c_win_half(3.0, p.b.fs, cf0) + 1;
    }
    int total, off = block_excl_scan_int(cnt, &total, scratch);
    if (f < nf) off_out[f] = running + (unsigned)off;
    running += (unsigned)total;
  }
  if (threadIdx.x == 0) p.draws1[u] = running;
}

}
```

### world_amd/csrc/stage_params.h

```cpp
#pragma once
#include "common.h"

namespace world_hip {

template <class T> __device__ __forceinline__ T uniform_const_load(const T *p) {
#if !defined(WORLD_EMU) && !defined(WORLD_SIMT)
  static_assert(std::is_arithmetic<T>::value, "scalars only");
  return *(const __attribute__((address_space(4))) T *)p;
#else
  return *p;
#endif
}
struct CtFrameRec {
  double cf0;
  double win_scale;
  double step_s, step_c;
  double width;
  double origin_axis;
  double f0_over_fs;
  int hw, origin;
  int upper, bnd;
};
struct D4cSmoothConsts {
  double f_lo, f_hi, inv_width;
  int bnd, i_lo, i_hi, pad_;
};
struct D4cFrameRec {
  double love_scale, love_step_s, love_step_c;
  int love_hw, love_origin;
  double scale, step_s, step_c, fr0;
  int hw, origin[3];
  int upper, b0;
  D4cSmoothConsts sm[2];
};

struct CtParams {
  BatchView b;
  const double *tpos;
  const double *f0;
  double *spectrogram;
  const int *out_row;
  size_t out_stride;
  size_t out_col_bytes;
  int out_f32;
  unsigned *offsets;
  CtFrameRec *frec;
  int frame_consts;
  int frame_threads;
  double lift0;
  const uint32_t *noise;
  Tables tab;
  double q1;
  double f0_floor;
  int lg_fft;
  int frame_lo, frame_hi;
  int skip_prepare;
  int code_ndim;
  const int *code_knot;
  const double *code_frac, *code_w_re, *code_w_im;
};

struct D4cParams {
  BatchView b;
  const double *tpos;
  const double *f0;
  double *aperiodicity;
  const int *out_row;
  size_t out_stride;
  size_t out_col_bytes;
  int out_f32;
  double *rec;
  double *ap0;
  double *coarse;
  unsigned *offsets1;
  unsigned *draws2;
  unsigned *draws1;
  D4cFrameRec *frec;
  int frame_consts;
  int love_threads, frame_threads;
  int love_b[3];
  int band_bnd;
  const uint32_t *noise;
  const double *nuttall;
  double *park_ws;
  int park_slots;
  Tables tab;
  double threshold;
  int fft_out;
  int lg_love;
  int lg_d4c;
  int nap;
  int wl;
  const double *ap_frac;
  const int *ap_knot;
  int code_nap;
  int band_center[8];
  int frame_lo, frame_hi;
  int skip_prepare;
};
constexpr int kD4cSkipScan = 1, kD4cSkipLoveTrain = 2;

void launch_cheaptrick(const CtParams &p, int max_frames, hipStream_t stream);
void launch_d4c(const D4cParams &p, int max_frames, hipStream_t stream);
void launch_spectral_prepare(const CtParams &cp, const D4cParams &dp, int max_frames, hipStream_t stream);
size_t ct_max_draws_per_frame(int fft_size);
size_t d4c_max_draws_per_frame(int fs);
size_t d4c_park_slot_doubles(int lg_d4c);
int ct_frame_threads(int lg_fft);
int d4c_love_threads(int lg_love);
int d4c_frame_threads(int lg_d4c);

}
```

Before: 4.441 million frames/s.

## Skip D4C spectral bins above the last aperiodicity band and precompute draw offsets

```diff
diff --git a/include/world_hip.h b/include/world_hip.h
--- a/include/world_hip.h
+++ b/include/world_hip.h
@@ -234,6 +234,7 @@
                                       long long batch, const void *d_in, void *d_out);
 WORLD_HIP_API int world_hip_probe_select(WorldHipContext *ctx, int mode, int threads, int K, long long rows,
                                          const double *d_keys, double *d_out);
+WORLD_HIP_API int world_hip_d4c_last_bins(int fs, double f0, int *out);
 WORLD_HIP_API int world_hip_probe_harvest_contour(WorldHipContext *ctx, int n_utt, const int *nfb, const int *nc, int maxc,
                                                   int fb_stride, const double *d_cand, const double *d_score, double frame_period,
                                                   int f_stride, double *d_pruned_cand, double *d_pruned_score, double *d_step2,
diff --git a/world_amd/api.py b/world_amd/api.py
--- a/world_amd/api.py
+++ b/world_amd/api.py
@@ -266,6 +266,8 @@
         lib.world_hip_probe_fft.argtypes = [vp, C.c_int, C.c_int, C.c_int, C.c_int, C.c_int, C.c_longlong, vp, vp]
     if hasattr(lib, "world_hip_probe_select"):
         lib.world_hip_probe_select.argtypes = [vp, C.c_int, C.c_int, C.c_int, C.c_longlong, vp, vp]
+    if hasattr(lib, "world_hip_d4c_last_bins"):
+        lib.world_hip_d4c_last_bins.argtypes = [C.c_int, C.c_double, _ip]
     if hasattr(lib, "world_hip_probe_harvest_contour"):
         lib.world_hip_probe_harvest_contour.argtypes = [vp, C.c_int, _ip, _ip, C.c_int, C.c_int, vp, vp, C.c_double, C.c_int,
                                                         vp, vp, vp, vp, vp, C.c_int, vp, vp, vp, vp, vp]
diff --git a/world_amd/csrc/api.hip b/world_amd/csrc/api.hip
--- a/world_amd/csrc/api.hip
+++ b/world_amd/csrc/api.hip
@@ -447,6 +447,8 @@
   p.offsets1 = a.take<unsigned>(fr);
   p.draws2 = a.take<unsigned>(fr);
   p.draws1 = a.take<unsigned>(p.b.n_utt);
+  p.offsets2 = a.take<unsigned>(fr);
+  p.tickets = a.take<unsigned>(p.b.n_utt);
   p.frec = a.take<D4cFrameRec>(fr);
   p.coarse = a.take<double>(fr * 16);
   const size_t slot = d4c_park_slot_doubles(p.lg_d4c);
@@ -483,6 +485,7 @@
   if (!lim.empty()) fail("%s", lim.c_str());
 }
 static bool inkernel_consts() { return getenv("WORLD_HIP_INKERNEL_CONSTS") != nullptr; }
+static bool d4c_all_bins() { return getenv("WORLD_HIP_D4C_ALL_BINS") != nullptr; }
 static CtParams setup_cheaptrick(WorldHipContext *c, int n_utt, int fs, const double *d_x, int x_stride,
                                  const int *x_length, const int *n_frames, int f_stride, const double *d_tpos,
                                  const double *d_f0, const CheapTrickOption *opt, double *d_sp, const RowLayout &lay,
@@ -604,6 +607,8 @@
   p.love_b[1] = static_cast<int>(ceil(4000.0 * fft_love / fs));
   p.love_b[2] = static_cast<int>(ceil(7900.0 * fft_love / fs));
   p.band_bnd = mround(fft_d4c * 8.0 / wl);
+  p.band_last = p.band_center[nap - 1] + wl / 2;
+  p.all_bins = d4c_all_bins() ? 1 : 0;
   if (lay.frame_lo < 0 || lay.frame_hi < lay.frame_lo) fail("bad frame range [%d, %d)", lay.frame_lo, lay.frame_hi);
   p.frame_lo = lay.frame_lo; p.frame_hi = lay.frame_hi;
   p.skip_prepare = lay.skip_prepare ? kD4cSkipScan | kD4cSkipLoveTrain : 0;
@@ -2714,6 +2719,19 @@
     if (rows == 0) return;
     if (!launch_d4c_select_probe(mode, threads, K, (long)rows, d_keys, d_out, c->stream)) fail("probe_select: threads = %d has no kernel", threads);
   });
+}
+
+int world_hip_d4c_last_bins(int fs, double f0, int *out) {
+  if (!out || fs < 15800 || fs > 192000 || !(f0 >= 0.0)) return -1;
+  const int fft_d4c = d4c_internal_fft(fs);
+  const int nap = static_cast<int>(std::min(15000.0, fs / 2.0 - 3000.0) / 3000.0);
+  const int wl = static_cast<int>(3000.0 * fft_d4c / fs) * 2 + 1;
+  if (fft_d4c > 16384 || nap < 1 || nap > 6) return -1;
+  const int band_last = static_cast<int>(3000.0 * nap * fft_d4c / fs) + wl / 2;
+  const double nyq = 0.5 * fs;
+  d4c_last_bins_host(fs, ilog2_exact(fft_d4c), f0 > nyq ? nyq : f0, band_last, out);
+  out[8] = band_last;
+  return 0;
 }
 
 int world_hip_probe_harvest_contour(WorldHipContext *c, int n_utt, const int *nfb, const int *nc, int maxc, int fb_stride,
diff --git a/world_amd/csrc/d4c.hip b/world_amd/csrc/d4c.hip
--- a/world_amd/csrc/d4c.hip
+++ b/world_amd/csrc/d4c.hip
@@ -322,13 +322,50 @@
   return s1 / s2;
 }
 
+#ifndef D4C_OFFSETS2
+#define D4C_OFFSETS2 1
+#endif
+__device__ __forceinline__ void d4c_offsets2_utt(const D4cParams &p, int u, int nf, int *flag) {
+  if (!D4C_OFFSETS2) return;
+  if (threadIdx.x == 0) {
+    __builtin_amdgcn_fence(__ATOMIC_RELEASE, "agent");
+    const unsigned t = atomicAdd(p.tickets + u, 1u);
+    *flag = t == (unsigned)(nf - 1);
+    if (*flag) __builtin_amdgcn_fence(__ATOMIC_ACQUIRE, "agent");
+  }
+  __syncthreads();
+  if (!*flag) return;
+  const unsigned *cnt = p.draws2 + (size_t)u * p.b.f_stride;
+  unsigned *off_out = p.offsets2 + (size_t)u * p.b.f_stride;
+  int *part = flag + 1;
+  const int nt = blockDim.x, nw = nt / WAVE;
+  unsigned running = 0;
+  for (int base = 0; base < nf; base += nt) {
+    const int g = base + threadIdx.x;
+    const int c = g < nf ? (int)cnt[g] : 0;
+    int wt;
+    const int off = wave_excl_scan_int(c, &wt);
+    __syncthreads();
+    if (lane_id() == 0) part[wave_in_block()] = wt;
+    __syncthreads();
+    unsigned before = 0, tot = 0;
+    for (int w = 0; w < nw; ++w) { const unsigned s = (unsigned)part[w]; if (w < wave_in_block()) before += s; tot += s; }
+    if (g < nf) off_out[g] = running + before + (unsigned)off;
+    running += tot;
+  }
+}
 template <int LGN, bool REC>
 __device__ __forceinline__ void d4c_love_frame(const D4cParams &p, char *lds) {
   const int u = blockIdx.y, f = blockIdx.x;
-  if (f >= p.b.n_frames[u]) return;
+  const int nf_u = p.b.n_frames[u];
+  if (f >= nf_u) return;
   const size_t fi = (size_t)u * p.b.f_stride + f;
   const double f0 = d4c_sane_f0(p.f0[fi], p.b.fs);
-  if (f0 == 0.0) { if (threadIdx.x == 0) { p.ap0[fi] = 0.0; p.draws2[fi] = 0u; } return; }
+  if (f0 == 0.0) {
+    if (threadIdx.x == 0) { p.ap0[fi] = 0.0; p.draws2[fi] = 0u; }
+    d4c_offsets2_utt(p, u, nf_u, reinterpret_cast<int *>(lds));
+    return;
+  }
   const int lgn = LGN > 0 ? LGN : p.lg_love, M = 1 << lgn, fs = p.b.fs;
   cplx *Z = reinterpret_cast<cplx *>(lds);
   double *Zr = reinterpret_cast<double *>(lds);
@@ -377,11 +414,12 @@
     block_cfft_dif_static<LGN - 1, 3, T>(Z, tw);
     const cplx wb = twiddle(tw, tid, LGN, -1);
     const int h = 1 << (LGN - 1);
+    const bool mirrors = b2 >= h / 2;
     rfft_merge_items_w<kItems, T, true>(Z, LGN, plan, [&](int m, int) { return mul_w16_fwd(wb, m); },
                                   [&](int, int k, double ar, double ai, bool paired, double br, double bi) {
       band_power(k, ar, ai);
-      if (paired) band_power(h - k, br, bi);
-    });
+      if (paired && mirrors) band_power(h - k, br, bi);
+    }, [&](int m) { return m * T <= b2; });
   } else {
     const double coef = d4c_window_to_lds(w, rot0, Z, scratch);
     {
@@ -399,6 +437,8 @@
     const int body_hw = REC ? fld(&rec->hw) : d4c_win_half(4.0, fs, bf0);
     p.draws2[fi] = ap0 <= p.threshold ? 0u : 3u * (unsigned)(2 * body_hw + 1);
   }
+  __syncthreads();
+  d4c_offsets2_utt(p, u, nf_u, reinterpret_cast<int *>(lds));
 }
 template <int LGN, bool REC = true>
 __global__ void __launch_bounds__(256) d4c_lovetrain(D4cParams p) {
@@ -443,7 +483,10 @@
   const unsigned draws1_u = p.draws1[u];
   constexpr int kCntAhead = 8;
   unsigned cnt_v[kCntAhead];
-  {
+  unsigned at2 = 0u;
+  if constexpr (REC && D4C_OFFSETS2) {
+    at2 = uniform_const_load(p.offsets2 + fi);
+  } else {
     const unsigned *cnt = p.draws2 + (size_t)u * p.b.f_stride;
 #pragma unroll
     for (int k = 0; k < kCntAhead; ++k) cnt_v[k] = cnt[imin(tid + k * nt, f)];
@@ -466,19 +509,26 @@
   constexpr FftPlan plan = make_plan_max(lgn - 1, 3);
   auto cfft = [&]() __attribute__((always_inline)) { block_cfft_dif_static<lgn - 1, 3, T>(Z, tw); };
   const cplx wb = twiddle(tw, tid, lgn, -1);
-  auto for_nat = [&](auto body) __attribute__((always_inline)) {
+#ifndef D4C_LAST_BINS
+#define D4C_LAST_BINS 1
+#endif
+  const int tid_w = D4C_LAST_BINS ? __builtin_amdgcn_readfirstlane(tid) : 0;
+  auto for_nat = [&](auto body, const int last) __attribute__((always_inline)) {
 #pragma unroll
     for (int m = 0; m < kItems; ++m) {
-      const int it = tid + m * nt;
-      if (it <= q) { body(2 * m, it); if (it < q) body(2 * m + 1, H - it); }
+      const int it = tid + m * nt, it_w = tid_w + m * nt;
+      if (!D4C_LAST_BINS || it_w <= last) { if (it <= q && (!D4C_LAST_BINS || it <= last)) body(2 * m, it); }
+      if (!D4C_LAST_BINS || H - it_w - (WAVE - 1) <= last) { if (it < q && (!D4C_LAST_BINS || H - it <= last)) body(2 * m + 1, H - it); }
       D4C_SCHED_FENCE();
     }
   };
-  auto for_pair = [&](auto body) __attribute__((always_inline)) {
+  auto for_pair = [&](auto body, const int last) __attribute__((always_inline)) {
 #pragma unroll
     for (int m = 0; m < kItems; ++m) {
-      const int it = tid + m * nt;
-      if (it <= q) { body(2 * m, 2 * it); if (it < q) body(2 * m + 1, 2 * it + 1); }
+      const int it = tid + m * nt, it_w = tid_w + m * nt;
+      if (!D4C_LAST_BINS || 2 * it_w <= last) {
+        if (it <= q && (!D4C_LAST_BINS || 2 * it <= last)) { body(2 * m, 2 * it); if (it < q) body(2 * m + 1, 2 * it + 1); }
+      }
       D4C_SCHED_FENCE();
     }
   };
@@ -487,12 +537,15 @@
   D4cFrameRec own;
   const D4cFrameRec *rec = &own;
   if constexpr (REC) rec = p.frec + fi;
-  else d4c_body_consts(own, f0, p.tpos[fi], fs, N, nt);
+  else d4c_body_consts(own, f0, p.tpos[fi], fs, N, nt, p.all_bins ? N : p.band_last);
   auto fld = [](auto *field) __attribute__((always_inline)) {
     if constexpr (REC) return uniform_const_load(field); else return *field;
   };
   unsigned stream_at;
-  {
+  if constexpr (REC && D4C_OFFSETS2) {
+    stream_at = draws1_u + at2;
+    __syncthreads();
+  } else {
     const unsigned *cnt = p.draws2 + (size_t)u * p.b.f_stride;
     unsigned su = 0;
 #pragma unroll
@@ -517,7 +570,7 @@
   auto dc_correct = [&](double (&S)[kBins], auto for_own) __attribute__((always_inline)) {
     const int upper = fld(&rec->upper), nrep = upper - 1;
     __syncthreads();
-    for_own([&](int slot, int k) { if (k <= upper) Zr[k] = S[slot]; });
+    for_own([&](int slot, int k) { if (k <= upper) Zr[k] = S[slot]; }, H);
     __syncthreads();
     const int b0 = fld(&rec->b0);
     const double fr0 = fld(&rec->fr0);
@@ -527,20 +580,24 @@
         const double y0 = Zr[b], y1 = Zr[b + 1 <= upper ? b + 1 : upper];
         S[slot] = keep(S[slot] + (y0 + (y1 - y0) * fr0));
       }
-    });
-    __syncthreads();
-  };
-  auto smooth = [&](const double (&in)[kBins], auto for_in, const D4cSmoothConsts *sc, double (&out)[kBins], auto for_out, const bool pre = true) __attribute__((always_inline)) {
+    }, H);
+    __syncthreads();
+  };
+  auto smooth = [&](const double (&in)[kBins], auto for_in, const int kin, const D4cSmoothConsts *sc, double (&out)[kBins], auto for_out,
+                    const int kout, const bool pre = true) __attribute__((always_inline)) {
     const int bnd = fld(&sc->bnd);
     const int seg_len = H + 2 * bnd + 1;
+    D4cSmoothConsts geo;
+    geo.bnd = bnd; geo.i_hi = fld(&sc->i_hi);
+    const int scan_len = D4C_LAST_BINS ? d4c_scan_len(geo, kout, H, nt) : seg_len;
     if (pre) __syncthreads();
     for_in([&](int slot, int k) {
       const double v = in[slot] * fs * inv_n;
       Zr[k + bnd] = v;
       if (k >= 1 && k <= bnd) Zr[bnd - k] = v;
-      if (k < H && k >= H - bnd) Zr[2 * H + bnd - k] = v;
-    });
-    block_scan_incl_double<T>(Zr, seg_len, scratch);
+      if (k < H && k >= H - bnd && 2 * H + bnd - k < scan_len) Zr[2 * H + bnd - k] = v;
+    }, kin);
+    block_scan_incl_double<T>(Zr, scan_len, scratch, seg_len);
     const double inv_width = fld(&sc->inv_width);
     const int i_lo = fld(&sc->i_lo), i_hi = fld(&sc->i_hi);
     const double f_lo = fld(&sc->f_lo), f_hi = fld(&sc->f_hi);
@@ -549,7 +606,7 @@
       const double l0 = z_lo[k], l1 = z_lo[k + 1], h0 = z_hi[k], h1 = z_hi[k + 1];
       const double lo = l0 + (l1 - l0) * f_lo, hi = h0 + (h1 - h0) * f_hi;
       out[slot] = keep((hi - lo) * inv_width);
-    });
+    }, kout);
     (void)seg_len;
   };
 
@@ -626,6 +683,7 @@
     __syncthreads();
   };
 
+  const int last_ratio = fld(&rec->last[1]);
 #pragma unroll 1
   for (int c = 0; c < 2; ++c) {
     const D4cWin w = d4c_win(x, x_len, fld(&rec->hw), fld(&rec->origin[c]), fld(&rec->scale), kBlackman, noise + (size_t)c * wdraws);
@@ -652,7 +710,8 @@
 #pragma unroll
     for (int m = 0; m < kItems; ++m) {
       const int it = tid + m * nt;
-      if (it <= q) {
+      if (D4C_LAST_BINS && 2 * (tid_w + m * nt) > last_ratio) continue;
+      if (it <= q && (!D4C_LAST_BINS || 2 * it <= last_ratio)) {
         const cplx P = Z[fft_slot(plan, it)], Q = Z[fft_slot(plan, (H - it) & (H - 1))];
         const double v = (P.im * Q.re + Q.im * P.re) * half_inv_pw;
         park[2 * it] = c == 0 ? v : park[2 * it] + v;
@@ -674,7 +733,8 @@
 #pragma unroll
     for (int m = 0; m < kItems; ++m) {
       const int it = tid + m * nt;
-      if (it < q) {
+      if (D4C_LAST_BINS && 2 * (tid_w + m * nt) > last_ratio) continue;
+      if (it < q && (!D4C_LAST_BINS || 2 * it <= last_ratio)) {
         const cplx P = Z[fft_slot(plan, it)], Q = Z[fft_slot(plan, H - 1 - it)];
         const double v = (P.im * Q.re + Q.im * P.re) * half_inv_pw;
         park[2 * it + 1] = c == 0 ? v : park[2 * it + 1] + v;
@@ -718,7 +778,7 @@
       }
     } else
     dc_correct(Bn, for_nat);
-    smooth(Bn, for_nat, &rec->sm[0], B, for_pair, false);
+    smooth(Bn, for_nat, fld(&rec->last[0]), &rec->sm[0], B, for_pair, fld(&rec->last[1]), false);
   }
   WH_STAMP(32, 12);
   lds_dead(Zr, N);
@@ -736,25 +796,26 @@
         v = v + (y0 + (y1 - y0) * fr0);
       }
       A[slot] = keep(v);
-    });
+    }, fld(&rec->last[1]));
   }
   WH_STAMP(32, 13);
   D4C_FRESH_TID();
-#pragma unroll
-  for (int e = 0; e < kBins; ++e) A[e] = fast_div(A[e], B[e]);
+  for_pair([&](int slot, int) { A[slot] = fast_div(A[slot], B[slot]); }, fld(&rec->last[1]));
   D4C_FRESH_TID();
-  smooth(A, for_pair, &rec->sm[1], A, for_pair);
+  smooth(A, for_pair, fld(&rec->last[1]), &rec->sm[1], A, for_pair, fld(&rec->last[2]));
   WH_STAMP(32, 14);
   D4C_FRESH_TID();
-  smooth(A, for_pair, &rec->sm[0], B, for_pair);
-  for_pair([&](int slot, int k) { park[k] = A[slot] - B[slot]; });
+  lds_dead(Zr, N);
+  smooth(A, for_pair, fld(&rec->last[2]), &rec->sm[0], B, for_pair, fld(&rec->last[3]));
+  for_pair([&](int slot, int k) { park[k] = A[slot] - B[slot]; }, fld(&rec->last[3]));
+  lds_dead(park + fld(&rec->last[3]) + 1, H - fld(&rec->last[3]));
   WH_STAMP(32, 15);
 
   const int bnd = REC ? p.band_bnd : mround(N * 8.0 / p.wl);
   const int hwl = p.wl / 2, wl = 2 * hwl + 1;
   const int nz = hwl + 1;
   int mine = 0;
-  for_nat([&](int, int) { ++mine; });
+  for_nat([&](int, int) { ++mine; }, H);
   int *hist = reinterpret_cast<int *>(Zr);
   constexpr int kWaves = (T + WAVE - 1) / WAVE;
   double *band_sums = park_global ? after_tw : park + (H + 2);
@@ -974,6 +1035,18 @@
   return (size_t)(2 * mround(3.0 * fs / 40.0 / 2.0) + 1) + 3 * (size_t)(2 * mround(4.0 * fs / kFloorF0D4C / 2.0) + 1);
 }
 
+void d4c_last_bins_host(int fs, int lg_d4c, double f0, int band_last, int *out) {
+  const int N = 1 << lg_d4c;
+  const double cf0 = kFloorF0D4C > f0 ? kFloorF0D4C : f0;
+  D4cFrameRec r;
+  r.upper = 2 + static_cast<int>(cf0 * N / fs);
+  r.sm[0] = d4c_smooth_consts(cf0, N, fs);
+  r.sm[1] = d4c_smooth_consts(cf0 / 2.0, N, fs);
+  d4c_last_bins(r.last, r.sm, r.upper, band_last, N / 2, d4c_frame_threads(lg_d4c));
+  for (int j = 0; j < 4; ++j) out[j] = r.last[j];
+  out[4] = r.upper; out[5] = r.sm[0].bnd; out[6] = r.sm[1].bnd; out[7] = N / 2;
+}
+
 void launch_spectral_prepare(const CtParams &cp, const D4cParams &dp, int max_frames, hipStream_t stream) {
   WH_BLOCKS(spectral_prepare, dim3(cp.b.n_utt, 2, 1 + rec_chunks(max_frames)), 256, 64 * sizeof(double), stream, cp, dp);
 }
diff --git a/world_amd/csrc/devrt.h b/world_amd/csrc/devrt.h
--- a/world_amd/csrc/devrt.h
+++ b/world_amd/csrc/devrt.h
@@ -637,9 +637,9 @@
 }
 
 template <int NT = 0>
-__device__ __forceinline__ void block_scan_incl_double(double *a, int n, double *scratch) {
+__device__ __forceinline__ void block_scan_incl_double(double *a, int n, double *scratch, int n_of = 0) {
   int nt = wg_size<NT>(), tid = wg_thread<NT>();
-  int chunk = (n + nt - 1) / nt;
+  int chunk = ((n_of > n ? n_of : n) + nt - 1) / nt;
   int lo = tid * chunk, hi = lo + chunk < n ? lo + chunk : n;
   __syncthreads();
 #ifndef WORLD_EMU
diff --git a/world_amd/csrc/fft.h b/world_amd/csrc/fft.h
--- a/world_amd/csrc/fft.h
+++ b/world_amd/csrc/fft.h
@@ -541,14 +541,16 @@
     default: return mul_w16<true, 15>(a);
   }
 }
-template <int KITEMS, int NT, bool TWICE = false, class Wk, class Emit>
-__device__ __forceinline__ void rfft_merge_items_w(cplx *z, int lgn, const FftPlan &plan, Wk wk, Emit emit) {
+struct MergeEveryItem { __device__ __forceinline__ bool operator()(int) const { return true; } };
+template <int KITEMS, int NT, bool TWICE = false, class Wk, class Emit, class Want = MergeEveryItem>
+__device__ __forceinline__ void rfft_merge_items_w(cplx *z, int lgn, const FftPlan &plan, Wk wk, Emit emit, Want want = Want()) {
   const int lgh = lgn - 1, h = 1 << lgh, q = h >> 1;
   const int tid = wg_thread<NT>(), nt = wg_size<NT>();
 #pragma unroll
   for (int m = 0; m < KITEMS; ++m) {
     const int k = tid + m * nt;
-    if (k == 0) {
+    if (!want(m)) {
+    } else if (k == 0) {
       const cplx za = z[fft_slot(plan, 0)];
       const double a = za.re + za.im, b = za.re - za.im;
       if (TWICE) emit(m, 0, a + a, 0.0, true, b + b, 0.0);
diff --git a/world_amd/csrc/prepare.h b/world_amd/csrc/prepare.h
--- a/world_amd/csrc/prepare.h
+++ b/world_amd/csrc/prepare.h
@@ -41,7 +41,7 @@
 __device__ __forceinline__ int d4c_win_half(double ratio, int fs, double f0) { return mround(ratio * fs / f0 / 2.0); }
 __device__ __forceinline__ int d4c_win_origin(double pos, int fs) { return mround(pos * fs + 0.001); }
 __device__ __forceinline__ double d4c_win_scale(double ratio, int fs, double f0) { return 2.0 / ratio / fs * f0; }
-__device__ __forceinline__ D4cSmoothConsts d4c_smooth_consts(double width, int N, int fs) {
+__host__ __device__ __forceinline__ D4cSmoothConsts d4c_smooth_consts(double width, int N, int fs) {
   D4cSmoothConsts s;
   s.bnd = static_cast<int>(width * N / fs) + 1;
   const double origin_axis = -(s.bnd - 0.5) * fs / N;
@@ -53,6 +53,27 @@
   s.pad_ = 0;
   return s;
 }
+__host__ __device__ __forceinline__ int d4c_scan_len(const D4cSmoothConsts &s, int kout, int H, int nt) {
+  const int seg_len = H + 2 * s.bnd + 1, chunk = (seg_len + nt - 1) / nt;
+  const int len = (kout + s.i_hi + 2 + chunk - 1) / chunk * chunk;
+  return len < seg_len ? len : seg_len;
+}
+__host__ __device__ __forceinline__ int d4c_last_odd(int k, int H) { return (k | 1) < H ? (k | 1) : H; }
+__host__ __device__ __forceinline__ int d4c_smooth_input_last(const D4cSmoothConsts &s, int kout, int H, int nt) {
+  int k = d4c_scan_len(s, kout, H, nt) - 1 - s.bnd;
+  k = k > kout ? k : kout;
+  return d4c_last_odd(k > s.bnd ? k : s.bnd, H);
+}
+__host__ __device__ __forceinline__ void d4c_last_bins(int (&last)[4], const D4cSmoothConsts (&sm)[2], int upper, int band_last,
+                                                       int H, int nt) {
+  const int dc = d4c_last_odd(upper, H);
+  last[3] = d4c_last_odd(band_last < H ? band_last : H, H);
+  last[2] = d4c_smooth_input_last(sm[0], last[3], H, nt);
+  last[1] = d4c_smooth_input_last(sm[1], last[2], H, nt);
+  last[1] = last[1] > dc ? last[1] : dc;
+  last[0] = d4c_smooth_input_last(sm[0], last[1], H, nt);
+  last[0] = last[0] > dc ? last[0] : dc;
+}
 __device__ __forceinline__ void d4c_love_consts(D4cFrameRec &r, double f0, double pos, int fs, int nt) {
   const double cf0 = f0 > 40.0 ? f0 : 40.0;
   r.love_hw = d4c_win_half(3.0, fs, cf0);
@@ -60,7 +81,7 @@
   r.love_scale = d4c_win_scale(3.0, fs, cf0);
   sincospi(r.love_scale * nt, &r.love_step_s, &r.love_step_c);
 }
-__device__ __forceinline__ void d4c_body_consts(D4cFrameRec &r, double f0, double pos, int fs, int N, int nt) {
+__device__ __forceinline__ void d4c_body_consts(D4cFrameRec &r, double f0, double pos, int fs, int N, int nt, int band_last) {
   const double cf0 = kFloorF0D4C > f0 ? kFloorF0D4C : f0;
   r.hw = d4c_win_half(4.0, fs, cf0);
   r.scale = d4c_win_scale(4.0, fs, cf0);
@@ -74,6 +95,7 @@
   r.fr0 = pos0 - r.b0;
   r.sm[0] = d4c_smooth_consts(cf0, N, fs);
   r.sm[1] = d4c_smooth_consts(cf0 / 2.0, N, fs);
+  d4c_last_bins(r.last, r.sm, r.upper, band_last, N / 2, nt);
 }
 
 constexpr int kRecSpan = 256;
@@ -93,7 +115,7 @@
     const double pos = p.tpos[fi];
     D4cFrameRec r;
     d4c_love_consts(r, f0f, pos, p.b.fs, p.love_threads);
-    d4c_body_consts(r, f0f, pos, p.b.fs, 1 << p.lg_d4c, p.frame_threads);
+    d4c_body_consts(r, f0f, pos, p.b.fs, 1 << p.lg_d4c, p.frame_threads, p.all_bins ? 1 << p.lg_d4c : p.band_last);
     p.frec[fi] = r;
   }
 }
@@ -134,7 +156,7 @@
     if (f < nf) off_out[f] = running + (unsigned)off;
     running += (unsigned)total;
   }
-  if (threadIdx.x == 0) p.draws1[u] = running;
+  if (threadIdx.x == 0) { p.draws1[u] = running; p.tickets[u] = 0u; }
 }
 
 }
diff --git a/world_amd/csrc/stage_params.h b/world_amd/csrc/stage_params.h
--- a/world_amd/csrc/stage_params.h
+++ b/world_amd/csrc/stage_params.h
@@ -32,6 +32,7 @@
   int hw, origin[3];
   int upper, b0;
   D4cSmoothConsts sm[2];
+  int last[4];
 };
 
 struct CtParams {
@@ -75,10 +76,14 @@
   unsigned *offsets1;
   unsigned *draws2;
   unsigned *draws1;
+  unsigned *offsets2;
+  unsigned *tickets;
   D4cFrameRec *frec;
   int frame_consts;
+  int all_bins;
   int love_threads, frame_threads;
   int love_b[3];
+  int band_last;
   int band_bnd;
   const uint32_t *noise;
   const double *nuttall;
@@ -109,5 +114,6 @@
 int ct_frame_threads(int lg_fft);
 int d4c_love_threads(int lg_love);
 int d4c_frame_threads(int lg_d4c);
+void d4c_last_bins_host(int fs, int lg_d4c, double f0, int band_last, int *out);
 
 }
```

Result: slower. 4.172 million frames/s (-6.1%).
